# lodestone-rock/stable_diffusion_training

Measured on AMD Instinct MI355X. Metric: training images/sec, SD1.5 512×512 bf16, ε-pred MSE parity; 1/2/4/8 GPUs, higher is better.
Workload: dtype bf16; 1 GPU; SD1.5 512x512 train_step: VAE encode + CLIP-L fwd/bwd + UNet fwd/bwd + clip + Lion-8bit + EMA, batch 4/GPU, 77-token captions, random-init weights; global_batch=4, latent=64x64x4, parallelism=dp1, launch=hip_graph, setup_steps=3

## Files before the change

include/sdt.h:

```cpp
#ifndef SDT_H_
#define SDT_H_

#include <stdint.h>

#ifdef __cplusplus
extern "C" {
#endif

#ifndef __HIP_PLATFORM_AMD__
typedef struct ihipStream_t* hipStream_t;
#endif

enum { SDT_OK = 0, SDT_ERR_INVALID_ARG = -1, SDT_ERR_UNSUPPORTED = -2, SDT_ERR_LAUNCH = -3 };

const char* sdt_last_error(void);
int sdt_abi_version(void);
int sdt_device_count(void);

int sdt_event_create(void** event);
int sdt_event_destroy(void* event);
int sdt_event_record(void* event, int external, hipStream_t stream);
int sdt_stream_wait_event(hipStream_t stream, void* event);
int sdt_stream_wait_event_external(hipStream_t stream, void* event);

// ... 41 lines not shown
                             float offset_mag, float perturb_mag, int prediction_type, hipStream_t stream);
int sdt_inpaint_pack_input(const uint16_t* latents_nhwc, const uint16_t* masked_latents_nhwc, const float* latent_mask,
                           uint16_t* input_nhwc, int R, int B, int L, int H, int W, int cpad_src, int cpad_m, int cpad_dst,
                           hipStream_t stream);
int sdt_control_concat_add(const uint16_t* a, const uint16_t* skip, const uint16_t* res, const float* scale, uint16_t* wide,
                           int64_t rows, int64_t rows_per_sample, int Ca, int Cb, hipStream_t stream);
int sdt_ip_attention_fwd(const uint16_t* q, const uint16_t* kv, const uint16_t* o_txt, const float* scale_ip, uint16_t* out, int B, int H,
                         int Nq, int T, int D, int ldq, int ldkv, float scale, hipStream_t stream);
int sdt_ip_attention_bwd(const uint16_t* q, const uint16_t* kv, const uint16_t* dout, const float* scale_ip, const uint16_t* dq_in,
                         uint16_t* dq, uint16_t* dkv, int B, int H, int Nq, int T, int D, int ldq, int ldkv, int ld_dkv, float scale,
                         void* workspace, int64_t workspace_bytes, hipStream_t stream);
int64_t sdt_ip_attention_bwd_workspace_bytes(int B, int H, int Nq, int T, int D);
int sdt_mse_loss_fwd_bwd(const uint16_t* pred_nhwc, const float* target_nchw, const float* weight, float* loss_accum,
                         uint16_t* dpred_nhwc, int B, int C, int H, int W, int cpad, void* workspace, int64_t workspace_bytes,
                         hipStream_t stream);
int64_t sdt_reduce_workspace_bytes(void);
int sdt_loss_mask_prepare(const float* mask, float* effective, float* pooled, float* sums, int B, int h, int w, int f, float floor_value,
                          void* workspace, int64_t workspace_bytes, hipStream_t stream);
int sdt_masked_mse_loss_fwd_bwd(const uint16_t* pred_nhwc, const float* target_nchw, const float* effective_mask, const float* mask_sums,
                                const float* snr_weight, const float* loss_weight, float* loss_accum, float* loss_per_sample,
                                uint16_t* dpred_nhwc, int B, int C, int H, int W, int cpad, void* workspace, int64_t workspace_bytes,
                                hipStream_t stream);
int sdt_robust_loss_fwd_bwd(const uint16_t* pred_nhwc, const float* target_nchw, const float* effective_mask, const float* mask_sums,
                            const float* snr_weight, const float* loss_weight, const float* huber_c, int loss_type, float* loss_accum,
                            float* loss_per_sample, uint16_t* dpred_nhwc, int B, int C, int H, int W, int cpad, void* workspace,
                            int64_t workspace_bytes, hipStream_t stream);
int sdt_timestep_embedding(const int32_t* timesteps, uint16_t* out, int B, int dim, int flip_sin_to_cos,
                           float freq_shift, hipStream_t stream);

int sdt_sqnorm_accumulate(const float* g, int64_t n, double* out_sq, void* workspace, int64_t workspace_bytes, hipStream_t stream);
int sdt_sqnorm_accumulate_bf16(const uint16_t* g, int64_t n, double* out_sq, void* workspace, int64_t workspace_bytes, hipStream_t stream);
int64_t sdt_sqnorm_workspace_bytes(void);
#define SDT_ACC_INIT 0
#define SDT_ACC_ADD 1
#define SDT_ACC_FINISH 2
#define SDT_ACC_SCALE 3
int sdt_grad_accumulate(float* acc, const void* g, int g_bf16, int64_t n, int mode, float scale, double* out_sq, void* workspace,
                        int64_t workspace_bytes, hipStream_t stream);
int sdt_lion8_step(float* p, const void* g, int g_bf16, int8_t* codes, float* inv_scale, float* ema, uint16_t* w_bf16, int64_t n,
                   int block_size, const double* sqnorm, const float* thresholds, double max_norm, double lr, double wd,
                   double b1, double b2, double ema_rate, hipStream_t stream);
int sdt_lion32_step(float* p, const float* g, float* mom, float* ema, uint16_t* w_bf16, int64_t n,
                    const double* sqnorm, double max_norm, double lr, double wd, double b1, double b2, double ema_rate,
                    hipStream_t stream);
int sdt_opt_schedule_select(int64_t* step, const float* lr_tab, int64_t n_lr, const float* ema_tab, int64_t n_ema, float* cur,
                            hipStream_t stream);
int sdt_lion8_step_scheduled(float* p, const void* g, int g_bf16, int8_t* codes, float* inv_scale, float* ema, uint16_t* w_bf16,
                             int64_t n, int block_size, const double* sqnorm, const float* thresholds, double max_norm, const float* cur,
                             double wd, double b1, double b2, hipStream_t stream);
int sdt_lion32_step_scheduled(float* p, const float* g, float* mom, float* ema, uint16_t* w_bf16, int64_t n, const double* sqnorm,
                              double max_norm, const float* cur, double wd, double b1, double b2, hipStream_t stream);
int sdt_adamw_select(int64_t* step, double* prods, const float* lr_tab, int64_t n_lr, const float* ema_tab, int64_t n_ema, double lr,
                     double ema_rate, double b1, double b2, float* cur, hipStream_t stream);
int sdt_adamw8_step(float* p, const void* g, int g_bf16, int8_t* m_codes, float* m_inv_scale, int8_t* s_codes, float* s_inv_scale,
                    float* ema, uint16_t* w_bf16, int64_t n, int block_size, const double* sqnorm, const float* thresholds,
                    double max_norm, const float* cur, double wd, double b1, double b2, double eps, hipStream_t stream);
int sdt_adamw32_step(float* p, const float* g, float* m, float* v, float* ema, uint16_t* w_bf16, int64_t n, const double* sqnorm,
                     double max_norm, const float* cur, double wd, double b1, double b2, double eps, hipStream_t stream);
int sdt_prodigy_select(int64_t* step, double* state, const float* lr_tab, int64_t n_lr, const float* ema_tab, int64_t n_ema, double lr,
                       double ema_rate, double b1, double b2, double d0, int use_bias_correction, int safeguard_warmup, float* cur,
                       hipStream_t stream);
int sdt_prodigy_moments_step(const float* p, const void* g, int g_bf16, float* p0, float* m, float* v, float* s, int64_t n,
                             const double* sqnorm, double max_norm, const float* cur, double* state, double b1, double b2, double beta3,
                             void* workspace, int64_t workspace_bytes, hipStream_t stream);
int sdt_prodigy_finish(double* state, float* cur, double beta3, double d0, double d_coef, double growth_rate, double eps,
                       hipStream_t stream);
int sdt_prodigy_apply_step(float* p, const float* m, const float* v, float* ema, uint16_t* w_bf16, int64_t n, const float* cur, double wd,
                           hipStream_t stream);
int64_t sdt_prodigy_workspace_bytes(void);
int sdt_lion8_quantize(const float* x, int8_t* codes, float* inv_scale, int64_t n, int block_size, const float* thresholds,
                       hipStream_t stream);
int sdt_lion8_dequantize(const int8_t* codes, const float* inv_scale, float* x, int64_t n, int block_size,
                         hipStream_t stream);

int sdt_groupnorm_fwd(const uint16_t* x, const float* gamma, const float* beta, uint16_t* y, float* stats, int B, int HW,
                      int C, int G, float eps, int fuse_silu, const float* parts, int nparts, void* workspace,
                      int64_t workspace_bytes, hipStream_t stream);
int64_t sdt_groupnorm_fwd_workspace_bytes(int B, int HW, int C, int G);
int sdt_groupnorm_bwd(const uint16_t* x, const uint16_t* dy, const float* stats, const float* gamma, const float* beta,
                      uint16_t* dx, float* dgamma, float* dbeta, const uint16_t* dres, int B, int HW, int C, int G, float eps,
                      int fuse_silu, void* workspace, int64_t workspace_bytes, hipStream_t stream);
int64_t sdt_groupnorm_bwd_workspace_bytes(int B, int HW, int C);
int sdt_layernorm_fwd(const uint16_t* x, const float* gamma, const float* beta, uint16_t* y, float* mean_rstd, int64_t M,
                      int C, float eps, hipStream_t stream);
int sdt_layernorm_bwd(const uint16_t* x, const uint16_t* dy, const float* gamma, const float* mean_rstd, uint16_t* dx,
                      float* dgamma, float* dbeta, const uint16_t* dres, int64_t M, int C, int defer_param_grads, void* workspace,
                      int64_t workspace_bytes, hipStream_t stream);
int64_t sdt_layernorm_bwd_workspace_bytes(int64_t M, int C);
int64_t sdt_layernorm_bwd_partial_rows(int64_t M, int C);
typedef struct SdtNormGradJob {
  const float* partial;
  float* dgamma;
  float* dbeta;
  int nrows, C;
} SdtNormGradJob;
int sdt_norm_param_grads_group(const SdtNormGradJob* jobs, int n, hipStream_t stream);
int sdt_norm_param_grads_group_max(void);
int sdt_clip_pool_fwd(const int32_t* ids, const uint16_t* x, const float* gamma, const float* beta, uint16_t* pooled, float* mean_rstd,
                      int32_t* pos, int R, int windows, int S, int D, int eos_id, float eps, hipStream_t stream);
int sdt_clip_pool_bwd(const uint16_t* x, const uint16_t* dpooled, const float* gamma, const float* mean_rstd, const int32_t* pos,
                      uint16_t* dx, float* dgamma, float* dbeta, int R, int windows, int S, int D, hipStream_t stream);

int sdt_gemm_nt_bf16(const uint16_t* A, const uint16_t* Bt, uint16_t* C, const float* bias, const uint16_t* rowbias,
                     const uint16_t* residual, int64_t M, int N, int Kc, int taps, int lda, int ldb,
                     int64_t b_tap_stride, int ldc, int ldres, int rows_per_batch, int gather_mode,
                     const SdtConvGeom* geom, void* workspace, int64_t workspace_bytes, float* gn_stats, int gn_groups,
                     int b_kmajor, int b_nseg, int64_t b_seg_stride, int ld_rowbias, hipStream_t stream);
int sdt_gemm_nt_gn_parts(int64_t M, int N, int Kc, int taps, int rows_per_batch, int gn_groups, int gather_mode,
                         const SdtConvGeom* geom);
int64_t sdt_gemm_nt_workspace_bytes(int64_t M, int N, int Kc, int taps);
int sdt_ff_geglu_supported(int64_t M, int F, int K);
int sdt_ff_geglu_fwd(const uint16_t* x, const uint16_t* W1, const float* bias, uint16_t* h, uint16_t* out, int64_t M, int F, int K,
                     hipStream_t stream);


int sdt_gemm_tn_wgrad(const uint16_t* A, const uint16_t* dY, void* dW, int dw_bf16, float* dbias, int64_t M, int K1, int N, int K1_valid,
                      int N_valid, int taps, int lda, int ldb, int ldw, int64_t w_tap_stride, int n_seg, int64_t seg_stride,
                      int gather_mode, const SdtConvGeom* geom, void* workspace, int64_t workspace_bytes, double* sq_slots,
                      hipStream_t stream);
int64_t sdt_wgrad_sq_slots(int K1, int N, int taps);
int sdt_sum_f64_accumulate(const double* x, int64_t n, double* out, void* workspace, int64_t workspace_bytes, hipStream_t stream);
int64_t sdt_gemm_tn_workspace_bytes(int64_t M, int K1, int N, int taps, int n_seg, int gather_mode, const SdtConvGeom* geom);
typedef struct SdtTnProblem {
  const uint16_t* A;
  const uint16_t* dY;
  void* dW;
  float* dbias;
  int64_t M;
  int K1, N, K1_valid, N_valid, lda, ldb, ldw, n_seg;
  int64_t seg_stride;
  double* sq_slots;
  int dw_bf16;
} SdtTnProblem;
int sdt_gemm_tn_wgrad_group(const SdtTnProblem* problems, int n, void* workspace, int64_t workspace_bytes, hipStream_t stream);
int64_t sdt_gemm_tn_wgrad_group_workspace_bytes(const SdtTnProblem* problems, int n);
int sdt_gemm_tn_wgrad_group_max(void);
typedef struct SdtConvWgradProblem {
  const uint16_t* A;
  const uint16_t* dY;
  void* dW;
  float* dbias;
  SdtConvGeom geom;
  int K1, N, K1_valid, N_valid, lda, ldb;
  double* sq_slots;
  int dw_bf16;
} SdtConvWgradProblem;
int sdt_conv_wgrad_group(const SdtConvWgradProblem* problems, int n, void* workspace, int64_t workspace_bytes, hipStream_t stream);
int64_t sdt_conv_wgrad_group_workspace_bytes(const SdtConvWgradProblem* problems, int n);
int sdt_colsum_accumulate(const uint16_t* dy, float* db, int64_t M, int N, int ld, void* workspace, int64_t workspace_bytes,
                          hipStream_t stream);
int sdt_colsum_batched_bf16(const uint16_t* dy, uint16_t* out, int batch, int64_t rows_per_batch, int N, int ld, void* workspace,
                            int64_t workspace_bytes, hipStream_t stream);
int64_t sdt_colsum_workspace_bytes(int batch, int64_t rows_per_batch, int N);

int sdt_attention_fwd(const uint16_t* q, const uint16_t* k, const uint16_t* v, uint16_t* out, float* lse,
                      const SdtAttnDesc* desc, hipStream_t stream);
int sdt_attention_bwd(const uint16_t* q, const uint16_t* k, const uint16_t* v, const uint16_t* out, const uint16_t* dout,
                      const float* lse, uint16_t* dq, uint16_t* dk, uint16_t* dv, float* workspace, int64_t workspace_bytes,
                      const SdtAttnDesc* desc, hipStream_t stream);
int64_t sdt_attention_bwd_workspace_bytes(const SdtAttnDesc* desc);
int sdt_softmax_rows_inplace(uint16_t* x, int64_t rows, int n, float scale, hipStream_t stream);

int sdt_act_fwd(const uint16_t* x, uint16_t* y, int64_t n, int act, hipStream_t stream);
int sdt_act_bwd(const uint16_t* x, const uint16_t* dy, uint16_t* dx, int64_t n, int act, hipStream_t stream);
int sdt_geglu_fwd(const uint16_t* h, uint16_t* out, int64_t M, int F, hipStream_t stream);
int sdt_geglu_bwd(const uint16_t* h, const uint16_t* dout, uint16_t* dh, int64_t M, int F, hipStream_t stream);
int sdt_sum_n_bf16(const uint16_t* const* inputs, int n, uint16_t* out, int64_t numel, hipStream_t stream);
int sdt_copy2d_bf16(uint16_t* dst, int64_t dst_stride, const uint16_t* src, int64_t src_stride, int64_t rows, int cols,
                    hipStream_t stream);
int sdt_copy_cols_bf16(uint16_t* wide, int64_t ld_wide, void* const* parts, const int64_t* ld_parts, const int* cols, int n,
                       int64_t rows, int to_wide, hipStream_t stream);
int sdt_add_bf16(const uint16_t* a, const uint16_t* b, uint16_t* y, int64_t n, hipStream_t stream);
int sdt_upsample2x_fwd(const uint16_t* x, uint16_t* y, int B, int H, int W, int C, hipStream_t stream);
int sdt_upsample2x_bwd(const uint16_t* dy, uint16_t* dx, int B, int H, int W, int C, hipStream_t stream);
int sdt_nchw_f32_to_nhwc_bf16(const float* x, uint16_t* y, int B, int C, int H, int W, int cpad, hipStream_t stream);
int sdt_nhwc_bf16_to_nchw_f32(const uint16_t* x, float* y, int B, int C, int H, int W, int cpad, hipStream_t stream);
int sdt_cast_f32_to_bf16(const float* x, uint16_t* y, int64_t n, hipStream_t stream);
int sdt_transpose_bf16(const uint16_t* x, uint16_t* y, int batch, int R, int C, hipStream_t stream);
int sdt_param_prepare(const float* master, uint16_t* w_bf16, uint16_t* wt_bf16, const void* descs_device, int ndesc,
                      int total_tiles, hipStream_t stream);
int sdt_param_prepare_desc_size(void);
int sdt_zero_ranges(float* base, const int64_t* ranges_device, int nranges, hipStream_t stream);
int sdt_zero_ranges_chunk(void);
int sdt_embedding_fwd(const int32_t* ids, const float* tok, const float* pos, uint16_t* out, int64_t rows, int S, int D,
                      hipStream_t stream);
int sdt_embedding_bwd(const int32_t* ids, const uint16_t* dout, float* dtok, float* dpos, int64_t rows, int S, int D,
                      hipStream_t stream);

int sdt_embedding_ext_fwd(const int32_t* ids, const float* tok, const float* ext, const float* pos, uint16_t* out, int64_t rows, int S,
                          int D, int V, int n_ext, hipStream_t stream);
int sdt_embedding_ext_bwd(const int32_t* ids, const uint16_t* dout, float* dext, int64_t rows, int D, int V, int n_ext,
                          hipStream_t stream);
int sdt_embedding_retract(float* ext, int n_ext, int D, double target_std, double power, double* stats, hipStream_t stream);

typedef struct SdtLoraJob {
  int64_t w0_off;
  int64_t a_off, b_off;
  int64_t w_off, f_off;
  int64_t dw_off;
  int64_t ga_off, gb_off;
  int32_t K, N, r;
  float scale;
  int32_t tile0_merge, tile0_project, tiles_da, reserved;
} SdtLoraJob;
int sdt_lora_job_size(void);
int sdt_lora_merge(const float* w0_base, const float* ab_base, uint16_t* w_bf16, float* f32_dst, const SdtLoraJob* jobs_host,
                   const void* jobs_device, int n, hipStream_t stream);
int sdt_lora_project(const uint16_t* dw_base, const float* ab_base, float* grad_base, const SdtLoraJob* jobs_host,
                     const void* jobs_device, int n, hipStream_t stream);

typedef struct SdtDoraJob {
  int64_t m_off;
  int64_t gm_off;
  int64_t stat_off;
  int32_t N;
  int32_t stripe0_merge;
} SdtDoraJob;
int sdt_dora_job_size(void);
int sdt_dora_merge(const float* w0_base, const float* ab_base, uint16_t* w_bf16, float* f32_dst, float* stat_base,
                   const SdtLoraJob* jobs_host, const SdtDoraJob* dora_host, const void* jobs_device, const void* dora_device, int n,
                   hipStream_t stream);
int sdt_dora_init_magnitude(const float* w0_base, const float* ab_base, float* m_base, const SdtLoraJob* jobs_host,
                            const SdtDoraJob* dora_host, const void* jobs_device, const void* dora_device, int n, hipStream_t stream);
int sdt_dora_project(const uint16_t* dw_base, const float* w0_base, const float* ab_base, float* grad_base, const float* stat_base,
                     const SdtLoraJob* jobs_host, const SdtDoraJob* dora_host, const void* jobs_device, const void* dora_device, int n,
                     hipStream_t stream);

int sdt_dpo_loss_fwd_bwd(const uint16_t* pred_nhwc, const uint16_t* ref_pred_nhwc, const float* target_nchw, float beta, float* loss_accum,
                         float* sample_mse, float* logits, float* pair_loss, float* coef, uint16_t* dpred_nhwc, int B, int C, int H, int W,
                         int cpad, void* workspace, int64_t workspace_bytes, hipStream_t stream);
int64_t sdt_dpo_loss_workspace_bytes(int B, int H, int W);
int sdt_lora_restore(const float* w0_base, uint16_t* w_bf16, const SdtLoraJob* jobs_host, const void* jobs_device, int n,
                     hipStream_t stream);

typedef struct SdtLoraSplitJob {
  int64_t part_off;
  int32_t K, N;
  int32_t tile0;
  int32_t chunks;
  int32_t cnt0;
  int32_t reserved;
} SdtLoraSplitJob;
int sdt_lora_split_job_size(void);
int sdt_lora_project_split_rows(void);
int64_t sdt_lora_project_split_workspace_bytes(const SdtLoraJob* jobs_host, int n);
int sdt_lora_project_split(const uint16_t* dw_base, const float* ab_base, float* grad_base, const SdtLoraJob* jobs_host,
                           const SdtLoraSplitJob* split_host, const void* jobs_device, const void* split_device, int n, void* workspace,
                           int64_t workspace_bytes, hipStream_t stream);

typedef struct SdtLohaJob {
  int64_t a2_off, b2_off;
  int64_t ga2_off, gb2_off;
  int64_t part_off;
  int32_t K, N;
} SdtLohaJob;
int sdt_loha_job_size(void);
int sdt_loha_merge(const float* w0_base, const float* ab_base, uint16_t* w_bf16, float* f32_dst, const SdtLoraJob* jobs_host,
                   const SdtLohaJob* loha_host, const void* jobs_device, const void* loha_device, int n, hipStream_t stream);
int64_t sdt_loha_project_workspace_bytes(const SdtLoraJob* jobs_host, int n);
int sdt_loha_project(const uint16_t* dw_base, const float* ab_base, float* grad_base, const SdtLoraJob* jobs_host,
                     const SdtLoraSplitJob* split_host, const SdtLohaJob* loha_host, const void* jobs_device, const void* split_device,
                     const void* loha_device, int n, void* workspace, int64_t workspace_bytes, hipStream_t stream);

int sdt_conv_halo_set_tile_width(int bn);

#ifdef __cplusplus
}
#endif
#endif
```

stable_diffusion_training_amd/_lib.py:

```python
import ctypes
import os

_P = ctypes.c_void_p
_I = ctypes.c_int
_L = ctypes.c_int64
_F = ctypes.c_float
_D = ctypes.c_double


class SdtConvGeom(ctypes.Structure):
    _fields_ = [(n, _I) for n in ("batch", "in_h", "in_w", "out_h", "out_w", "kh", "kw", "stride", "pad_top", "pad_left")]


class SdtAttnDesc(ctypes.Structure):
    _fields_ = [("B", _I), ("H", _I), ("Nq", _I), ("Nk", _I), ("D", _I), ("ldq", _I), ("ldk", _I), ("ldv", _I),
                ("ldo", _I), ("scale", _F), ("causal", _I), ("ldgrad_q", _I), ("ldgrad_k", _I), ("ldgrad_v", _I),
                ("ld_dout", _I), ("key_weight", _P)]


class SdtPrepDesc(ctypes.Structure):
    _fields_ = [("src_off", _L), ("w_off", _L), ("wt_off", _L), ("batch", _I), ("R", _I), ("C", _I), ("Rp", _I),
                ("Cp", _I), ("tile0", _I), ("flags", _I)]


class SdtNormGradJob(ctypes.Structure):
    _fields_ = [("partial", _P), ("dgamma", _P), ("dbeta", _P), ("nrows", _I), ("C", _I)]


class SdtConvWgradProblem(ctypes.Structure):
    _fields_ = [("A", _P), ("dY", _P), ("dW", _P), ("dbias", _P), ("geom", SdtConvGeom), ("K1", _I), ("N", _I), ("K1_valid", _I),
                ("N_valid", _I), ("lda", _I), ("ldb", _I), ("sq_slots", _P), ("dw_bf16", _I)]


class SdtTnProblem(ctypes.Structure):
    _fields_ = [("A", _P), ("dY", _P), ("dW", _P), ("dbias", _P), ("M", _L), ("K1", _I), ("N", _I), ("K1_valid", _I),
                ("N_valid", _I), ("lda", _I), ("ldb", _I), ("ldw", _I), ("n_seg", _I), ("seg_stride", _L), ("sq_slots", _P), ("dw_bf16", _I)]


class SdtLoraJob(ctypes.Structure):
    _fields_ = [(n, _L) for n in ("w0_off", "a_off", "b_off", "w_off", "f_off", "dw_off", "ga_off", "gb_off")] + [
        ("K", _I), ("N", _I), ("r", _I), ("scale", _F), ("tile0_merge", _I), ("tile0_project", _I), ("tiles_da", _I), ("reserved", _I)]


class SdtDoraJob(ctypes.Structure):
    _fields_ = [("m_off", _L), ("gm_off", _L), ("stat_off", _L), ("N", _I), ("stripe0_merge", _I)]


class SdtLoraSplitJob(ctypes.Structure):
    _fields_ = [("part_off", _L), ("K", _I), ("N", _I), ("tile0", _I), ("chunks", _I), ("cnt0", _I), ("reserved", _I)]


class SdtLohaJob(ctypes.Structure):
    _fields_ = [(n, _L) for n in ("a2_off", "b2_off", "ga2_off", "gb2_off", "part_off")] + [("K", _I), ("N", _I)]


GATHER_PLAIN, GATHER_FPROP, GATHER_DGRAD = 0, 1, 2
ACT_SILU, ACT_QUICK_GELU, ACT_GELU_ERF = 0, 1, 2

SIGNATURES = {
    "sdt_add_noise_velocity": [_P, _P, _P, _P, _P, _P, _P, _I, _I, _I, _I, _I, _P],
    "sdt_vae_posterior_sample": [_P, _P, _P, _I, _I, _I, _I, _I, _F, _P],
    "sdt_latent_noise_target": [_P, _P, _P, _P, _P, _P, _P, _P, _P, _P, _P, _I, _I, _I, _I, _I, _I, _F, _F, _F, _I, _P],
    "sdt_inpaint_mask_pixels": [_P, _P, _P, _P, _I, _I, _I, _I, _I, _I, _P],
    "sdt_inpaint_noise_target": [_P, _P, _P, _P, _P, _P, _P, _P, _P, _P, _P, _P, _P, _P, _P, _I, _I, _I, _I, _I, _I, _F, _F, _F, _I, _P],
    "sdt_inpaint_pack_input": [_P, _P, _P, _P, _I, _I, _I, _I, _I, _I, _I, _I, _P],
    "sdt_control_concat_add": [_P, _P, _P, _P, _P, _L, _L, _I, _I, _P],
    "sdt_ip_attention_fwd": [_P, _P, _P, _P, _P, _I, _I, _I, _I, _I, _I, _I, _F, _P],
    "sdt_ip_attention_bwd": [_P, _P, _P, _P, _P, _P, _P, _I, _I, _I, _I, _I, _I, _I, _I, _F, _P, _L, _P],
    "sdt_ddim_cfg_step": [_P, _P, _P, _I, _I, _I, _I, _I, _F, _F, _F, _I, _P],
    "sdt_cfg_rescale_factors": [_P, _P, _I, _I, _I, _I, _I, _F, _F, _P],
    "sdt_sampler_cfg_step": [_P, _P, _P, _P, _P, _I, _I, _I, _I, _I, _F, _F, _F, _I, _F, _F, _F, _F, _P],
    "sdt_mse_loss_fwd_bwd": [_P, _P, _P, _P, _P, _I, _I, _I, _I, _I, _P, _L, _P],
    "sdt_loss_mask_prepare": [_P, _P, _P, _P, _I, _I, _I, _I, _F, _P, _L, _P],
    "sdt_masked_mse_loss_fwd_bwd": [_P, _P, _P, _P, _P, _P, _P, _P, _P, _I, _I, _I, _I, _I, _P, _L, _P],
    "sdt_robust_loss_fwd_bwd": [_P, _P, _P, _P, _P, _P, _P, _I, _P, _P, _P, _I, _I, _I, _I, _I, _P, _L, _P],
    "sdt_dpo_loss_fwd_bwd": [_P, _P, _P, _F, _P, _P, _P, _P, _P, _P, _I, _I, _I, _I, _I, _P, _L, _P],
    "sdt_timestep_embedding": [_P, _P, _I, _I, _I, _F, _P],
    "sdt_sqnorm_accumulate": [_P, _L, _P, _P, _L, _P],
    "sdt_sqnorm_accumulate_bf16": [_P, _L, _P, _P, _L, _P],
    "sdt_grad_accumulate": [_P, _P, _I, _L, _I, _F, _P, _P, _L, _P],
    "sdt_lion8_step": [_P, _P, _I, _P, _P, _P, _P, _L, _I, _P, _P, _D, _D, _D, _D, _D, _D, _P],
    "sdt_lion32_step": [_P, _P, _P, _P, _P, _L, _P, _D, _D, _D, _D, _D, _D, _P],
    "sdt_opt_schedule_select": [_P, _P, _L, _P, _L, _P, _P],
    "sdt_lion8_step_scheduled": [_P, _P, _I, _P, _P, _P, _P, _L, _I, _P, _P, _D, _P, _D, _D, _D, _P],
    "sdt_lion32_step_scheduled": [_P, _P, _P, _P, _P, _L, _P, _D, _P, _D, _D, _D, _P],
    "sdt_adamw_select": [_P, _P, _P, _L, _P, _L, _D, _D, _D, _D, _P, _P],
    "sdt_adamw8_step": [_P, _P, _I, _P, _P, _P, _P, _P, _P, _L, _I, _P, _P, _D, _P, _D, _D, _D, _D, _P],
    "sdt_adamw32_step": [_P, _P, _P, _P, _P, _P, _L, _P, _D, _P, _D, _D, _D, _D, _P],
    "sdt_prodigy_select": [_P, _P, _P, _L, _P, _L, _D, _D, _D, _D, _D, _I, _I, _P, _P],
    "sdt_prodigy_moments_step": [_P, _P, _I, _P, _P, _P, _P, _L, _P, _D, _P, _P, _D, _D, _D, _P, _L, _P],
    "sdt_prodigy_finish": [_P, _P, _D, _D, _D, _D, _D, _P],
    "sdt_prodigy_apply_step": [_P, _P, _P, _P, _P, _L, _P, _D, _P],
    "sdt_lion8_quantize": [_P, _P, _P, _L, _I, _P, _P],
    "sdt_lion8_dequantize": [_P, _P, _P, _L, _I, _P],
    "sdt_groupnorm_fwd": [_P, _P, _P, _P, _P, _I, _I, _I, _I, _F, _I, _P, _I, _P, _L, _P],
    "sdt_groupnorm_bwd": [_P, _P, _P, _P, _P, _P, _P, _P, _P, _I, _I, _I, _I, _F, _I, _P, _L, _P],
    "sdt_layernorm_fwd": [_P, _P, _P, _P, _P, _L, _I, _F, _P],
    "sdt_layernorm_bwd": [_P, _P, _P, _P, _P, _P, _P, _P, _L, _I, _I, _P, _L, _P],
    "sdt_norm_param_grads_group": [_P, _I, _P],
    "sdt_clip_pool_fwd": [_P, _P, _P, _P, _P, _P, _P, _I, _I, _I, _I, _I, _F, _P],
    "sdt_clip_pool_bwd": [_P, _P, _P, _P, _P, _P, _P, _P, _I, _I, _I, _I, _P],
    "sdt_sum_n_bf16": [_P, _I, _P, _L, _P],
    "sdt_event_create": [_P],
    "sdt_event_destroy": [_P],
    "sdt_event_record": [_P, _I, _P],
    "sdt_stream_wait_event": [_P, _P],
    "sdt_stream_wait_event_external": [_P, _P],
    "sdt_gemm_nt_bf16": [_P, _P, _P, _P, _P, _P, _L, _I, _I, _I, _I, _I, _L, _I, _I, _I, _I, _P, _P, _L, _P, _I, _I, _I, _L, _I, _P],
    "sdt_gemm_nt_gn_parts": [_L, _I, _I, _I, _I, _I, _I, _P],
    "sdt_gemm_tn_wgrad": [_P, _P, _P, _I, _P, _L, _I, _I, _I, _I, _I, _I, _I, _I, _L, _I, _L, _I, _P, _P, _L, _P, _P],
    "sdt_sum_f64_accumulate": [_P, _L, _P, _P, _L, _P],
    "sdt_gemm_tn_wgrad_group": [_P, _I, _P, _L, _P],
    "sdt_conv_wgrad_group": [_P, _I, _P, _L, _P],
    "sdt_zero_ranges": [_P, _P, _I, _P],
    "sdt_colsum_accumulate": [_P, _P, _L, _I, _I, _P, _L, _P],
    "sdt_colsum_batched_bf16": [_P, _P, _I, _L, _I, _I, _P, _L, _P],
    "sdt_attention_fwd": [_P, _P, _P, _P, _P, _P, _P],
    "sdt_attention_bwd": [_P, _P, _P, _P, _P, _P, _P, _P, _P, _P, _L, _P, _P],
    "sdt_softmax_rows_inplace": [_P, _L, _I, _F, _P],
    "sdt_act_fwd": [_P, _P, _L, _I, _P],
    "sdt_act_bwd": [_P, _P, _P, _L, _I, _P],
    "sdt_geglu_fwd": [_P, _P, _L, _I, _P],
    "sdt_geglu_bwd": [_P, _P, _P, _L, _I, _P],
    "sdt_copy2d_bf16": [_P, _L, _P, _L, _L, _I, _P],
    "sdt_copy_cols_bf16": [_P, _L, _P, _P, _P, _I, _L, _I, _P],
    "sdt_add_bf16": [_P, _P, _P, _L, _P],
    "sdt_upsample2x_fwd": [_P, _P, _I, _I, _I, _I, _P],
    "sdt_upsample2x_bwd": [_P, _P, _I, _I, _I, _I, _P],
    "sdt_nchw_f32_to_nhwc_bf16": [_P, _P, _I, _I, _I, _I, _I, _P],
    "sdt_nhwc_bf16_to_nchw_f32": [_P, _P, _I, _I, _I, _I, _I, _P],
    "sdt_cast_f32_to_bf16": [_P, _P, _L, _P],
    "sdt_transpose_bf16": [_P, _P, _I, _I, _I, _P],
    "sdt_param_prepare": [_P, _P, _P, _P, _I, _I, _P],
    "sdt_lora_merge": [_P, _P, _P, _P, _P, _P, _I, _P],
    "sdt_lora_restore": [_P, _P, _P, _P, _I, _P],
    "sdt_lora_project": [_P, _P, _P, _P, _P, _I, _P],
    "sdt_lora_project_split": [_P, _P, _P, _P, _P, _P, _P, _I, _P, _L, _P],
    "sdt_loha_merge": [_P, _P, _P, _P, _P, _P, _P, _P, _I, _P],
    "sdt_loha_project": [_P, _P, _P, _P, _P, _P, _P, _P, _P, _I, _P, _L, _P],
    "sdt_dora_merge": [_P, _P, _P, _P, _P, _P, _P, _P, _P, _I, _P],
    "sdt_dora_init_magnitude": [_P, _P, _P, _P, _P, _P, _P, _I, _P],
    "sdt_dora_project": [_P, _P, _P, _P, _P, _P, _P, _P, _P, _I, _P],
    "sdt_embedding_fwd": [_P, _P, _P, _P, _L, _I, _I, _P],
    "sdt_embedding_bwd": [_P, _P, _P, _P, _L, _I, _I, _P],
    "sdt_embedding_ext_fwd": [_P, _P, _P, _P, _P, _L, _I, _I, _I, _I, _P],
    "sdt_embedding_ext_bwd": [_P, _P, _P, _L, _I, _I, _I, _P],
    "sdt_embedding_retract": [_P, _I, _I, _D, _D, _P, _P],
    "sdt_ff_geglu_fwd": [_P, _P, _P, _P, _P, _L, _I, _I, _P],
    "sdt_ff_geglu_supported": [_L, _I, _I],
    "sdt_conv_halo_set_tile_width": [_I],
}
WS_QUERY = {"sdt_gemm_nt_workspace_bytes": [_L, _I, _I, _I], "sdt_gemm_tn_workspace_bytes": [_L, _I, _I, _I, _I, _I, _P], "sdt_layernorm_bwd_workspace_bytes": [_L, _I], "sdt_layernorm_bwd_partial_rows": [_L, _I],
            "sdt_groupnorm_bwd_workspace_bytes": [_I, _I, _I],
            "sdt_groupnorm_fwd_workspace_bytes": [_I, _I, _I, _I], "sdt_attention_bwd_workspace_bytes": [_P],
            "sdt_ip_attention_bwd_workspace_bytes": [_I, _I, _I, _I, _I],
            "sdt_gemm_tn_wgrad_group_workspace_bytes": [_P, _I], "sdt_conv_wgrad_group_workspace_bytes": [_P, _I], "sdt_reduce_workspace_bytes": [], "sdt_dpo_loss_workspace_bytes": [_I, _I, _I], "sdt_sqnorm_workspace_bytes": [], "sdt_prodigy_workspace_bytes": [], "sdt_colsum_workspace_bytes": [_I, _L, _I],
            "sdt_lora_project_split_workspace_bytes": [_P, _I],
            "sdt_loha_project_workspace_bytes": [_P, _I],
            "sdt_wgrad_sq_slots": [_I, _I, _I]}
NOARG = {"sdt_abi_version": _I, "sdt_gemm_tn_wgrad_group_max": _I, "sdt_norm_param_grads_group_max": _I, "sdt_zero_ranges_chunk": _I, "sdt_device_count": _I, "sdt_param_prepare_desc_size": _I, "sdt_lora_job_size": _I, "sdt_dora_job_size": _I, "sdt_lora_split_job_size": _I, "sdt_lora_project_split_rows": _I, "sdt_loha_job_size": _I, "sdt_last_error": ctypes.c_char_p}

LIB_PATH = os.path.join(os.path.dirname(os.path.abspath(__file__)), "csrc", "libsdtrain_hip.so")
if os.environ.get("SDT_LIB"):
    LIB_PATH = os.path.abspath(os.environ["SDT_LIB"])
_lib = None


class SdtError(RuntimeError):
    pass


def load():
    global _lib
    if _lib is not None:
        return _lib
    if not os.path.exists(LIB_PATH):
        raise SdtError(f"{LIB_PATH} is missing: run `python -c 'import __graft_entry__ as g; g.build()'` "
                       "(hipcc --offload-arch=gfx950). There is no CPU fallback.")
    import torch
    lib = ctypes.CDLL(LIB_PATH)
    for name, argtypes in SIGNATURES.items():
        fn = getattr(lib, name)
        fn.argtypes = argtypes
        fn.restype = _I
    for name, argtypes in WS_QUERY.items():
        fn = getattr(lib, name)
        fn.argtypes = argtypes
        fn.restype = _L
    for name, res in NOARG.items():
        fn = getattr(lib, name)
        fn.argtypes = []
        fn.restype = res
    if lib.sdt_param_prepare_desc_size() != ctypes.sizeof(SdtPrepDesc):
        raise SdtError("SdtPrepDesc layout mismatch between _lib.py and the library")
    if lib.sdt_lora_job_size() != ctypes.sizeof(SdtLoraJob):
        raise SdtError("SdtLoraJob layout mismatch between _lib.py and the library")
    if lib.sdt_dora_job_size() != ctypes.sizeof(SdtDoraJob):
        raise SdtError("SdtDoraJob layout mismatch between _lib.py and the library")
    if lib.sdt_lora_split_job_size() != ctypes.sizeof(SdtLoraSplitJob):
        raise SdtError("SdtLoraSplitJob layout mismatch between _lib.py and the library")
    if lib.sdt_loha_job_size() != ctypes.sizeof(SdtLohaJob):
        raise SdtError("SdtLohaJob layout mismatch between _lib.py and the library")
    _lib = lib
    return lib


def require_device():
    lib = load()
    if lib.sdt_device_count() < 1:
        raise SdtError("no HIP device visible: the train_step hot path runs only on the HIP kernels (no CPU fallback)")
    return lib


def call(name, *args):
    lib = _lib if _lib is not None else load()
    rc = getattr(lib, name)(*args)
    if rc != 0:
        raise SdtError(f"{name} failed ({rc}): {lib.sdt_last_error().decode()}")
```

stable_diffusion_training_amd/csrc/attention.hip:

```cpp
#include <type_traits>

#include "sdt_common.h"

#define KT 64
#define NEG_BIG -1.0e30f

typedef __attribute__((ext_vector_type(4))) short s16x4_t;

__device__ __attribute__((aligned(16))) unsigned int g_attn_zero16[4] = {0u, 0u, 0u, 0u};
__device__ __attribute__((aligned(16))) unsigned int g_attn_one16[4] = {0x3f80u, 0u, 0u, 0u};

__device__ __forceinline__ unsigned lds_offset_of(const void* p) {
  return (unsigned)(size_t)(__attribute__((address_space(3))) const unsigned char*)p;
}
__device__ __forceinline__ void glds16(const void* gsrc, void* lds_wave_base) {
  unsigned keep;
  asm volatile("s_mov_b32 %0, m0\n\ts_mov_b32 m0, %2\n\ts_nop 0\n\tglobal_load_lds_dwordx4 %1, off\n\ts_mov_b32 m0, %0"
               : "=&s"(keep) : "v"(gsrc), "s"(lds_offset_of(lds_wave_base)) : "memory");
}
__device__ __forceinline__ void glds4(const void* gsrc, void* lds_wave_base) {
  unsigned keep;
  asm volatile("s_mov_b32 %0, m0\n\ts_mov_b32 m0, %2\n\ts_nop 0\n\tglobal_load_lds_dword %1, off\n\ts_mov_b32 m0, %0"
               : "=&s"(keep) : "v"(gsrc), "s"(lds_offset_of(lds_wave_base)) : "memory");
}
// ... 241 lines not shown
        }
      if (!MSUM) l_run += psum;
    }
  };
  attn_tile_loops(tiles, p.key_w != nullptr, p.causal != 0, 0, kend, p.Nk);
  float l_tot;
  if (MSUM) l_tot = __shfl(o_acc[NB - 1][12], fr, 64);
  else l_tot = l_run + __shfl_xor(l_run, 32, 64);
  const float inv_l = 1.f / l_tot;
  if (qi < p.Nq) {
    if (fh == 0 && p.lse) p.lse[((long)b * p.H + h) * p.Nq + qi] = m_run * p.scale2 + log2f(l_tot);
    bf16_t* ob = p.out + (long)b * p.bso + (long)qi * p.ldo + h * p.D;
#pragma unroll
    for (int i = 0; i < NB; ++i)
#pragma unroll
      for (int g4 = 0; g4 < 4; ++g4) {
        const int d = i * 32 + 8 * g4 + 4 * fh;
        if (d < p.D) {
          uint2 pk;
          pk.x = pack2bf(o_acc[i][4 * g4] * inv_l, o_acc[i][4 * g4 + 1] * inv_l);
          pk.y = pack2bf(o_acc[i][4 * g4 + 2] * inv_l, o_acc[i][4 * g4 + 3] * inv_l);
          *reinterpret_cast<uint2*>(ob + d) = pk;
        }
      }
  }
}

template <int DPP, int NS, int NB>
__global__ void __launch_bounds__(256) attn_bwd_dq_kernel(const AttnParams p) {
  extern __shared__ __attribute__((aligned(16))) unsigned char smem[];
  using I = Img<DPP>;
  constexpr int STAGE = 2 * I::BYTES;
  const int lane = threadIdx.x & 63, wave = threadIdx.x >> 6, fr = lane & 31, fh = lane >> 5;
  const int wave_u = __builtin_amdgcn_readfirstlane(wave);
  const int b = blockIdx.z, h = blockIdx.y;
  const int q0 = blockIdx.x * 128;
  const int qi = q0 + wave * 32 + fr;
  const bf16_t* qb = p.q + (long)b * p.bsq + h * p.D;
  const bf16_t* dob = p.dout + (long)b * p.bsdo + h * p.D;
  const bf16_t* kb = p.k + (long)b * p.bsk + h * p.D;
  const bf16_t* vb = p.v + (long)b * p.bsv + h * p.D;

  TileDma<DPP> dma, dmav;
  dma.init(wave, lane, p.D);
  dmav.init(wave, lane, p.D);
  TrLane<DPP> tr;
  tr.init(lane);
  int kend = p.Nk;
  if (p.causal) kend = min(p.Nk, q0 + 128);
  dma.bind(kb, p.ldk, 0);
  dmav.bind(vb, p.ldv, 0);
  dma.issue(0, p.Nk, smem, wave_u);
  dmav.issue(0, p.Nk, smem + I::BYTES, wave_u);

  bf16x8_t qf[NS], dof[NS];
#pragma unroll
  for (int s = 0; s < NS; ++s) {
    uint4 v = make_uint4(0, 0, 0, 0), w = make_uint4(0, 0, 0, 0);
    const int d0 = 16 * s + 8 * fh;
    if (qi < p.Nq && d0 < p.D) {
      v = *reinterpret_cast<const uint4*>(qb + (long)qi * p.ldq + d0);
      w = *reinterpret_cast<const uint4*>(dob + (long)qi * p.lddo + d0);
    }
    qf[s] = __builtin_bit_cast(bf16x8_t, v);
    dof[s] = __builtin_bit_cast(bf16x8_t, w);
  }
  float lse2 = 0.f, dlt = 0.f;
  if (qi < p.Nq) {
    lse2 = p.lse[((long)b * p.H + h) * p.Nq + qi];
    const bf16_t* orow = p.o + (long)b * p.bso + (long)qi * p.ldo + h * p.D;
#pragma unroll
    for (int s = 0; s < NS; ++s) {
      const int d0 = 16 * s + 8 * fh;
      if (d0 < p.D) {
        float fo[8], fd[8];
        unpack8(*reinterpret_cast<const uint4*>(orow + d0), fo);
        unpack8(__builtin_bit_cast(uint4, dof[s]), fd);
#pragma unroll
        for (int e = 0; e < 8; ++e) dlt += fo[e] * fd[e];
      }
    }
  }
  dlt += __shfl_xor(dlt, 32, 64);
  if (qi < p.Nq && fh == 0) const_cast<float*>(p.delta)[((long)b * p.H + h) * p.Nq + qi] = dlt;
  f32x16_t dq_acc[NB];
#pragma unroll
  for (int i = 0; i < NB; ++i)
#pragma unroll
    for (int e = 0; e < 16; ++e) dq_acc[i][e] = 0.f;

  int cur = 0;
  auto tiles = [&](auto masked, auto weighted, int kfrom, int kto) {
    constexpr bool MASK = decltype(masked)::value, KW = decltype(weighted)::value;
    for (int kbase = kfrom; kbase < kto; kbase += KT, cur ^= 1) {
      dma_join();
      if (kbase + KT < kend) {
        dma.issue(kbase + KT, p.Nk, smem + (cur ^ 1) * STAGE, wave_u);
        dmav.issue(kbase + KT, p.Nk, smem + (cur ^ 1) * STAGE + I::BYTES, wave_u);
      }
      const unsigned char* k_img = smem + cur * STAGE;
      const unsigned char* v_img = k_img + I::BYTES;
#pragma unroll
      for (int kt = 0; kt < 2; ++kt) {
        f32x16_t st, dpt;
#pragma unroll
        for (int e = 0; e < 16; ++e) { st[e] = 0.f; dpt[e] = -dlt; }
#pragma unroll
        for (int s = 0; s < NS; ++s) {
          const bf16x8_t kf = row_frag<DPP>(k_img, kt * 32 + fr, 2 * s + fh);
          st = __builtin_amdgcn_mfma_f32_32x32x16_bf16(kf, qf[s], st, 0, 0, 0);
          const bf16x8_t vf = row_frag<DPP>(v_img, kt * 32 + fr, 2 * s + fh);
          dpt = __builtin_amdgcn_mfma_f32_32x32x16_bf16(vf, dof[s], dpt, 0, 0, 0);
        }
        float ds[16];
#pragma unroll
        for (int e = 0; e < 16; ++e) {
          float pv = __builtin_amdgcn_exp2f(fmaf(st[e], p.scale2, -lse2));
          const int key = kbase + kt * 32 + (e & 3) + 8 * (e >> 2) + 4 * fh;
          if (MASK) pv = (key >= p.Nk || (p.causal && key > qi) || qi >= p.Nq) ? 0.f : pv;
          if (KW) pv *= p.key_w[min(key, p.Nk - 1)];
          ds[e] = pv * dpt[e];
        }
#pragma unroll
        for (int s = 0; s < 2; ++s) {
          const bf16x8_t dsf = cvt_frag(ds + 8 * s);
#pragma unroll
          for (int i = 0; i < NB; ++i) {
            const bf16x8_t ktf = tr.frag(k_img, kt * 32 + 16 * s, i);
            dq_acc[i] = __builtin_amdgcn_mfma_f32_32x32x16_bf16(ktf, dsf, dq_acc[i], 0, 0, 0);
          }
        }
      }
    }
  };
  attn_tile_loops(tiles, p.key_w != nullptr, p.causal || q0 + 128 > p.Nq, 0, kend, p.Nk);
  if (qi < p.Nq) {
    bf16_t* ob = p.dq + (long)b * p.bsdq + (long)qi * p.lddq + h * p.D;
#pragma unroll
    for (int i = 0; i < NB; ++i)
#pragma unroll
      for (int g4 = 0; g4 < 4; ++g4) {
        const int d = i * 32 + 8 * g4 + 4 * fh;
        if (d < p.D) {
          uint2 pk;
          pk.x = pack2bf(dq_acc[i][4 * g4] * p.scale, dq_acc[i][4 * g4 + 1] * p.scale);
          pk.y = pack2bf(dq_acc[i][4 * g4 + 2] * p.scale, dq_acc[i][4 * g4 + 3] * p.scale);
          *reinterpret_cast<uint2*>(ob + d) = pk;
        }
      }
  }
}

template <int DPP, int NS, int NB, bool QSPLIT>
__global__ void __launch_bounds__(256) attn_bwd_dkv_kernel(const AttnParams p) {
  extern __shared__ __attribute__((aligned(16))) unsigned char smem[];
  using I = Img<DPP>;
  constexpr int STAGE = 2 * I::BYTES + 2 * KT * 4;
  const int lane = threadIdx.x & 63, wave = threadIdx.x >> 6, fr = lane & 31, fh = lane >> 5;
  const int wave_u = __builtin_amdgcn_readfirstlane(wave);
  const int b = blockIdx.z, h = blockIdx.y;
  const int kblk = QSPLIT ? (int)blockIdx.x % p.kblocks : (int)blockIdx.x;
  const int k0 = kblk * 128;
  const int ki = k0 + wave * 32 + fr;
  const float kwt = p.key_w ? p.key_w[min(ki, p.Nk - 1)] : 1.f;
  const bf16_t* qb = p.q + (long)b * p.bsq + h * p.D;
  const bf16_t* dob = p.dout + (long)b * p.bsdo + h * p.D;
  const bf16_t* kb = p.k + (long)b * p.bsk + h * p.D;
  const bf16_t* vb = p.v + (long)b * p.bsv + h * p.D;
  const float* lse_g = p.lse + ((long)b * p.H + h) * p.Nq;
  const float* dlt_g = p.delta + ((long)b * p.H + h) * p.Nq;

  TileDma<DPP> dma, dmad;
  dma.init(wave, lane, p.D);
  dmad.init(wave, lane, p.D);
  TrLane<DPP> tr;
  tr.init(lane);
  int qstart = 0, qend = p.Nq;
  if (p.causal) qstart = (k0 / KT) * KT;
  if (QSPLIT) {
    qstart = ((int)blockIdx.x / p.kblocks) * p.qchunk;
    qend = min(p.Nq, qstart + p.qchunk);
  }
  dma.bind(qb, p.ldq, qstart);
  dmad.bind(dob, p.lddo, qstart);
  auto stage = [&](int qbase, unsigned char* st) {
    dma.issue(qbase, p.Nq, st, wave_u);
    dmad.issue(qbase, p.Nq, st + I::BYTES, wave_u);
    if (wave_u < 2) {
      const int q = min(qbase + lane, p.Nq - 1);
      glds4((wave_u == 0 ? lse_g : dlt_g) + q, st + 2 * I::BYTES + wave_u * (KT * 4));
    }
  };
  if (qstart < qend) stage(qstart, smem);

  bf16x8_t kf[NS], vf[NS];
#pragma unroll
  for (int s = 0; s < NS; ++s) {
    uint4 v = make_uint4(0, 0, 0, 0), w = make_uint4(0, 0, 0, 0);
    const int d0 = 16 * s + 8 * fh;
    if (ki < p.Nk && d0 < p.D) {
      v = *reinterpret_cast<const uint4*>(kb + (long)ki * p.ldk + d0);
      w = *reinterpret_cast<const uint4*>(vb + (long)ki * p.ldv + d0);
    }
    kf[s] = __builtin_bit_cast(bf16x8_t, v);
    vf[s] = __builtin_bit_cast(bf16x8_t, w);
  }
  f32x16_t dk_acc[NB], dv_acc[NB];
#pragma unroll
  for (int i = 0; i < NB; ++i)
#pragma unroll
    for (int e = 0; e < 16; ++e) { dk_acc[i][e] = 0.f; dv_acc[i][e] = 0.f; }

  int cur = 0;
  auto tiles = [&](auto masked, auto weighted, int qfrom, int qto) {
    constexpr bool MASK = decltype(masked)::value, KW = decltype(weighted)::value;
    for (int qbase = qfrom; qbase < qto; qbase += KT, cur ^= 1) {
      dma_join();
      if (qbase + KT < qend) stage(qbase + KT, smem + (cur ^ 1) * STAGE);
      const unsigned char* q_img = smem + cur * STAGE;
      const unsigned char* do_img = q_img + I::BYTES;
      const float* lse_s = reinterpret_cast<const float*>(q_img + 2 * I::BYTES);
      const float* dlt_s = lse_s + KT;
#pragma unroll
      for (int qt = 0; qt < 2; ++qt) {
        f32x16_t sa, dpa;
        float lrow[16];
#pragma unroll
        for (int g4 = 0; g4 < 4; ++g4) {
          const float4 l4 = *reinterpret_cast<const float4*>(lse_s + qt * 32 + 8 * g4 + 4 * fh);
          const float4 d4 = *reinterpret_cast<const float4*>(dlt_s + qt * 32 + 8 * g4 + 4 * fh);
          lrow[4 * g4] = l4.x; lrow[4 * g4 + 1] = l4.y; lrow[4 * g4 + 2] = l4.z; lrow[4 * g4 + 3] = l4.w;
          dpa[4 * g4] = -d4.x; dpa[4 * g4 + 1] = -d4.y; dpa[4 * g4 + 2] = -d4.z; dpa[4 * g4 + 3] = -d4.w;
        }
#pragma unroll
        for (int e = 0; e < 16; ++e) sa[e] = 0.f;
#pragma unroll
        for (int s = 0; s < NS; ++s) {
          const bf16x8_t qf = row_frag<DPP>(q_img, qt * 32 + fr, 2 * s + fh);
          sa = __builtin_amdgcn_mfma_f32_32x32x16_bf16(qf, kf[s], sa, 0, 0, 0);
          const bf16x8_t df = row_frag<DPP>(do_img, qt * 32 + fr, 2 * s + fh);
          dpa = __builtin_amdgcn_mfma_f32_32x32x16_bf16(df, vf[s], dpa, 0, 0, 0);
        }
        float pr[16], ds[16];
#pragma unroll
        for (int e = 0; e < 16; ++e) {
          float pv = __builtin_amdgcn_exp2f(fmaf(sa[e], p.scale2, -lrow[e]));
          if (KW) pv *= kwt;
          if (MASK) {
            const int q = qbase + qt * 32 + (e & 3) + 8 * (e >> 2) + 4 * fh;
            pv = (q >= p.Nq || ki >= p.Nk || (p.causal && ki > q)) ? 0.f : pv;
          }
          pr[e] = pv;
          ds[e] = pv * dpa[e];
        }
#pragma unroll
        for (int s = 0; s < 2; ++s) {
          const bf16x8_t pf = cvt_frag(pr + 8 * s);
          const bf16x8_t dsf = cvt_frag(ds + 8 * s);
#pragma unroll
          for (int i = 0; i < NB; ++i) {
            const bf16x8_t dotf = tr.frag(do_img, qt * 32 + 16 * s, i);
            dv_acc[i] = __builtin_amdgcn_mfma_f32_32x32x16_bf16(dotf, pf, dv_acc[i], 0, 0, 0);
            const bf16x8_t qtf = tr.frag(q_img, qt * 32 + 16 * s, i);
            dk_acc[i] = __builtin_amdgcn_mfma_f32_32x32x16_bf16(qtf, dsf, dk_acc[i], 0, 0, 0);
          }
        }
      }
    }
  };
  attn_tile_loops(tiles, p.key_w != nullptr, p.causal || k0 + 128 > p.Nk, qstart, qend, p.Nq);
  if (QSPLIT) {
    if (ki < p.Nk) {
      const long C = (long)p.H * p.D;
      const long slab = 2 * (long)p.B * p.Nk * C;
      float* wk = p.kv_ws + ((int)blockIdx.x / p.kblocks) * slab + ((long)b * p.Nk + ki) * C + h * p.D;
      float* wv = wk + (long)p.B * p.Nk * C;
#pragma unroll
      for (int i = 0; i < NB; ++i)
#pragma unroll
        for (int g4 = 0; g4 < 4; ++g4) {
          const int d = i * 32 + 8 * g4 + 4 * fh;
          if (d < p.D) {
            *reinterpret_cast<float4*>(wk + d) = make_float4(dk_acc[i][4 * g4] * p.scale, dk_acc[i][4 * g4 + 1] * p.scale,
                                                             dk_acc[i][4 * g4 + 2] * p.scale, dk_acc[i][4 * g4 + 3] * p.scale);
            *reinterpret_cast<float4*>(wv + d) = make_float4(dv_acc[i][4 * g4], dv_acc[i][4 * g4 + 1], dv_acc[i][4 * g4 + 2], dv_acc[i][4 * g4 + 3]);
          }
        }
    }
    return;
  }
  if (ki < p.Nk) {
    bf16_t* dkb = p.dk + (long)b * p.bsdk + (long)ki * p.lddk + h * p.D;
    bf16_t* dvb = p.dv + (long)b * p.bsdv + (long)ki * p.lddv + h * p.D;
#pragma unroll
    for (int i = 0; i < NB; ++i)
#pragma unroll
      for (int g4 = 0; g4 < 4; ++g4) {
        const int d = i * 32 + 8 * g4 + 4 * fh;
        if (d < p.D) {
          uint2 pk;
          pk.x = pack2bf(dk_acc[i][4 * g4] * p.scale, dk_acc[i][4 * g4 + 1] * p.scale);
          pk.y = pack2bf(dk_acc[i][4 * g4 + 2] * p.scale, dk_acc[i][4 * g4 + 3] * p.scale);
          *reinterpret_cast<uint2*>(dkb + d) = pk;
          pk.x = pack2bf(dv_acc[i][4 * g4], dv_acc[i][4 * g4 + 1]);
          pk.y = pack2bf(dv_acc[i][4 * g4 + 2], dv_acc[i][4 * g4 + 3]);
          *reinterpret_cast<uint2*>(dvb + d) = pk;
        }
      }
  }
}

__global__ void __launch_bounds__(256) attn_kv_finish_kernel(const AttnParams p, int nsplit) {
  const int C = p.H * p.D, cv = C >> 3;
  const long rows = (long)p.B * p.Nk, total = rows * cv;
  const long slab = 2 * rows * C;
  for (long i = (long)blockIdx.x * blockDim.x + threadIdx.x; i < total; i += (long)gridDim.x * blockDim.x) {
    const long r = i / cv;
    const int c = (int)(i - r * cv) * 8;
    const int b = (int)(r / p.Nk), ki = (int)(r - (long)b * p.Nk);
    float fk[8], fv[8];
#pragma unroll
    for (int e = 0; e < 8; ++e) { fk[e] = 0.f; fv[e] = 0.f; }
    for (int sp = 0; sp < nsplit; ++sp) {
      const float* wk = p.kv_ws + sp * slab + r * C + c;
      const float* wv = wk + rows * C;
      const float4 a0 = *reinterpret_cast<const float4*>(wk), a1 = *reinterpret_cast<const float4*>(wk + 4);
      const float4 b0 = *reinterpret_cast<const float4*>(wv), b1 = *reinterpret_cast<const float4*>(wv + 4);
      fk[0] += a0.x; fk[1] += a0.y; fk[2] += a0.z; fk[3] += a0.w; fk[4] += a1.x; fk[5] += a1.y; fk[6] += a1.z; fk[7] += a1.w;
      fv[0] += b0.x; fv[1] += b0.y; fv[2] += b0.z; fv[3] += b0.w; fv[4] += b1.x; fv[5] += b1.y; fv[6] += b1.z; fv[7] += b1.w;
    }
    *reinterpret_cast<uint4*>(p.dk + (long)b * p.bsdk + (long)ki * p.lddk + c) = pack8(fk);
    *reinterpret_cast<uint4*>(p.dv + (long)b * p.bsdv + (long)ki * p.lddv + c) = pack8(fv);
  }
}

static int attn_qsplits(int B, int H, int Nq, int Nk, int causal) {
  if (causal) return 1;
  const long base = (long)sdt_ceil_div(Nk, 128) * H * B;
  if (base >= 128 || Nq < 1024) return 1;
  int s = (int)((256 + base - 1) / base);
  const int max_s = Nq / 256;
  if (s > max_s) s = max_s;
  return s < 2 ? 1 : s;
}

static int attn_fill(AttnParams* p, const SdtAttnDesc* d, const char* name) {
  SDT_CHECK_ARG(d, "%s: null descriptor", name);
  SDT_CHECK_ARG(d->B > 0 && d->H > 0 && d->Nq > 0 && d->Nk > 0 && d->D > 0 && d->B <= 65535 && d->H <= 65535,
                "%s: bad shape B=%d H=%d Nq=%d Nk=%d D=%d", name, d->B, d->H, d->Nq, d->Nk, d->D);
  SDT_CHECK_ARG(d->D % 8 == 0 && d->D <= 160, "%s: head dim %d must be a multiple of 8 and <= 160", name, d->D);
  SDT_CHECK_ARG(d->ldq % 8 == 0 && d->ldk % 8 == 0 && d->ldv % 8 == 0 && d->ldo % 8 == 0, "%s: row strides must be multiples of 8", name);
  SDT_CHECK_ARG(d->ldq < (1 << 24) && d->ldk < (1 << 24) && d->ldv < (1 << 24) && d->ldo < (1 << 24) && d->ld_dout < (1 << 24),
                "%s: row strides must be below 2^24 elements (a tile's byte step is kept in 32 bits)", name);
  p->B = d->B; p->H = d->H; p->Nq = d->Nq; p->Nk = d->Nk; p->D = d->D;
  p->ldq = d->ldq; p->ldk = d->ldk; p->ldv = d->ldv; p->ldo = d->ldo;
  p->bsq = (long)d->Nq * d->ldq; p->bsk = (long)d->Nk * d->ldk; p->bsv = (long)d->Nk * d->ldv; p->bso = (long)d->Nq * d->ldo;
  p->lddo = d->ldo; p->bsdo = p->bso;
  p->lddq = d->ldq; p->bsdq = p->bsq; p->lddk = d->ldk; p->bsdk = p->bsk; p->lddv = d->ldv; p->bsdv = p->bsv;
  p->scale = d->scale;
  p->scale2 = d->scale * 1.4426950408889634f;
  p->causal = d->causal;
  p->key_w = d->key_weight;
  return SDT_OK;
}

template <typename K>
static void ensure_lds(K kernel, size_t lds, bool* done) {
  if (!*done) {
    hipFuncSetAttribute((const void*)kernel, hipFuncAttributeMaxDynamicSharedMemorySize, (int)lds);
    *done = true;
  }
}
template <int DPP, int NS, int NB>
static void launch_fwd(const AttnParams& p, hipStream_t stream) {
  static_assert(NB * 32 <= DPP && NS * 16 <= DPP, "image pitch too small");
  static bool set_m = false, set_a = false;
  const size_t lds = (size_t)2 * 2 * Img<DPP>::BYTES;
  const dim3 grid(sdt_ceil_div(p.Nq, 128), p.H, p.B);
  if (p.D <= NB * 32 - 8) {
    ensure_lds(attn_fwd_kernel<DPP, NS, NB, true>, lds, &set_m);
    hipLaunchKernelGGL((attn_fwd_kernel<DPP, NS, NB, true>), grid, dim3(256), lds, stream, p);
  } else {
    ensure_lds(attn_fwd_kernel<DPP, NS, NB, false>, lds, &set_a);
    hipLaunchKernelGGL((attn_fwd_kernel<DPP, NS, NB, false>), grid, dim3(256), lds, stream, p);
  }
}
template <int DPP, int NS, int NB>
static void launch_bwd(const AttnParams& p, hipStream_t stream) {
  static_assert(NB * 32 <= DPP && NS * 16 <= DPP, "image pitch too small");
  static bool set_q = false, set_kv = false;
  const size_t lds_dq = (size_t)2 * 2 * Img<DPP>::BYTES;
  const size_t lds_dkv = (size_t)2 * (2 * Img<DPP>::BYTES + 2 * KT * sizeof(float));
  static bool set_kvs = false;
  ensure_lds(attn_bwd_dq_kernel<DPP, NS, NB>, lds_dq, &set_q);
  hipLaunchKernelGGL((attn_bwd_dq_kernel<DPP, NS, NB>), dim3(sdt_ceil_div(p.Nq, 128), p.H, p.B), dim3(256), lds_dq, stream, p);
  if (p.kv_ws) {
    AttnParams ps = p;
    const int splits = attn_qsplits(p.B, p.H, p.Nq, p.Nk, p.causal);
    ps.kblocks = sdt_ceil_div(p.Nk, 128);
    ps.qchunk = sdt_ceil_div(sdt_ceil_div(p.Nq, splits), KT) * KT;
    const int nsplit = sdt_ceil_div(p.Nq, ps.qchunk);
    ensure_lds(attn_bwd_dkv_kernel<DPP, NS, NB, true>, lds_dkv, &set_kvs);
    hipLaunchKernelGGL((attn_bwd_dkv_kernel<DPP, NS, NB, true>), dim3(ps.kblocks * nsplit, p.H, p.B), dim3(256), lds_dkv, stream, ps);
    hipLaunchKernelGGL(attn_kv_finish_kernel, dim3(sdt_grid_1d((long)p.B * p.Nk * p.H * p.D / 8, 256, 1024)), dim3(256), 0, stream, ps, nsplit);
  } else {
    ensure_lds(attn_bwd_dkv_kernel<DPP, NS, NB, false>, lds_dkv, &set_kv);
    hipLaunchKernelGGL((attn_bwd_dkv_kernel<DPP, NS, NB, false>), dim3(sdt_ceil_div(p.Nk, 128), p.H, p.B), dim3(256), lds_dkv, stream, p);
  }
}

extern "C" {

int sdt_attention_fwd(const uint16_t* q, const uint16_t* k, const uint16_t* v, uint16_t* out, float* lse,
                      const SdtAttnDesc* desc, hipStream_t stream) {
  SDT_CHECK_ARG(q && k && v && out, "sdt_attention_fwd: null pointer");
  AttnParams p = {};
  int rc = attn_fill(&p, desc, "sdt_attention_fwd");
  if (rc) return rc;
  SDT_CHECK_ARG((((uintptr_t)q | (uintptr_t)k | (uintptr_t)v | (uintptr_t)out) & 15) == 0, "sdt_attention_fwd: pointers must be 16-byte aligned");
  p.q = (const bf16_t*)q; p.k = (const bf16_t*)k; p.v = (const bf16_t*)v; p.out = (bf16_t*)out; p.lse = lse;
  const int D = p.D;
  if (D <= 48) launch_fwd<64, 3, 2>(p, stream);
  else if (D <= 64) launch_fwd<64, 4, 2>(p, stream);
  else if (D <= 80) launch_fwd<128, 5, 3>(p, stream);
  else if (D <= 96) launch_fwd<128, 6, 3>(p, stream);
  else if (D <= 128) launch_fwd<128, 8, 4>(p, stream);
  else launch_fwd<256, 10, 5>(p, stream);
  SDT_LAUNCH_CHECK("sdt_attention_fwd");
  return SDT_OK;
}

int64_t sdt_attention_bwd_workspace_bytes(const SdtAttnDesc* d) {
  if (!d || d->B <= 0 || d->H <= 0 || d->Nq <= 0 || d->Nk <= 0 || d->D <= 0) return 0;
  int64_t n = (int64_t)d->B * d->H * d->Nq;
  n = (n + 3) / 4 * 4;
  const int qs = attn_qsplits(d->B, d->H, d->Nq, d->Nk, d->causal);
  if (qs > 1) n += (int64_t)qs * 2 * d->B * d->Nk * d->H * d->D;
  return n * (int64_t)sizeof(float);
}

int sdt_attention_bwd(const uint16_t* q, const uint16_t* k, const uint16_t* v, const uint16_t* out, const uint16_t* dout,
                      const float* lse, uint16_t* dq, uint16_t* dk, uint16_t* dv, float* delta_ws, int64_t workspace_bytes,
                      const SdtAttnDesc* desc, hipStream_t stream) {
  SDT_CHECK_ARG(q && k && v && out && dout && lse && dq && dk && dv && delta_ws, "sdt_attention_bwd: null pointer");
  SDT_CHECK_ARG(desc && workspace_bytes >= (int64_t)sizeof(float) * desc->B * desc->H * desc->Nq, "sdt_attention_bwd: workspace too small");
  AttnParams p = {};
  int rc = attn_fill(&p, desc, "sdt_attention_bwd");
  if (rc) return rc;
  p.q = (const bf16_t*)q; p.k = (const bf16_t*)k; p.v = (const bf16_t*)v; p.o = (const bf16_t*)out;
  p.dout = (const bf16_t*)dout; p.lse = const_cast<float*>(lse); p.delta = delta_ws;
  p.dq = (bf16_t*)dq; p.dk = (bf16_t*)dk; p.dv = (bf16_t*)dv;
  if (desc->ldgrad_q) { p.lddq = desc->ldgrad_q; p.bsdq = (long)p.Nq * p.lddq; }
  if (desc->ldgrad_k) { p.lddk = desc->ldgrad_k; p.bsdk = (long)p.Nk * p.lddk; }
  if (desc->ldgrad_v) { p.lddv = desc->ldgrad_v; p.bsdv = (long)p.Nk * p.lddv; }
  if (desc->ld_dout) { p.lddo = desc->ld_dout; p.bsdo = (long)p.Nq * p.lddo; }
  if (attn_qsplits(p.B, p.H, p.Nq, p.Nk, p.causal) > 1 && workspace_bytes >= sdt_attention_bwd_workspace_bytes(desc))
    p.kv_ws = delta_ws + ((long)p.B * p.H * p.Nq + 3) / 4 * 4;
  const int D = p.D;
  if (D <= 48) launch_bwd<64, 3, 2>(p, stream);
  else if (D <= 64) launch_bwd<64, 4, 2>(p, stream);
  else if (D <= 80) launch_bwd<128, 5, 3>(p, stream);
  else if (D <= 96) launch_bwd<128, 6, 3>(p, stream);
  else if (D <= 128) launch_bwd<128, 8, 4>(p, stream);
  else launch_bwd<256, 10, 5>(p, stream);
  SDT_LAUNCH_CHECK("sdt_attention_bwd");
  return SDT_OK;
}

}
```

stable_diffusion_training_amd/csrc/elementwise.hip:

```cpp
#include "sdt_common.h"

__global__ void __launch_bounds__(256) add_noise_kernel(const float* __restrict__ lat, const float* __restrict__ noise,
                                                        const int* __restrict__ t, const float* __restrict__ acp,
                                                        bf16_t* __restrict__ noisy_nhwc, float* __restrict__ noisy_nchw,
                                                        float* __restrict__ vel_nchw, int B, int C, int HW, int cpad) {
  const long total = (long)B * HW;
  for (long i = (long)blockIdx.x * blockDim.x + threadIdx.x; i < total; i += (long)gridDim.x * blockDim.x) {
    const int b = (int)(i / HW), p = (int)(i % HW);
    const float a = acp[t[b]];
    const float sa = sqrtf(a), so = sqrtf(1.0f - a);
    for (int c = 0; c < cpad; ++c) {
      float nz = 0.f;
      if (c < C) {
        const long off = ((long)b * C + c) * HW + p;
        const float x0 = lat[off], e = noise[off];
        nz = sa * x0 + so * e;
        if (noisy_nchw) noisy_nchw[off] = nz;
        if (vel_nchw) vel_nchw[off] = sa * e - so * x0;
      }
      noisy_nhwc[i * cpad + c] = f2bf(nz);
    }
  }
}

// ... 973 lines not shown
                   ((d.src_off | d.w_off | d.wt_off) & 3) == 0;
  if (vec) {
#pragma unroll
    for (int ps = 0; ps < 4; ++ps) {
      const int r = ps * 16 + (threadIdx.x >> 4), c = (threadIdx.x & 15) * 4;
      const float4 f = *reinterpret_cast<const float4*>(src + (long)(r0 + r) * d.C + c0 + c);
      uint2 pk;
      pk.x = pack2bf(f.x, f.y);
      pk.y = pack2bf(f.z, f.w);
      *reinterpret_cast<uint2*>(w + (long)(r0 + r) * d.Cp + c0 + c) = pk;
      tile[r][c] = (bf16_t)(pk.x & 0xffffu); tile[r][c + 1] = (bf16_t)(pk.x >> 16);
      tile[r][c + 2] = (bf16_t)(pk.y & 0xffffu); tile[r][c + 3] = (bf16_t)(pk.y >> 16);
    }
    if (!wt) return;
    __syncthreads();
#pragma unroll
    for (int ps = 0; ps < 4; ++ps) {
      const int c = ps * 16 + (threadIdx.x >> 4), r = (threadIdx.x & 15) * 4;
      uint2 pk;
      pk.x = (unsigned)(unsigned short)tile[r][c] | ((unsigned)(unsigned short)tile[r + 1][c] << 16);
      pk.y = (unsigned)(unsigned short)tile[r + 2][c] | ((unsigned)(unsigned short)tile[r + 3][c] << 16);
      *reinterpret_cast<uint2*>(wt + (long)(c0 + c) * d.Rp + r0 + r) = pk;
    }
    return;
  }
  for (int i = threadIdx.x; i < 64 * 64; i += 256) {
    const int r = i >> 6, c = i & 63;
    bf16_t v = 0;
    if (r0 + r < d.R && c0 + c < d.C) v = f2bf(src[(long)(r0 + r) * d.C + c0 + c]);
    tile[r][c] = v;
    if (r0 + r < d.Rp && c0 + c < d.Cp) w[(long)(r0 + r) * d.Cp + c0 + c] = v;
  }
  if (!wt) return;
  __syncthreads();
  for (int i = threadIdx.x; i < 64 * 64; i += 256) {
    const int c = i >> 6, r = i & 63;
    if (r0 + r < d.Rp && c0 + c < d.Cp) wt[(long)(c0 + c) * d.Rp + r0 + r] = tile[r][c];
  }
}

__global__ void __launch_bounds__(256) embedding_fwd_kernel(const int* __restrict__ ids, const float* __restrict__ tok,
                                                            const float* __restrict__ pos, bf16_t* __restrict__ out,
                                                            long rows, int S, int D) {
  const long total = rows * D;
  for (long i = (long)blockIdx.x * blockDim.x + threadIdx.x; i < total; i += (long)gridDim.x * blockDim.x) {
    const long r = i / D;
    const int c = (int)(i % D);
    out[i] = f2bf(tok[(long)ids[r] * D + c] + pos[(long)(r % S) * D + c]);
  }
}
__global__ void __launch_bounds__(256) embedding_bwd_kernel(const int* __restrict__ ids, const bf16_t* __restrict__ dout,
                                                            float* __restrict__ dtok, float* __restrict__ dpos, long rows,
                                                            int S, int D) {
  const long blk = blockIdx.x;
  if (blk >= rows) {
    const long s0 = blk - rows;
    for (int c = threadIdx.x; c < D; c += 256) {
      float g = 0.f;
      for (long r = s0; r < rows; r += S) g += bf2f(dout[r * D + c]);
      dpos[s0 * D + c] += g;
    }
    return;
  }
  const int id = ids[blk];
  int dup = 0;
  for (long j = threadIdx.x; j < blk; j += 256) dup |= ids[j] == id;
  if (__syncthreads_or(dup)) return;
  for (int c = threadIdx.x; c < D; c += 256) {
    float g = 0.f;
    for (long j = blk; j < rows; ++j)
      if (ids[j] == id) g += bf2f(dout[j * D + c]);
    dtok[(long)id * D + c] += g;
  }
}

__device__ __forceinline__ const float* embedding_ext_row(int id, const float* tok, const float* ext, int D, int V, int n_ext) {
  if (id >= 0 && id < V) return tok + (long)id * D;
  const long e = (long)id - V;
  if (e >= 0 && e < n_ext) return ext + e * D;
  return nullptr;
}
template <bool VEC>
__global__ void __launch_bounds__(256) embedding_ext_fwd_kernel(const int* __restrict__ ids, const float* __restrict__ tok,
                                                                const float* __restrict__ ext, const float* __restrict__ pos,
                                                                bf16_t* __restrict__ out, long rows, int S, int D, int V, int n_ext) {
  if (VEC) {
    const int dv = D >> 2;
    const long total = rows * dv;
    for (long i = (long)blockIdx.x * blockDim.x + threadIdx.x; i < total; i += (long)gridDim.x * blockDim.x) {
      const long r = i / dv;
      const int c = (int)(i % dv) << 2;
      const float* t = embedding_ext_row(ids[r], tok, ext, D, V, n_ext);
      const float4 a = t ? *reinterpret_cast<const float4*>(t + c) : make_float4(0.f, 0.f, 0.f, 0.f);
      const float4 p = *reinterpret_cast<const float4*>(pos + (long)(r % S) * D + c);
      uint2 o;
      o.x = (unsigned)f2bf(a.x + p.x) | ((unsigned)f2bf(a.y + p.y) << 16);
      o.y = (unsigned)f2bf(a.z + p.z) | ((unsigned)f2bf(a.w + p.w) << 16);
      *reinterpret_cast<uint2*>(out + r * D + c) = o;
    }
  } else {
    const long total = rows * D;
    for (long i = (long)blockIdx.x * blockDim.x + threadIdx.x; i < total; i += (long)gridDim.x * blockDim.x) {
      const long r = i / D;
      const int c = (int)(i % D);
      const float* t = embedding_ext_row(ids[r], tok, ext, D, V, n_ext);
      out[i] = f2bf((t ? t[c] : 0.f) + pos[(long)(r % S) * D + c]);
    }
  }
}
__global__ void __launch_bounds__(256) embedding_ext_bwd_kernel(const int* __restrict__ ids, const bf16_t* __restrict__ dout,
                                                                float* __restrict__ dext, long rows, int D, int V) {
  const int j = blockIdx.x;
  const int c = blockIdx.y * 256 + threadIdx.x;
  const long want = (long)V + j;
  if (c >= D) return;
  float g = 0.f;
  for (long r = 0; r < rows; ++r)
    if ((long)ids[r] == want) g += bf2f(dout[r * D + c]);
  dext[(long)j * D + c] = g;
}
__device__ __forceinline__ double block_tree_sum_256(double v, double* sm) {
  const int t = threadIdx.x;
  __syncthreads();
  sm[t] = v;
  __syncthreads();
  for (int s = 128; s > 0; s >>= 1) {
    if (t < s) sm[t] += sm[t + s];
    __syncthreads();
  }
  return sm[0];
}
__global__ void __launch_bounds__(256) embedding_retract_kernel(float* __restrict__ ext, long n, double target_std, double power,
                                                                double* __restrict__ stats) {
  __shared__ double sm[256];
  double s = 0.0;
  for (long i = threadIdx.x; i < n; i += 256) s += (double)ext[i];
  const double mean = block_tree_sum_256(s, sm) / (double)n;
  double q = 0.0;
  for (long i = threadIdx.x; i < n; i += 256) {
    const double d = (double)ext[i] - mean;
    q += d * d;
  }
  const double ss = block_tree_sum_256(q, sm);
  const double sd = n > 1 ? sqrt(ss / (double)(n - 1)) : 0.0;
  const float factor = sd == 0.0 ? 1.0f : (float)pow(target_std / sd, power);
  for (long i = threadIdx.x; i < n; i += 256) ext[i] = ext[i] * factor;
  if (threadIdx.x == 0) {
    stats[0] = mean;
    stats[1] = sd;
    stats[2] = (double)factor;
  }
}

__global__ void __launch_bounds__(256) colsum_kernel(const bf16_t* __restrict__ dy, float* __restrict__ db, bf16_t* __restrict__ out_bf,
                                                     long M, int N, int ld, int rows_per_block, long batch_stride_dy,
                                                     int batch_stride_db, int* counters, float* __restrict__ part) {
  dy += (long)blockIdx.z * batch_stride_dy;
  __shared__ float red[8][32][8];
  __shared__ int s_last;
  const int tx = threadIdx.x & 31, ty = threadIdx.x >> 5;
  const int cv = blockIdx.x * 32 + tx;
  const long m0 = (long)blockIdx.y * rows_per_block;
  const long m1 = (m0 + rows_per_block < M) ? m0 + rows_per_block : M;
  float acc[8] = {0, 0, 0, 0, 0, 0, 0, 0};
  if (cv * 8 < N) {
    for (long m = m0 + ty; m < m1; m += 8) {
      float f[8];
      unpack8(*reinterpret_cast<const uint4*>(dy + m * ld + cv * 8), f);
#pragma unroll
      for (int j = 0; j < 8; ++j) acc[j] += f[j];
    }
  }
#pragma unroll
  for (int j = 0; j < 8; ++j) red[ty][tx][j] = acc[j];
  __syncthreads();
  const int group = blockIdx.z * gridDim.x + blockIdx.x;
  float* grp = part + (long)group * gridDim.y * 256;
  {
    const int col = threadIdx.x;
    float sum = 0.f;
#pragma unroll
    for (int k = 0; k < 8; ++k) sum += red[k][col >> 3][col & 7];
    sdt_store_wt(grp + (long)blockIdx.y * 256 + col, sum);
  }
  if (!sdt_arrive_last<true>(counters + group, (int)gridDim.y, &s_last)) return;
  const int n = blockIdx.x * 256 + threadIdx.x;
  if (n < N) {
    float t = 0.f;
    for (int y = 0; y < (int)gridDim.y; ++y) t += sdt_load_wt(grp + (long)y * 256 + threadIdx.x);
    if (out_bf) out_bf[(long)blockIdx.z * batch_stride_db + n] = f2bf(t);
    else db[(long)blockIdx.z * batch_stride_db + n] += t;
  }
}


__global__ void __launch_bounds__(256) softmax_rows_kernel(bf16_t* __restrict__ x, int n, float scale) {
  __shared__ float scratch[16];
  bf16_t* row = x + (long)blockIdx.x * n;
  float mx = -3.0e38f;
  for (int i = threadIdx.x; i < n; i += blockDim.x) mx = fmaxf(mx, bf2f(row[i]) * scale);
  mx = wave_max(mx);
  {
    const int w = threadIdx.x >> 6;
    if ((threadIdx.x & 63) == 0) scratch[w] = mx;
    __syncthreads();
    mx = scratch[0];
    for (int i = 1; i < (int)(blockDim.x >> 6); ++i) mx = fmaxf(mx, scratch[i]);
  }
  float s = 0.f;
  for (int i = threadIdx.x; i < n; i += blockDim.x) s += __expf(bf2f(row[i]) * scale - mx);
  s = block_sum(s, scratch);
  const float inv = 1.f / s;
  for (int i = threadIdx.x; i < n; i += blockDim.x) row[i] = f2bf(__expf(bf2f(row[i]) * scale - mx) * inv);
}

struct SumPtrs { const uint4* p[32]; };
__global__ void __launch_bounds__(256) sum_n_kernel(const SumPtrs ptrs, uint4* __restrict__ out, int n, long nvec) {
  for (long i = (long)blockIdx.x * blockDim.x + threadIdx.x; i < nvec; i += (long)gridDim.x * blockDim.x) {
    float acc[8], f[8];
    unpack8(ptrs.p[0][i], acc);
    for (int k = 1; k < n; ++k) {
      unpack8(ptrs.p[k][i], f);
#pragma unroll
      for (int e = 0; e < 8; ++e) acc[e] += f[e];
    }
    out[i] = pack8(acc);
  }
}


#define ZR_CHUNK 4096
__global__ void __launch_bounds__(256) zero_ranges_kernel(float4* __restrict__ base, const long* __restrict__ ranges) {
  const long first = ranges[2 * blockIdx.x], count = ranges[2 * blockIdx.x + 1];
  for (long i = threadIdx.x; i < count; i += 256) base[first + i] = make_float4(0.f, 0.f, 0.f, 0.f);
}

#define MASKED_MAX_BLOCKS 128
#define MASKED_MAX_B 8192
static int masked_blocks(int B, long hw) {
  long nb = (hw + 255) / 256, fit = (65536 / (long)sizeof(float) - B) / B;
  if (nb > MASKED_MAX_BLOCKS) nb = MASKED_MAX_BLOCKS;
  if (nb > fit) nb = fit;
  return (int)(nb < 1 ? 1 : nb);
}

template <int F>
static void loss_mask_prepare_launch(bool vec, dim3 grid, hipStream_t stream, const float* mask, float floor_v, float* e, float* mp,
                                     float* S, int h, int w, int* counters, float* part) {
  if (vec) hipLaunchKernelGGL((loss_mask_prepare_kernel<F, (F >= 4)>), grid, dim3(256), 0, stream, mask, floor_v, e, mp, S, h, w, counters, part);
  else hipLaunchKernelGGL((loss_mask_prepare_kernel<F, false>), grid, dim3(256), 0, stream, mask, floor_v, e, mp, S, h, w, counters, part);
}

extern "C" {

int sdt_add_noise_velocity(const float* latents, const float* noise, const int32_t* timesteps,
                           const float* alphas_cumprod, uint16_t* noisy_nhwc_bf16, float* noisy_nchw,
                           float* velocity_nchw, int B, int C, int H, int W, int cpad, hipStream_t stream) {
  SDT_CHECK_ARG(latents && noise && timesteps && alphas_cumprod && noisy_nhwc_bf16, "sdt_add_noise_velocity: null pointer");
  SDT_CHECK_ARG(B > 0 && C > 0 && H > 0 && W > 0 && cpad >= C, "sdt_add_noise_velocity: bad shape B=%d C=%d H=%d W=%d cpad=%d", B, C, H, W, cpad);
  hipLaunchKernelGGL(add_noise_kernel, dim3(sdt_grid_1d((long)B * H * W, 256)), dim3(256), 0, stream, latents, noise,
                     timesteps, alphas_cumprod, (bf16_t*)noisy_nhwc_bf16, noisy_nchw, velocity_nchw, B, C, H * W, cpad);
  SDT_LAUNCH_CHECK("sdt_add_noise_velocity");
  return SDT_OK;
}

int sdt_ddim_cfg_step(const uint16_t* pred_nhwc, float* latents_nchw, uint16_t* next_input_nhwc, int B, int C, int H, int W,
                      int cpad, float guidance_scale, float alpha_prod_t, float alpha_prod_prev, int prediction_type,
                      hipStream_t stream) {
  SDT_CHECK_ARG(pred_nhwc && latents_nchw && next_input_nhwc, "sdt_ddim_cfg_step: null pointer");
  SDT_CHECK_ARG(B > 0 && C > 0 && H > 0 && W > 0 && cpad >= C, "sdt_ddim_cfg_step: bad shape B=%d C=%d H=%d W=%d cpad=%d", B, C, H, W, cpad);
  SDT_CHECK_ARG(prediction_type >= 0 && prediction_type <= 2, "sdt_ddim_cfg_step: prediction_type %d (0 epsilon, 1 sample, 2 v_prediction)", prediction_type);
  SDT_CHECK_ARG(alpha_prod_t > 0.f && alpha_prod_t <= 1.f && alpha_prod_prev > 0.f && alpha_prod_prev <= 1.f,
                "sdt_ddim_cfg_step: alpha products must lie in (0, 1]");
  hipLaunchKernelGGL(ddim_cfg_step_kernel, dim3(sdt_grid_1d((long)B * H * W, 256)), dim3(256), 0, stream, (const bf16_t*)pred_nhwc,
                     latents_nchw, (bf16_t*)next_input_nhwc, B, C, H * W, cpad, guidance_scale, sqrtf(alpha_prod_t),
                     sqrtf(1.0f - alpha_prod_t), sqrtf(alpha_prod_prev), sqrtf(1.0f - alpha_prod_prev), prediction_type);
  SDT_LAUNCH_CHECK("sdt_ddim_cfg_step");
  return SDT_OK;
}

int sdt_cfg_rescale_factors(const uint16_t* pred_nhwc, float* factors, int B, int C, int H, int W, int cpad, float guidance_scale,
                            float guidance_rescale, hipStream_t stream) {
  SDT_CHECK_ARG(pred_nhwc && factors, "sdt_cfg_rescale_factors: null pointer");
  SDT_CHECK_ARG(((uintptr_t)pred_nhwc & 15) == 0, "sdt_cfg_rescale_factors: pred_nhwc misaligned (16 bytes)");
  SDT_CHECK_ARG(B > 0 && C > 0 && H > 0 && W > 0 && cpad >= C && cpad % 8 == 0 && (long)C * H * W >= 2,
                "sdt_cfg_rescale_factors: bad shape B=%d C=%d H=%d W=%d cpad=%d (cpad a multiple of 8, C*H*W >= 2)", B, C, H, W, cpad);
  SDT_CHECK_ARG(guidance_rescale >= 0.f && guidance_rescale <= 1.f && std::isfinite(guidance_scale),
                "sdt_cfg_rescale_factors: guidance_rescale %g must lie in [0, 1], guidance_scale finite", guidance_rescale);
  hipLaunchKernelGGL(cfg_rescale_factors_kernel, dim3(B), dim3(256), 0, stream, (const uint4*)pred_nhwc, factors, B, C, H * W, cpad,
                     guidance_scale, guidance_rescale);
  SDT_LAUNCH_CHECK("sdt_cfg_rescale_factors");
  return SDT_OK;
}

int sdt_sampler_cfg_step(const uint16_t* pred_nhwc, float* latents_nchw, uint16_t* next_input_nhwc, float* x0_history_nchw,
                         const float* rescale_factors, int B, int C, int H, int W, int cpad, float guidance_scale, float alpha_s,
                         float sigma_s, int prediction_type, float c_x, float c_x0, float c_eps, float c_d1, hipStream_t stream) {
  SDT_CHECK_ARG(pred_nhwc && latents_nchw && next_input_nhwc, "sdt_sampler_cfg_step: null pointer");
  SDT_CHECK_ARG((((uintptr_t)pred_nhwc | (uintptr_t)next_input_nhwc) & 15) == 0, "sdt_sampler_cfg_step: pred / next input misaligned (16 bytes)");
  SDT_CHECK_ARG(B > 0 && C > 0 && H > 0 && W > 0 && cpad >= C && cpad % 8 == 0,
                "sdt_sampler_cfg_step: bad shape B=%d C=%d H=%d W=%d cpad=%d (cpad a multiple of 8)", B, C, H, W, cpad);
  SDT_CHECK_ARG(prediction_type >= 0 && prediction_type <= 2, "sdt_sampler_cfg_step: prediction_type %d (0 epsilon, 1 sample, 2 v_prediction)", prediction_type);
  SDT_CHECK_ARG(alpha_s >= 0.f && alpha_s <= 1.f && sigma_s >= 0.f && sigma_s <= 1.f, "sdt_sampler_cfg_step: alpha_s / sigma_s must lie in [0, 1]");
  SDT_CHECK_ARG(!(prediction_type == 0 && alpha_s == 0.f) && !(prediction_type == 1 && sigma_s == 0.f),
                "sdt_sampler_cfg_step: %s prediction needs %s > 0", prediction_type == 0 ? "epsilon" : "sample",
                prediction_type == 0 ? "alpha_s" : "sigma_s");
  SDT_CHECK_ARG(std::isfinite(guidance_scale) && std::isfinite(c_x) && std::isfinite(c_x0) && std::isfinite(c_eps) && std::isfinite(c_d1),
                "sdt_sampler_cfg_step: guidance scale and coefficients must be finite");
  SDT_CHECK_ARG(c_d1 == 0.f || x0_history_nchw, "sdt_sampler_cfg_step: c_d1 != 0 needs the x0 history");
  hipLaunchKernelGGL(sampler_cfg_step_kernel, dim3(sdt_grid_1d((long)B * H * W, 256)), dim3(256), 0, stream, (const uint4*)pred_nhwc,
                     latents_nchw, (uint4*)next_input_nhwc, x0_history_nchw, rescale_factors, B, C, H * W, cpad, guidance_scale,
                     alpha_s, sigma_s, prediction_type, c_x, c_x0, c_eps, c_d1);
  SDT_LAUNCH_CHECK("sdt_sampler_cfg_step");
  return SDT_OK;
}

int sdt_vae_posterior_sample(const uint16_t* moments_nhwc, const float* eps_nhwc, float* latents_nchw, int B, int L,
                             int H, int W, int moment_stride, float scale, hipStream_t stream) {
  SDT_CHECK_ARG(moments_nhwc && eps_nhwc && latents_nchw && B > 0 && L > 0 && moment_stride >= 2 * L,
                "sdt_vae_posterior_sample: bad args");
  hipLaunchKernelGGL(posterior_sample_kernel, dim3(sdt_grid_1d((long)B * H * W * L, 256)), dim3(256), 0, stream,
                     (const bf16_t*)moments_nhwc, eps_nhwc, latents_nchw, B, L, H * W, moment_stride, scale);
  SDT_LAUNCH_CHECK("sdt_vae_posterior_sample");
  return SDT_OK;
}

int sdt_latent_noise_target(const uint16_t* moments_nhwc, const float* eps_nhwc, const float* noise_nchw, const float* offset,
                            const float* perturb_nchw, const int32_t* timesteps, const float* alphas_cumprod,
                            uint16_t* noisy_nhwc_bf16, float* target_nchw, float* latents_nchw, float* noisy_nchw, int B, int L,
                            int H, int W, int moment_stride, int cpad, float scale, float offset_mag, float perturb_mag,
                            int prediction_type, hipStream_t stream) {
  SDT_CHECK_ARG(moments_nhwc && eps_nhwc && noise_nchw && timesteps && alphas_cumprod && noisy_nhwc_bf16,
                "sdt_latent_noise_target: null pointer");
  SDT_CHECK_ARG(B > 0 && L > 0 && H > 0 && W > 0 && cpad >= L && moment_stride >= 2 * L,
                "sdt_latent_noise_target: bad shape B=%d L=%d H=%d W=%d moment_stride=%d cpad=%d (cpad >= L, moment_stride >= 2L)", B, L,
                H, W, moment_stride, cpad);
  SDT_CHECK_ARG(prediction_type == 0 || prediction_type == 2,
                "sdt_latent_noise_target: prediction_type %d (0 epsilon, 2 v_prediction)", prediction_type);
  SDT_CHECK_ARG(offset || offset_mag == 0.f, "sdt_latent_noise_target: offset_mag %g needs the offset noise", offset_mag);
  SDT_CHECK_ARG(perturb_nchw || perturb_mag == 0.f, "sdt_latent_noise_target: perturb_mag %g needs the perturbation noise", perturb_mag);
  SDT_CHECK_ARG(target_nchw || (prediction_type == 0 && !offset && !perturb_nchw),
                "sdt_latent_noise_target: the target may be NULL only for epsilon without offset or perturbation noise (it is the noise)");
  const bool vin = moment_stride % 8 == 0 && L % 4 == 0 && ((uintptr_t)moments_nhwc & 15) == 0;
  const bool vout = cpad % 8 == 0 && ((uintptr_t)noisy_nhwc_bf16 & 15) == 0;
  auto kern = vin ? (vout ? latent_noise_target_kernel<true, true> : latent_noise_target_kernel<true, false>)
// ... 333 lines not shown
  SDT_LAUNCH_CHECK("sdt_copy_cols_bf16");
  return SDT_OK;
}

int sdt_add_bf16(const uint16_t* a, const uint16_t* b, uint16_t* y, int64_t n, hipStream_t stream) {
  SDT_CHECK_ARG(a && b && y, "sdt_add_bf16: null pointer");
  int rc = check_vec(a, b, y, n, "sdt_add_bf16");
  if (rc) return rc;
  if (n == 0) return SDT_OK;
  hipLaunchKernelGGL(add_kernel, dim3(sdt_grid_1d(n / 8, 256)), dim3(256), 0, stream, (const uint4*)a, (const uint4*)b,
                     (uint4*)y, (long)(n / 8));
  SDT_LAUNCH_CHECK("sdt_add_bf16");
  return SDT_OK;
}

int sdt_upsample2x_fwd(const uint16_t* x, uint16_t* y, int B, int H, int W, int C, hipStream_t stream) {
  SDT_CHECK_ARG(x && y && B > 0 && H > 0 && W > 0 && C > 0 && C % 8 == 0, "sdt_upsample2x_fwd: bad args");
  hipLaunchKernelGGL(upsample2x_fwd_kernel, dim3(sdt_grid_1d((long)B * 4 * H * W * (C / 8), 256)), dim3(256), 0, stream,
                     (const uint4*)x, (uint4*)y, B, H, W, C / 8);
  SDT_LAUNCH_CHECK("sdt_upsample2x_fwd");
  return SDT_OK;
}

int sdt_upsample2x_bwd(const uint16_t* dy, uint16_t* dx, int B, int H, int W, int C, hipStream_t stream) {
  SDT_CHECK_ARG(dy && dx && B > 0 && H > 0 && W > 0 && C > 0 && C % 8 == 0, "sdt_upsample2x_bwd: bad args");
  hipLaunchKernelGGL(upsample2x_bwd_kernel, dim3(sdt_grid_1d((long)B * H * W * (C / 8), 256)), dim3(256), 0, stream,
                     (const uint4*)dy, (uint4*)dx, B, H, W, C / 8);
  SDT_LAUNCH_CHECK("sdt_upsample2x_bwd");
  return SDT_OK;
}

int sdt_nchw_f32_to_nhwc_bf16(const float* x, uint16_t* y, int B, int C, int H, int W, int cpad, hipStream_t stream) {
  SDT_CHECK_ARG(x && y && B > 0 && C > 0 && cpad >= C, "sdt_nchw_f32_to_nhwc_bf16: bad args");
  hipLaunchKernelGGL(nchw_to_nhwc_kernel, dim3(sdt_grid_1d((long)B * H * W * cpad, 256)), dim3(256), 0, stream, x,
                     (bf16_t*)y, B, C, H * W, cpad);
  SDT_LAUNCH_CHECK("sdt_nchw_f32_to_nhwc_bf16");
  return SDT_OK;
}

int sdt_nhwc_bf16_to_nchw_f32(const uint16_t* x, float* y, int B, int C, int H, int W, int cpad, hipStream_t stream) {
  SDT_CHECK_ARG(x && y && B > 0 && C > 0 && cpad >= C, "sdt_nhwc_bf16_to_nchw_f32: bad args");
  hipLaunchKernelGGL(nhwc_to_nchw_kernel, dim3(sdt_grid_1d((long)B * H * W * C, 256)), dim3(256), 0, stream,
                     (const bf16_t*)x, y, B, C, H * W, cpad);
  SDT_LAUNCH_CHECK("sdt_nhwc_bf16_to_nchw_f32");
  return SDT_OK;
}

int sdt_cast_f32_to_bf16(const float* x, uint16_t* y, int64_t n, hipStream_t stream) {
  SDT_CHECK_ARG(x && y && n >= 0, "sdt_cast_f32_to_bf16: bad args");
  if (n == 0) return SDT_OK;
  hipLaunchKernelGGL(cast_f32_bf16_kernel, dim3(sdt_grid_1d(n, 256 * 4)), dim3(256), 0, stream, x, (bf16_t*)y, (long)n);
  SDT_LAUNCH_CHECK("sdt_cast_f32_to_bf16");
  return SDT_OK;
}

int sdt_transpose_bf16(const uint16_t* x, uint16_t* y, int batch, int R, int C, hipStream_t stream) {
  SDT_CHECK_ARG(x && y && batch > 0 && R > 0 && C > 0 && batch < 65536, "sdt_transpose_bf16: bad args");
  hipLaunchKernelGGL(transpose_bf16_kernel, dim3(sdt_ceil_div(C, 64), sdt_ceil_div(R, 64), batch), dim3(256), 0, stream,
                     (const bf16_t*)x, (bf16_t*)y, R, C);
  SDT_LAUNCH_CHECK("sdt_transpose_bf16");
  return SDT_OK;
}

int sdt_param_prepare(const float* master, uint16_t* w_bf16, uint16_t* wt_bf16, const void* descs_device, int ndesc,
                      int total_tiles, hipStream_t stream) {
  SDT_CHECK_ARG(master && w_bf16 && descs_device && ndesc > 0 && total_tiles > 0, "sdt_param_prepare: bad args");
  hipLaunchKernelGGL(param_prepare_kernel, dim3(total_tiles), dim3(256), 0, stream, master, (bf16_t*)w_bf16,
                     (bf16_t*)wt_bf16, (const SdtPrepDesc*)descs_device, ndesc);
  SDT_LAUNCH_CHECK("sdt_param_prepare");
  return SDT_OK;
}

int sdt_zero_ranges_chunk(void) { return ZR_CHUNK; }

int sdt_zero_ranges(float* base, const int64_t* ranges_device, int nranges, hipStream_t stream) {
  SDT_CHECK_ARG(base && ranges_device && nranges > 0 && ((uintptr_t)base & 15) == 0, "sdt_zero_ranges: bad args");
  hipLaunchKernelGGL(zero_ranges_kernel, dim3(nranges), dim3(256), 0, stream, reinterpret_cast<float4*>(base),
                     reinterpret_cast<const long*>(ranges_device));
  SDT_LAUNCH_CHECK("sdt_zero_ranges");
  return SDT_OK;
}

int sdt_param_prepare_desc_size(void) { return (int)sizeof(SdtPrepDesc); }

int sdt_embedding_fwd(const int32_t* ids, const float* tok, const float* pos, uint16_t* out, int64_t rows, int S, int D,
                      hipStream_t stream) {
  SDT_CHECK_ARG(ids && tok && pos && out && rows > 0 && S > 0 && D > 0, "sdt_embedding_fwd: bad args");
  hipLaunchKernelGGL(embedding_fwd_kernel, dim3(sdt_grid_1d(rows * D, 256)), dim3(256), 0, stream, ids, tok, pos,
                     (bf16_t*)out, (long)rows, S, D);
  SDT_LAUNCH_CHECK("sdt_embedding_fwd");
  return SDT_OK;
}

int sdt_embedding_bwd(const int32_t* ids, const uint16_t* dout, float* dtok, float* dpos, int64_t rows, int S, int D,
                      hipStream_t stream) {
  SDT_CHECK_ARG(ids && dout && dtok && dpos && rows > 0 && S > 0 && D > 0, "sdt_embedding_bwd: bad args");
  SDT_CHECK_ARG(rows + S < (1L << 31), "sdt_embedding_bwd: too many rows");
  hipLaunchKernelGGL(embedding_bwd_kernel, dim3((unsigned)(rows + S)), dim3(256), 0, stream, ids,
                     (const bf16_t*)dout, dtok, dpos, (long)rows, S, D);
  SDT_LAUNCH_CHECK("sdt_embedding_bwd");
  return SDT_OK;
}

static inline bool sdt_aligned(const void* p, uintptr_t a) { return p && ((uintptr_t)p & (a - 1)) == 0; }

int sdt_embedding_ext_fwd(const int32_t* ids, const float* tok, const float* ext, const float* pos, uint16_t* out, int64_t rows, int S,
                          int D, int V, int n_ext, hipStream_t stream) {
  SDT_CHECK_ARG(sdt_aligned(ids, 4) && sdt_aligned(tok, 4) && sdt_aligned(ext, 4) && sdt_aligned(pos, 4) && sdt_aligned(out, 2),
                "sdt_embedding_ext_fwd: null or misaligned pointer");
  SDT_CHECK_ARG(rows > 0 && S > 0 && D > 0 && V > 0, "sdt_embedding_ext_fwd: rows=%ld S=%d D=%d V=%d must be positive", (long)rows, S, D, V);
  SDT_CHECK_ARG(n_ext >= 1 && n_ext <= 256, "sdt_embedding_ext_fwd: n_ext=%d outside 1..256", n_ext);
  const bool vec = D % 4 == 0 && sdt_aligned(tok, 16) && sdt_aligned(ext, 16) && sdt_aligned(pos, 16) && sdt_aligned(out, 8);
  if (vec)
    hipLaunchKernelGGL(embedding_ext_fwd_kernel<true>, dim3(sdt_grid_1d(rows * (D / 4), 256)), dim3(256), 0, stream, ids, tok, ext, pos,
                       (bf16_t*)out, (long)rows, S, D, V, n_ext);
  else
    hipLaunchKernelGGL(embedding_ext_fwd_kernel<false>, dim3(sdt_grid_1d(rows * D, 256)), dim3(256), 0, stream, ids, tok, ext, pos,
                       (bf16_t*)out, (long)rows, S, D, V, n_ext);
  SDT_LAUNCH_CHECK("sdt_embedding_ext_fwd");
  return SDT_OK;
}

int sdt_embedding_ext_bwd(const int32_t* ids, const uint16_t* dout, float* dext, int64_t rows, int D, int V, int n_ext,
                          hipStream_t stream) {
  SDT_CHECK_ARG(sdt_aligned(ids, 4) && sdt_aligned(dout, 2) && sdt_aligned(dext, 4), "sdt_embedding_ext_bwd: null or misaligned pointer");
  SDT_CHECK_ARG(rows > 0 && D > 0 && V > 0, "sdt_embedding_ext_bwd: rows=%ld D=%d V=%d must be positive", (long)rows, D, V);
  SDT_CHECK_ARG(n_ext >= 1 && n_ext <= 256, "sdt_embedding_ext_bwd: n_ext=%d outside 1..256", n_ext);
  SDT_CHECK_ARG((D + 255) / 256 <= 65535, "sdt_embedding_ext_bwd: D=%d too wide", D);
  hipLaunchKernelGGL(embedding_ext_bwd_kernel, dim3(n_ext, (D + 255) / 256), dim3(256), 0, stream, ids, (const bf16_t*)dout, dext,
                     (long)rows, D, V);
  SDT_LAUNCH_CHECK("sdt_embedding_ext_bwd");
  return SDT_OK;
}

int sdt_embedding_retract(float* ext, int n_ext, int D, double target_std, double power, double* stats, hipStream_t stream) {
  SDT_CHECK_ARG(sdt_aligned(ext, 4) && sdt_aligned(stats, 8), "sdt_embedding_retract: null or misaligned pointer");
  SDT_CHECK_ARG(D > 0, "sdt_embedding_retract: D=%d must be positive", D);
  SDT_CHECK_ARG(n_ext >= 1 && n_ext <= 256, "sdt_embedding_retract: n_ext=%d outside 1..256", n_ext);
  SDT_CHECK_ARG(target_std > 0.0 && target_std <= 3.4e38 && power == power && power >= -1e6 && power <= 1e6,
                "sdt_embedding_retract: target_std=%g must be finite and > 0, power=%g finite", target_std, power);
  hipLaunchKernelGGL(embedding_retract_kernel, dim3(1), dim3(256), 0, stream, ext, (long)n_ext * D, target_std, power, stats);
  SDT_LAUNCH_CHECK("sdt_embedding_retract");
  return SDT_OK;
}

static int64_t colsum_ws_need(int groups, int nby) { return SDT_WS_COUNTER_BYTES + (int64_t)groups * nby * 256 * (int64_t)sizeof(float); }

int64_t sdt_colsum_workspace_bytes(int batch, int64_t rows_per_batch, int N) {
  if (batch <= 0 || rows_per_batch <= 0 || N <= 0) return 0;
  const int ncb = sdt_ceil_div(sdt_ceil_div(N, 8), 32);
  return colsum_ws_need(ncb * batch, (int)((rows_per_batch + 63) / 64));
}

static int colsum_launch(const uint16_t* dy, float* db, uint16_t* out_bf, int batch, int64_t rows, int N, int ld, int want_blocks,
                         void* workspace, int64_t workspace_bytes, const char* name, hipStream_t stream) {
  const int ncb = sdt_ceil_div(sdt_ceil_div(N, 8), 32);
  int nby = (int)((rows + 63) / 64);
  const int want = (want_blocks + ncb * batch - 1) / (ncb * batch);
  if (nby > want) nby = want;
  const int rpb = (int)((rows + nby - 1) / nby);
  nby = sdt_ceil_div(rows, rpb);
  SDT_CHECK_ARG((int64_t)ncb * batch * (int64_t)sizeof(int) <= SDT_WS_COUNTER_BYTES, "%s: too many column groups", name);
  SDT_CHECK_ARG(workspace && ((uintptr_t)workspace & 15) == 0 && workspace_bytes >= colsum_ws_need(ncb * batch, nby),
                "%s: workspace of sdt_colsum_workspace_bytes() needed", name);
  hipLaunchKernelGGL(colsum_kernel, dim3(ncb, nby, batch), dim3(256), 0, stream, (const bf16_t*)dy, db, (bf16_t*)out_bf, (long)rows, N, ld,
                     rpb, batch > 1 ? (long)rows * ld : 0L, N, reinterpret_cast<int*>(workspace),
                     reinterpret_cast<float*>((unsigned char*)workspace + SDT_WS_COUNTER_BYTES));
  return SDT_OK;
}

int sdt_colsum_accumulate(const uint16_t* dy, float* db, int64_t M, int N, int ld, void* workspace, int64_t workspace_bytes,
                          hipStream_t stream) {
  SDT_CHECK_ARG(dy && db && M >= 0 && N > 0 && ld >= N && ld % 8 == 0 && ((uintptr_t)dy & 15) == 0,
                "sdt_colsum_accumulate: bad args (ld=%d must be a multiple of 8)", ld);
  if (M == 0) return SDT_OK;
  int rc = colsum_launch(dy, db, nullptr, 1, M, N, ld, 256, workspace, workspace_bytes, "sdt_colsum_accumulate", stream);
  if (rc) return rc;
  SDT_LAUNCH_CHECK("sdt_colsum_accumulate");
  return SDT_OK;
}

int sdt_colsum_batched_bf16(const uint16_t* dy, uint16_t* out, int batch, int64_t rows_per_batch, int N, int ld, void* workspace,
                            int64_t workspace_bytes, hipStream_t stream) {
  SDT_CHECK_ARG(dy && out && batch > 0 && batch < 65536 && rows_per_batch > 0 && N > 0 && ld >= N && ld % 8 == 0 &&
                    ((uintptr_t)dy & 15) == 0, "sdt_colsum_batched_bf16: bad args");
  int rc = colsum_launch(dy, nullptr, out, batch, rows_per_batch, N, ld, 512, workspace, workspace_bytes, "sdt_colsum_batched_bf16", stream);
  if (rc) return rc;
  SDT_LAUNCH_CHECK("sdt_colsum_batched_bf16");
  return SDT_OK;
}

int sdt_softmax_rows_inplace(uint16_t* x, int64_t rows, int n, float scale, hipStream_t stream) {
  SDT_CHECK_ARG(x && rows > 0 && n > 0 && rows < 2147483647L, "sdt_softmax_rows_inplace: bad args");
  hipLaunchKernelGGL(softmax_rows_kernel, dim3((unsigned)rows), dim3(256), 0, stream, (bf16_t*)x, n, scale);
  SDT_LAUNCH_CHECK("sdt_softmax_rows_inplace");
  return SDT_OK;
}

int sdt_sum_n_bf16(const uint16_t* const* inputs, int n, uint16_t* out, int64_t numel, hipStream_t stream) {
  SDT_CHECK_ARG(inputs && out && n >= 1 && n <= 32 && numel >= 0 && numel % 8 == 0, "sdt_sum_n_bf16: bad arguments (n=%d numel=%ld)", n, (long)numel);
  SumPtrs sp;
  for (int k = 0; k < n; ++k) {
    SDT_CHECK_ARG(inputs[k] && ((uintptr_t)inputs[k] & 15) == 0, "sdt_sum_n_bf16: input %d null or misaligned", k);
    sp.p[k] = reinterpret_cast<const uint4*>(inputs[k]);
  }
  for (int k = n; k < 32; ++k) sp.p[k] = nullptr;
  if (numel == 0) return SDT_OK;
  hipLaunchKernelGGL(sum_n_kernel, dim3(sdt_grid_1d(numel / 8, 256, 2048)), dim3(256), 0, stream, sp, reinterpret_cast<uint4*>(out), n, numel / 8);
  SDT_LAUNCH_CHECK("sdt_sum_n_bf16");
  return SDT_OK;
}

}
```

stable_diffusion_training_amd/ops.py:

```python
import contextlib
import os

import torch
from torch.autograd import Function

from . import _lib
from ._lib import GATHER_DGRAD, GATHER_FPROP, GATHER_PLAIN, SdtAttnDesc, SdtConvGeom, call

BF16 = torch.bfloat16


def _stream():
    return torch.cuda.current_stream().cuda_stream


def copy_cols(wide, parts, cols, rows, to_wide):
    ld_wide = wide.stride(-2) if wide.dim() > 1 else wide.shape[-1]
    col0 = 0
    for i in range(0, len(parts), 32):
        ps, cs = parts[i: i + 32], cols[i: i + 32]
        n = len(ps)
        ptrs = (_lib.ctypes.c_void_p * n)(*[None if t is None else t.data_ptr() for t in ps])
        lds = (_lib.ctypes.c_int64 * n)(*[c if t is None else t.stride(-2) for t, c in zip(ps, cs)])
        cv = (_lib.ctypes.c_int * n)(*cs)
# ... 84 lines not shown
        e1.record()
        GEMM_NT_TIMER.records.append((e0, e1, 2.0 * M * N * Kc * taps, (M, N, Kc, taps, mode)))
        return
    _gemm_nt(A, Bt, out, M, N, Kc, taps, lda, ldb, b_tap_stride, bias, rowbias, residual, rows_per_batch, mode, geom,
             gn_stats, gn_groups, b_kmajor, b_nseg, b_seg_stride)


_WS_CACHE = {}
_SPLITK_WS = {}


def _splitk_workspace(need, device):
    ws = _SPLITK_WS.get(device)
    if ws is None or ws.numel() < need:
        ws = _SPLITK_WS[device] = torch.zeros(max(need, 32 << 20), dtype=torch.uint8, device=device)
    return ws


def _gemm_nt(A, Bt, out, M, N, Kc, taps, lda, ldb, b_tap_stride, bias, rowbias, residual, rows_per_batch, mode, geom,
             gn_stats=None, gn_groups=0, b_kmajor=False, b_nseg=0, b_seg_stride=0):
    key = (M, N, Kc, taps)
    need = _WS_CACHE.get(key)
    if need is None:
        need = _WS_CACHE[key] = _lib.load().sdt_gemm_nt_workspace_bytes(M, N, Kc, taps)
    ws = _splitk_workspace(need, out.device) if need else None
    call("sdt_gemm_nt_bf16", A.data_ptr(), Bt.data_ptr(), out.data_ptr(), _ptr(bias), _ptr(rowbias), _ptr(residual), M, N,
         Kc, taps, lda, ldb, b_tap_stride, N, N if residual is not None else 0, rows_per_batch, mode,
         None if geom is None else _lib.ctypes.addressof(geom), _ptr(ws), ws.numel() if ws is not None else 0, _ptr(gn_stats),
         gn_groups, int(b_kmajor), b_nseg, b_seg_stride, 0 if rowbias is None else rowbias.stride(0), _stream())


_GN_ARENA = {}
_GN_PARTS = {}


def gn_arena_begin(device, nbytes=1 << 20):
    a = _GN_ARENA.get(device)
    if a is None:
        a = _GN_ARENA[device] = [torch.zeros(nbytes // 4, dtype=torch.float32, device=device), 0, True]
    else:
        a[0].zero_()
    a[1], a[2] = 0, True


def gn_arena_end(device):
    a = _GN_ARENA.get(device)
    if a is not None:
        a[2] = False


def gn_arena_active(device):
    a = _GN_ARENA.get(device)
    return a is not None and a[2]


@contextlib.contextmanager
def gn_arena(device):
    own = not gn_arena_active(device)
    if own:
        gn_arena_begin(device)
    try:
        yield
    finally:
        if own:
            gn_arena_end(device)


def _arena_zeros(n, device):
    a = _GN_ARENA.get(device)
    if a is not None and a[2] and a[1] + n <= a[0].numel():
        out = a[0][a[1]: a[1] + n]
        a[1] += (n + 3) // 4 * 4
        return out
    return torch.zeros(n, dtype=torch.float32, device=device)


def _gn_parts(M, N, Kc, taps, rows_per_batch, groups, mode, geom):
    key = (M, N, Kc, taps, rows_per_batch, groups, mode, None if geom is None else bytes(geom))
    r = _GN_PARTS.get(key)
    if r is None:
        r = _GN_PARTS[key] = int(_lib.load().sdt_gemm_nt_gn_parts(M, N, Kc, taps, rows_per_batch, groups, mode,
                                                                   None if geom is None else _lib.ctypes.addressof(geom)))
    return r


def gemm_tn(A, dY, dW, M, K1, N, K1v, Nv, taps, lda, ldb, *, mode=GATHER_PLAIN, geom=None, dbias=None, n_seg=0, seg_stride=0, sq=None):
    if GEMM_TN_TIMER is not None:
        e0, e1 = torch.cuda.Event(enable_timing=True), torch.cuda.Event(enable_timing=True)
        e0.record()
        _gemm_tn(A, dY, dW, M, K1, N, K1v, Nv, taps, lda, ldb, mode, geom, dbias, n_seg, seg_stride, sq)
        e1.record()
        GEMM_TN_TIMER.records.append((e0, e1, 2.0 * M * K1 * N * taps, (M, K1, N, taps, mode)))
        return
    _gemm_tn(A, dY, dW, M, K1, N, K1v, Nv, taps, lda, ldb, mode, geom, dbias, n_seg, seg_stride, sq)


def sq_begin(store):
    st = getattr(store, "_sq_state", None)
    if st is None:
        want = sum(lf.numel for lf in store.leaves.values() if lf.quantised)
        if not want:
            return
        n = store.quant_total // 512 + (1 << 16)
        st = store._sq_state = dict(buf=torch.zeros(n, dtype=torch.float64, device=store.device), want=want)
    else:
        st["buf"].zero_()
    st.update(next=0, cov=0, on=True)


def sq_end(store):
    st = getattr(store, "_sq_state", None)
    if st is None or not st.get("on"):
        return None
    st["on"] = False
    return (st["buf"], st["next"]) if st["cov"] == st["want"] else None


def _sq_slots(store, paths, K1, N, taps):
    st = getattr(store, "_sq_state", None)
    if st is None or not st.get("on"):
        return None
    leaves = [store.leaves[p] for p in paths if p is not None and p.endswith("/kernel")]
    if not leaves or not all(lf.quantised for lf in leaves):
        return None
    n = int(_lib.load().sdt_wgrad_sq_slots(K1, N, taps))
    if st["next"] + n > st["buf"].numel():
        st["cov"] = -1 << 60
        return None
    ptr = st["buf"].data_ptr() + 8 * st["next"]
    st["next"] += n
    st["cov"] += sum(lf.numel for lf in leaves)
    return ptr


_TN_WS_CACHE = {}
_TN_WS = {}


def _tn_workspace(need, device):
    ws = _TN_WS.get(device)
    if ws is None or ws.numel() < need:
        ws = _TN_WS[device] = torch.zeros(max(need, 64 << 20), dtype=torch.uint8, device=device)
    return ws


WGRAD_GROUP_LIMIT = 32
CONV_GROUP_LIMIT = 8
WGRAD_DUMP = bool(os.environ.get("SDT_WGRAD_DUMP"))
_WGRAD_QUEUE = None
_CONV_QUEUE = []
_NORM_QUEUE = []


class wgrad_grouping:
    def __enter__(self):
        global _WGRAD_QUEUE
        self.prev = _WGRAD_QUEUE
        _WGRAD_QUEUE = []
        return self

    def __exit__(self, *exc):
        global _WGRAD_QUEUE
        try:
            if exc[0] is None:
                flush_wgrads()
        finally:
            _WGRAD_QUEUE = self.prev
            del _NORM_QUEUE[:]
            del _CONV_QUEUE[:]


def flush_norm_grads():
    if not _NORM_QUEUE:
        return
    step = _lib.load().sdt_norm_param_grads_group_max()
    for i in range(0, len(_NORM_QUEUE), step):
        jobs = _NORM_QUEUE[i: i + step]
        arr = (_lib.SdtNormGradJob * len(jobs))(*[j[0] for j in jobs])
        call("sdt_norm_param_grads_group", arr, len(jobs), _stream())
    for job, keep, store, paths in _NORM_QUEUE:
        _ready(store, *paths)
    del _NORM_QUEUE[:]


def flush_conv_wgrads():
    q = _CONV_QUEUE
    if not q:
        return
    lib = _lib.load()
    step = lib.sdt_gemm_tn_wgrad_group_max()
    for i in range(0, len(q), step):
        jobs = q[i: i + step]
        arr = (_lib.SdtConvWgradProblem * len(jobs))(*[j[0] for j in jobs])
        need = lib.sdt_conv_wgrad_group_workspace_bytes(arr, len(jobs))
        ws = _tn_workspace(need, jobs[0][1][0].device) if need else None
        if WGRAD_DUMP:
            print("WGRAD_GROUP conv " + ";".join(f"{j[0].geom.batch},{j[0].geom.out_h},{j[0].geom.out_w},{j[0].K1},{j[0].N},{j[0].geom.kh},{j[0].geom.stride}"
                                               for j in jobs), flush=True)
        e0 = e1 = None
        if GEMM_TN_TIMER is not None:
            e0, e1 = torch.cuda.Event(enable_timing=True), torch.cuda.Event(enable_timing=True)
            e0.record()
        call("sdt_conv_wgrad_group", arr, len(jobs), _ptr(ws), ws.numel() if ws is not None else 0, _stream())
        if e0 is not None:
            e1.record()
            GEMM_TN_TIMER.records.append((e0, e1, sum(j[4] for j in jobs), ("conv group", len(jobs))))
    for prob, keep, store, paths, fl in q:
        _ready(store, *paths)
    del q[:]


def wgrad_conv(x, dy, dW, geom, lf, taps, M_out, *, dbias=None, store=None, paths=()):
    sq = _sq_slots(store, paths, lf.Rp, lf.Cp, taps)
    if _WGRAD_QUEUE is None:
        gemm_tn(x, dy, dW, M_out, lf.Rp, lf.Cp, lf.R, lf.C, taps, lf.Rp, lf.Cp, mode=GATHER_FPROP, geom=geom, dbias=dbias, sq=sq)
        _ready(store, *paths)
        return
    prob = _lib.SdtConvWgradProblem(x.data_ptr(), dy.data_ptr(), dW.data_ptr(), _ptr(dbias), geom, lf.Rp, lf.Cp, lf.R, lf.C, lf.Rp, lf.Cp, sq,
                                    int(dW.dtype == BF16))
    _CONV_QUEUE.append((prob, (x, dy), store, paths, 2.0 * M_out * lf.Rp * lf.Cp * taps))
    if len(_CONV_QUEUE) >= CONV_GROUP_LIMIT:
        flush_conv_wgrads()


def flush_wgrads():
    flush_norm_grads()
    flush_conv_wgrads()
    q = _WGRAD_QUEUE
    if not q:
        return
    lib = _lib.load()
    step = min(len(q), lib.sdt_gemm_tn_wgrad_group_max())
    for i in range(0, len(q), step):
        jobs = q[i: i + step]
        arr = (_lib.SdtTnProblem * len(jobs))(*[j[0] for j in jobs])
        need = lib.sdt_gemm_tn_wgrad_group_workspace_bytes(arr, len(jobs))
        ws = _tn_workspace(need, jobs[0][1][0].device) if need else None
        if WGRAD_DUMP:
            print("WGRAD_GROUP dense " + ";".join(f"{j[0].M},{j[0].K1},{j[0].N},{j[0].lda},{j[0].ldb},{j[0].n_seg}" for j in jobs), flush=True)
        e0 = e1 = None
        if GEMM_TN_TIMER is not None:
            e0, e1 = torch.cuda.Event(enable_timing=True), torch.cuda.Event(enable_timing=True)
            e0.record()
        call("sdt_gemm_tn_wgrad_group", arr, len(jobs), _ptr(ws), ws.numel() if ws is not None else 0, _stream())
        if e0 is not None:
            e1.record()
            GEMM_TN_TIMER.records.append((e0, e1, sum(2.0 * j[0].M * j[0].K1 * j[0].N for j in jobs), ("group", len(jobs))))
    for prob, keep, store, paths in q:
        _ready(store, *paths)
    del q[:]


def wgrad_dense(x, dy, dW, M, K1, N, K1v, Nv, lda, ldb, *, dbias=None, n_seg=0, seg_stride=0, store=None, paths=()):
    sq = _sq_slots(store, paths, K1, N, 1)
    if _WGRAD_QUEUE is None:
        gemm_tn(x, dy, dW, M, K1, N, K1v, Nv, 1, lda, ldb, dbias=dbias, n_seg=n_seg, seg_stride=seg_stride, sq=sq)
        _ready(store, *paths)
        return
    prob = _lib.SdtTnProblem(x.data_ptr(), dy.data_ptr(), dW.data_ptr(), _ptr(dbias), M, K1, N, K1v, Nv, lda, ldb,
                             n_seg if n_seg else Nv, n_seg, seg_stride, sq, int(dW.dtype == BF16))
    _WGRAD_QUEUE.append((prob, (x, dy), store, paths))
    if len(_WGRAD_QUEUE) >= WGRAD_GROUP_LIMIT:
        flush_wgrads()


def _gemm_tn(A, dY, dW, M, K1, N, K1v, Nv, taps, lda, ldb, mode, geom, dbias=None, n_seg=0, seg_stride=0, sq=None):
    ldw = n_seg if n_seg else Nv
    gp = None if geom is None else _lib.ctypes.addressof(geom)
    key = (M, K1, N, taps, n_seg, mode, None if geom is None else bytes(geom))
    need = _TN_WS_CACHE.get(key)
    if need is None:
        need = _TN_WS_CACHE[key] = _lib.load().sdt_gemm_tn_workspace_bytes(M, K1, N, taps, n_seg, mode, gp)
    ws = _tn_workspace(need, dY.device) if need else None
    call("sdt_gemm_tn_wgrad", A.data_ptr(), dY.data_ptr(), dW.data_ptr(), int(dW.dtype == BF16), _ptr(dbias), M, K1, N, K1v, Nv, taps, lda, ldb, ldw,
         K1v * Nv, n_seg, seg_stride, mode, gp, _ptr(ws), ws.numel() if ws is not None else 0, sq, _stream())


def reduce_workspace(need, device):
    return _splitk_workspace(max(int(need), 1), device)


def colsum(dy, db, M, N, ld):
    need = _lib.load().sdt_colsum_workspace_bytes(1, M, N)
    ws = reduce_workspace(need, dy.device)
    call("sdt_colsum_accumulate", dy.data_ptr(), db.data_ptr(), M, N, ld, ws.data_ptr(), ws.numel(), _stream())


def _wgrad_dest(store, wpaths):
    if store.trainable:
        return store.grad_view, True, store
    ad = getattr(store, "adapter", None)
    if ad is not None and ad.takes(wpaths):
        return ad.scratch_view, False, None
    return None


def _leaf_grad(view, lf):
    return view(lf.offset, lf.offset + lf.numel).view(lf.shape)


class _Linear(Function):

    @staticmethod
    def forward(ctx, x, residual, store, wpath, bpath, gn_groups):
        _check(x, "linear input")
        W, lf = store.wmat(wpath)
        K = x.shape[-1]
        if K != lf.Rp:
            raise _lib.SdtError(f"{wpath}: input width {K} != padded in-features {lf.Rp}")
        M = x.numel() // K
        y = torch.empty(*x.shape[:-1], lf.Cp, dtype=BF16, device=x.device)
        if residual is not None:
            _check(residual, "linear residual")
        stats, rpb = None, 0
        if gn_groups and x.dim() == 3:
            rpb = x.shape[1]
            nparts = _gn_parts(M, lf.Cp, lf.Rp, 1, rpb, gn_groups, GATHER_PLAIN, None)
            if nparts:
                stats = torch.empty(x.shape[0], nparts, gn_groups, 2, dtype=torch.float32, device=x.device)
        gemm_nt(x, W, y, M, lf.Cp, lf.Rp, 1, lf.Rp, lf.Cp, 0, bias=_padded_bias(store, bpath, lf.Cp), residual=residual,
                rows_per_batch=rpb if stats is not None else 0, gn_stats=stats, gn_groups=gn_groups if stats is not None else 0,
                b_kmajor=True)
        ctx.save_for_backward(x)
        ctx.meta = (store, wpath, bpath, residual is not None)
        if gn_groups:
            ctx.set_materialize_grads(False)
            if stats is not None:
                ctx.mark_non_differentiable(stats)
            return y, stats
        return y

    @staticmethod
    def backward(ctx, dy, dstats=None):
        if dy is None:
            return None, None, None, None, None, None
        (x,) = ctx.saved_tensors
        store, wpath, bpath, has_res = ctx.meta
        dy = dy.contiguous()
        W, lf = store.wmat(wpath)
        M = x.numel() // lf.Rp
        dx = None
        if ctx.needs_input_grad[0]:
            dx = torch.empty_like(x)
            gemm_nt(dy, W, dx, M, lf.Rp, lf.Cp, 1, lf.Cp, lf.Cp, 0)
        dest = _wgrad_dest(store, (wpath,))
        if dest is not None:
            view, with_bias, book = dest
            wgrad_dense(x, dy, _leaf_grad(view, lf), M, lf.Rp, lf.Cp, lf.R, lf.C, lf.Rp, lf.Cp,
                        dbias=store.g(bpath) if (bpath is not None and with_bias) else None, store=book,
                        paths=(wpath, bpath) if book is not None else ())
        return dx, (dy if has_res else None), None, None, None, None


def linear(x, store, name, residual=None, gn_groups=0):
    bpath = name + "/bias" if store.has(name + "/bias") else None
    return _Linear.apply(x, residual, store, name + "/kernel", bpath, gn_groups)


class _LinearMulti(Function):

    @staticmethod
    def forward(ctx, x, store, wpaths, bpaths):
        _check(x, "linear_multi input")
        lfs = [store.leaves[w] for w in wpaths]
        lf, n = lfs[0], len(lfs)
        K, N = lf.Rp, lf.Cp
        if x.shape[-1] != K:
            raise _lib.SdtError(f"{wpaths[0]}: input width {x.shape[-1]} != in-features {K}")
        M = x.numel() // K
        Wn = store.w[lf.w_off: lf.w_off + n * K * N]
        bias = None
        if bpaths is not None:
            b0 = store.leaves[bpaths[0]]
            bias = store.master[b0.offset: b0.offset + n * N]
        y = torch.empty(*x.shape[:-1], n * N, dtype=BF16, device=x.device)
        gemm_nt(x, Wn, y, M, n * N, K, 1, K, N, 0, bias=bias, b_kmajor=True, b_nseg=N, b_seg_stride=K * N)
        ctx.save_for_backward(x)
        ctx.meta = (store, wpaths, bpaths)
        return y

    @staticmethod
    def backward(ctx, dy):
        (x,) = ctx.saved_tensors
        store, wpaths, bpaths = ctx.meta
        dy = dy.contiguous()
        lfs = [store.leaves[w] for w in wpaths]
        lf, n = lfs[0], len(lfs)
        K, N = lf.Rp, lf.Cp
        M = x.numel() // K
        dx = None
        if ctx.needs_input_grad[0]:
            dx = torch.empty_like(x)
            W = store.w[lf.w_off: lf.w_off + n * K * N]
            gemm_nt(dy, W, dx, M, K, N, n, n * N, N, K * N)
        dest = _wgrad_dest(store, wpaths)
        if dest is not None:
            view, with_bias, book = dest
            g0 = view(lf.offset, lf.offset + n * K * N)
            db = None
            if bpaths is not None and with_bias:
                b0 = store.leaves[bpaths[0]]
                db = store.grad_view(b0.offset, b0.offset + n * N)
            wgrad_dense(x, dy, g0, M, K, n * N, K, n * N, K, n * N, dbias=db, n_seg=N, seg_stride=lfs[1].offset - lf.offset,
                        store=book, paths=(tuple(wpaths) + tuple(bpaths or ())) if book is not None else ())
        return dx, None, None, None


def linear_multi(x, store, names):
    wpaths = tuple(n + "/kernel" for n in names)
    has_b = [store.has(n + "/bias") for n in names]
    if any(has_b) and not all(has_b):
        return None
    bpaths = tuple(n + "/bias" for n in names) if all(has_b) else None
    if not store.mergeable(wpaths, bpaths):
        return None
    return _LinearMulti.apply(x, store, wpaths, bpaths)


class _Conv2d(Function):

    @staticmethod
    def forward(ctx, x, rowbias, residual, store, wpath, bpath, stride, pad, gn_groups):
        _check(x, "conv input")
        W, lf = store.wmat(wpath)
        B, H, Wd, C = x.shape
        kh, kw = store.leaves[wpath].shape[:2]
        if C != lf.Rp:
            raise _lib.SdtError(f"{wpath}: input channels {C} != padded in-channels {lf.Rp}")
        (pt, pb), (pl, pr) = pad
        OH = (H + pt + pb - kh) // stride + 1
        OW = (Wd + pl + pr - kw) // stride + 1
        geom = SdtConvGeom(B, H, Wd, OH, OW, kh, kw, stride, pt, pl)
        plain = kh == 1 and kw == 1 and stride == 1 and pt == 0 and pl == 0
        y = torch.empty(B, OH, OW, lf.Cp, dtype=BF16, device=x.device)
        M = B * OH * OW
        mode = GATHER_PLAIN if plain else GATHER_FPROP
        stats = None
        nparts = _gn_parts(M, lf.Cp, lf.Rp, kh * kw, OH * OW, gn_groups, mode, None if plain else geom) if gn_groups else 0
        if nparts:
            stats = torch.empty(B, nparts, gn_groups, 2, dtype=torch.float32, device=x.device)
        gemm_nt(x, W, y, M, lf.Cp, lf.Rp, kh * kw, lf.Rp, lf.Cp, lf.Rp * lf.Cp, bias=_padded_bias(store, bpath, lf.Cp),
                rowbias=rowbias, residual=residual, rows_per_batch=OH * OW, mode=mode, geom=None if plain else geom,
                gn_stats=stats, gn_groups=gn_groups if stats is not None else 0, b_kmajor=True)
        ctx.save_for_backward(x)
        ctx.meta = (store, wpath, bpath, geom, plain, rowbias is not None, residual is not None)
        if gn_groups:
            ctx.set_materialize_grads(False)
            if stats is not None:
                ctx.mark_non_differentiable(stats)
            return y, stats
        return y

    @staticmethod
    def backward(ctx, dy, dstats=None):
        if dy is None:
            return None, None, None, None, None, None, None, None, None
        (x,) = ctx.saved_tensors
        store, wpath, bpath, geom, plain, has_rb, has_res = ctx.meta
        dy = dy.contiguous()
        W, lf = store.wmat(wpath)
        B, H, Wd, C = x.shape
        taps = geom.kh * geom.kw
        M_out = B * geom.out_h * geom.out_w
        dx = None
        if ctx.needs_input_grad[0]:
            dx = torch.empty_like(x)
            gemm_nt(dy, W, dx, B * H * Wd, lf.Rp, lf.Cp, taps, lf.Cp, lf.Cp, lf.Rp * lf.Cp,
                    mode=GATHER_PLAIN if plain else GATHER_DGRAD, geom=None if plain else geom)
        dest = _wgrad_dest(store, (wpath,))
        if dest is not None:
            view, with_bias, book = dest
            dW = _leaf_grad(view, lf)
            db = store.g(bpath) if (bpath is not None and with_bias) else None
            paths = (wpath, bpath) if book is not None else ()
            if plain:
                wgrad_dense(x, dy, dW, M_out, lf.Rp, lf.Cp, lf.R, lf.C, lf.Rp, lf.Cp, dbias=db, store=book, paths=paths)
            else:
                wgrad_conv(x, dy, dW, geom, lf, taps, M_out, dbias=db, store=book, paths=paths)
        drb = None
        if has_rb:
            drb = torch.empty(B, lf.Cp, dtype=BF16, device=x.device)
            ws = reduce_workspace(_lib.load().sdt_colsum_workspace_bytes(B, geom.out_h * geom.out_w, lf.Cp), x.device)
            call("sdt_colsum_batched_bf16", dy.data_ptr(), drb.data_ptr(), B, geom.out_h * geom.out_w, lf.Cp, lf.Cp, ws.data_ptr(),
                 ws.numel(), _stream())
        return dx, drb, (dy if has_res else None), None, None, None, None, None, None


def conv2d(x, store, name, stride=1, pad=1, rowbias=None, residual=None, gn_groups=0):
    if isinstance(pad, int):
        pad = ((pad, pad), (pad, pad))
    bpath = name + "/bias" if store.has(name + "/bias") else None
    return _Conv2d.apply(x, rowbias, residual, store, name + "/kernel", bpath, stride, pad, gn_groups)


class _GroupNorm(Function):
    @staticmethod
    def forward(ctx, x, store, name, groups, eps, silu, skip, parts):
        _check(x, "groupnorm input")
        B, C = x.shape[0], x.shape[-1]
        HW = x.numel() // (B * C)
        y = torch.empty_like(x)
        stats = torch.empty(B, groups, 2, dtype=torch.float32, device=x.device)
        nparts = 0
        need = _lib.load().sdt_groupnorm_fwd_workspace_bytes(B, HW, C, groups)
        ws = torch.empty(need, dtype=torch.uint8, device=x.device)
        if parts is not None:
            if parts.dim() != 4 or parts.shape[0] != B or tuple(parts.shape[2:]) != (groups, 2) or not parts.is_contiguous():
                raise _lib.SdtError(f"{name}: producer statistics have shape {tuple(parts.shape)}, expected {(B, 'nparts', groups, 2)}")
            nparts = parts.shape[1]
        call("sdt_groupnorm_fwd", x.data_ptr(), store.p(name + "/scale").data_ptr(), store.p(name + "/bias").data_ptr(),
             y.data_ptr(), stats.data_ptr(), B, HW, C, groups, eps, int(silu), _ptr(parts), nparts, _ptr(ws), need, _stream())
        ctx.save_for_backward(x, stats)
        ctx.meta = (store, name, groups, eps, silu)
        ctx.set_materialize_grads(False)
        return (y, x) if skip else y

    @staticmethod
    def backward(ctx, dy, dskip=None):
        x, stats = ctx.saved_tensors
        store, name, groups, eps, silu = ctx.meta
        dy = dy.contiguous()
        if dskip is not None:
            dskip = dskip.contiguous()
        B, C = x.shape[0], x.shape[-1]
        HW = x.numel() // (B * C)
        dx = torch.empty_like(x)
        dg = store.g(name + "/scale").data_ptr() if store.trainable else None
        db = store.g(name + "/bias").data_ptr() if store.trainable else None
        need = _lib.load().sdt_groupnorm_bwd_workspace_bytes(B, HW, C)
        ws = torch.empty(need, dtype=torch.uint8, device=x.device)
        call("sdt_groupnorm_bwd", x.data_ptr(), dy.data_ptr(), stats.data_ptr(), store.p(name + "/scale").data_ptr(),
             store.p(name + "/bias").data_ptr(), dx.data_ptr(), dg, db, _ptr(dskip), B, HW, C, groups, eps,
             int(silu), ws.data_ptr(), need, _stream())
        if store.trainable:
            _ready(store, name + "/scale", name + "/bias")
        return dx, None, None, None, None, None, None, None


def group_norm(x, store, name, groups=32, eps=1e-5, silu=False, skip=False, stats=None):
    return _GroupNorm.apply(x, store, name, groups, eps, silu, skip, stats)


class _LayerNorm(Function):
    @staticmethod
    def forward(ctx, x, store, name, eps, skip):
        _check(x, "layernorm input")
        C = x.shape[-1]
        M = x.numel() // C
        y = torch.empty_like(x)
        mr = torch.empty(M, 2, dtype=torch.float32, device=x.device)
        call("sdt_layernorm_fwd", x.data_ptr(), store.p(name + "/scale").data_ptr(), store.p(name + "/bias").data_ptr(),
             y.data_ptr(), mr.data_ptr(), M, C, eps, _stream())
        ctx.save_for_backward(x, mr)
        ctx.meta = (store, name)
        ctx.set_materialize_grads(False)
        return (y, x) if skip else y

    @staticmethod
    def backward(ctx, dy, dskip=None):
        x, mr = ctx.saved_tensors
        store, name = ctx.meta
        dy = dy.contiguous()
        if dskip is not None:
            dskip = dskip.contiguous()
        C = x.shape[-1]
        M = x.numel() // C
        dx = torch.empty_like(x)
        dg = store.g(name + "/scale").data_ptr() if store.trainable else None
        db = store.g(name + "/bias").data_ptr() if store.trainable else None
        need = _lib.load().sdt_layernorm_bwd_workspace_bytes(M, C) if store.trainable else 0
        ws = torch.empty(need, dtype=torch.uint8, device=x.device) if need else None
        defer = store.trainable and _WGRAD_QUEUE is not None
        call("sdt_layernorm_bwd", x.data_ptr(), dy.data_ptr(), store.p(name + "/scale").data_ptr(), mr.data_ptr(),
             dx.data_ptr(), dg, db, _ptr(dskip), M, C, int(defer), _ptr(ws), need, _stream())
        if defer:
            job = _lib.SdtNormGradJob(ws.data_ptr(), dg, db, int(_lib.load().sdt_layernorm_bwd_partial_rows(M, C)), C)
            _NORM_QUEUE.append((job, ws, store, (name + "/scale", name + "/bias")))
        elif store.trainable:
            _ready(store, name + "/scale", name + "/bias")
        return dx, None, None, None, None


def layer_norm(x, store, name, eps=1e-5, skip=False):
    return _LayerNorm.apply(x, store, name, eps, skip)


class _ClipPool(Function):

    @staticmethod
    def forward(ctx, x, ids, store, name, eos_id, eps, windows):
        _check(x, "clip_pool input")
        rows, S, D = x.shape
        if ids.dtype != torch.int32 or not ids.is_contiguous() or tuple(ids.shape) != (rows, S):
            raise _lib.SdtError(f"clip_pool: ids must be contiguous int32 {(rows, S)}, got {ids.dtype} {tuple(ids.shape)}")
        if rows % windows:
            raise _lib.SdtError(f"clip_pool: {rows} rows are not a whole number of {windows}-window samples")
        R = rows // windows
        pooled = torch.empty(R, D, dtype=BF16, device=x.device)
        mr = torch.empty(R, 2, dtype=torch.float32, device=x.device)
        pos = torch.empty(R, dtype=torch.int32, device=x.device)
        call("sdt_clip_pool_fwd", ids.data_ptr(), x.data_ptr(), store.p(name + "/scale").data_ptr(), store.p(name + "/bias").data_ptr(),
             pooled.data_ptr(), mr.data_ptr(), pos.data_ptr(), R, windows, S, D, int(eos_id), float(eps), _stream())
        ctx.save_for_backward(x, mr, pos)
        ctx.meta = (store, name, R, windows)
        ctx.mark_non_differentiable(pos)
        ctx.set_materialize_grads(False)
        return pooled, pos

    @staticmethod
    def backward(ctx, dpooled, dpos=None):
        x, mr, pos = ctx.saved_tensors
        store, name, R, windows = ctx.meta
        if dpooled is None:
            return None, None, None, None, None, None, None
        dpooled = dpooled.contiguous()
        _, S, D = x.shape
        dx = torch.empty_like(x)
        dg = store.g(name + "/scale").data_ptr() if store.trainable else None
        db = store.g(name + "/bias").data_ptr() if store.trainable else None
        call("sdt_clip_pool_bwd", x.data_ptr(), dpooled.data_ptr(), store.p(name + "/scale").data_ptr(), mr.data_ptr(), pos.data_ptr(),
             dx.data_ptr(), dg, db, R, windows, S, D, _stream())
        if store.trainable:
            _ready(store, name + "/scale", name + "/bias")
        return dx, None, None, None, None, None, None


def clip_pool(x, ids, store, name, eos_id, eps=1e-5, windows=1):
    return _ClipPool.apply(x, ids, store, name, eos_id, eps, windows)


class _Fanout(Function):

    @staticmethod
    def forward(ctx, x, n):
        ctx.set_materialize_grads(False)
        return tuple(x.view_as(x) for _ in range(n))

    @staticmethod
    def backward(ctx, *grads):
        gs = [g.contiguous() for g in grads if g is not None]
        if not gs:
            return None, None
        if len(gs) == 1:
            return gs[0], None
        out = torch.empty_like(gs[0])
        for i in range(0, len(gs), 31):
            chunk = ([out] if i else []) + gs[i:i + 31]
            arr = (_lib.ctypes.c_void_p * len(chunk))(*[t.data_ptr() for t in chunk])
            call("sdt_sum_n_bf16", arr, len(chunk), out.data_ptr(), out.numel(), _stream())
        return out, None


class _ColSlices(Function):

    @staticmethod
    def forward(ctx, y, n):
        ctx.set_materialize_grads(False)
        ctx.n = n
        C = y.shape[-1] // n
        return tuple(y[..., i * C: (i + 1) * C] for i in range(n))

    @staticmethod
    def backward(ctx, *grads):
        n = ctx.n
        g0 = next((g for g in grads if g is not None), None)
        if g0 is None:
            return None, None
        C = g0.shape[-1]
        rows = g0.numel() // C
        dy = torch.empty(*g0.shape[:-1], n * C, dtype=BF16, device=g0.device)
        copy_cols(dy.view(rows, n * C), [None if g is None else g.contiguous().view(rows, C) for g in grads], [C] * n, rows, True)
        return dy, None


def col_slices(y, n):
    return _ColSlices.apply(y, n)


def fanout(x, n):
    if n <= 1 or not (torch.is_grad_enabled() and x.requires_grad):
        return (x,) * max(n, 1)
    _check(x, "fanout input")
    return _Fanout.apply(x, n)


class _Act(Function):
    @staticmethod
    def forward(ctx, x, act):
        _check(x, "activation input")
        y = torch.empty_like(x)
        call("sdt_act_fwd", x.data_ptr(), y.data_ptr(), x.numel(), act, _stream())
        ctx.save_for_backward(x)
        ctx.act = act
        return y

    @staticmethod
    def backward(ctx, dy):
        (x,) = ctx.saved_tensors
        dy = dy.contiguous()
        dx = torch.empty_like(x)
        call("sdt_act_bwd", x.data_ptr(), dy.data_ptr(), dx.data_ptr(), x.numel(), ctx.act, _stream())
        return dx, None


def silu(x):
    return _Act.apply(x, _lib.ACT_SILU)


def quick_gelu(x):
    return _Act.apply(x, _lib.ACT_QUICK_GELU)


def gelu_erf(x):
    return _Act.apply(x, _lib.ACT_GELU_ERF)


class _Geglu(Function):
    @staticmethod
    def forward(ctx, h):
        _check(h, "geglu input")
        F2 = h.shape[-1]
        M = h.numel() // F2
        out = torch.empty(*h.shape[:-1], F2 // 2, dtype=BF16, device=h.device)
        call("sdt_geglu_fwd", h.data_ptr(), out.data_ptr(), M, F2 // 2, _stream())
        ctx.save_for_backward(h)
        return out

    @staticmethod
    def backward(ctx, dout):
        (h,) = ctx.saved_tensors
        dout = dout.contiguous()
        F2 = h.shape[-1]
        dh = torch.empty_like(h)
        call("sdt_geglu_bwd", h.data_ptr(), dout.data_ptr(), dh.data_ptr(), h.numel() // F2, F2 // 2, _stream())
        return dh


def geglu(h):
    return _Geglu.apply(h)


class _FeedForwardGeglu(Function):

    @staticmethod
    def forward(ctx, x, residual, store, n1, n2):
        _check(x, "feed-forward input")
        W1, l1 = store.wmat(n1 + "/kernel")
        W2, l2 = store.wmat(n2 + "/kernel")
        K, F = l1.Rp, l1.Cp // 2
        M = x.numel() // K
        h = torch.empty(*x.shape[:-1], 2 * F, dtype=BF16, device=x.device)
        f = torch.empty(*x.shape[:-1], F, dtype=BF16, device=x.device)
        b1 = _ptr(_padded_bias(store, n1 + "/bias" if store.has(n1 + "/bias") else None, l1.Cp))
        if GEMM_NT_TIMER is not None:
            e0, e1 = torch.cuda.Event(enable_timing=True), torch.cuda.Event(enable_timing=True)
            e0.record()
            call("sdt_ff_geglu_fwd", x.data_ptr(), W1.data_ptr(), b1, h.data_ptr(), f.data_ptr(), M, F, K, _stream())
            e1.record()
            GEMM_NT_TIMER.records.append((e0, e1, 2.0 * M * 2 * F * K, (M, 2 * F, K, 1, "ff1+geglu")))
        else:
            call("sdt_ff_geglu_fwd", x.data_ptr(), W1.data_ptr(), b1, h.data_ptr(), f.data_ptr(), M, F, K, _stream())
        y = torch.empty(*x.shape[:-1], l2.Cp, dtype=BF16, device=x.device)
        if residual is not None:
            _check(residual, "feed-forward residual")
        gemm_nt(f, W2, y, M, l2.Cp, l2.Rp, 1, l2.Rp, l2.Cp, 0, bias=_padded_bias(store, n2 + "/bias" if store.has(n2 + "/bias") else None, l2.Cp),
                residual=residual, b_kmajor=True)
        ctx.save_for_backward(x, h, f)
        ctx.meta = (store, n1, n2, residual is not None)
        return y

    @staticmethod
    def backward(ctx, dy):
        x, h, f = ctx.saved_tensors
        store, n1, n2, has_res = ctx.meta
        dy = dy.contiguous()
        W1, l1 = store.wmat(n1 + "/kernel")
        W2, l2 = store.wmat(n2 + "/kernel")
        K, F = l1.Rp, l1.Cp // 2
        M = x.numel() // K
        df = torch.empty_like(f)
        gemm_nt(dy, W2, df, M, l2.Rp, l2.Cp, 1, l2.Cp, l2.Cp, 0)
        dh = torch.empty_like(h)
        call("sdt_geglu_bwd", h.data_ptr(), df.data_ptr(), dh.data_ptr(), M, F, _stream())
        dest = _wgrad_dest(store, (n2 + "/kernel",))
        if dest is not None:
            view, with_bias, book = dest
            b2 = n2 + "/bias" if (with_bias and store.has(n2 + "/bias")) else None
            wgrad_dense(f, dy, _leaf_grad(view, l2), M, l2.Rp, l2.Cp, l2.R, l2.C, l2.Rp, l2.Cp,
                        dbias=store.g(b2) if b2 is not None else None, store=book, paths=(n2 + "/kernel", b2) if book is not None else ())
        dx = None
        if ctx.needs_input_grad[0]:
            dx = torch.empty_like(x)
            gemm_nt(dh, W1, dx, M, l1.Rp, l1.Cp, 1, l1.Cp, l1.Cp, 0)
        dest = _wgrad_dest(store, (n1 + "/kernel",))
        if dest is not None:
            view, with_bias, book = dest
            b1 = n1 + "/bias" if (with_bias and store.has(n1 + "/bias")) else None
            wgrad_dense(x, dh, _leaf_grad(view, l1), M, l1.Rp, l1.Cp, l1.R, l1.C, l1.Rp, l1.Cp,
                        dbias=store.g(b1) if b1 is not None else None, store=book, paths=(n1 + "/kernel", b1) if book is not None else ())
        return dx, (dy if has_res else None), None, None, None


def feed_forward_geglu(x, store, n1, n2, residual=None):
    l1, l2 = store.leaves[n1 + "/kernel"], store.leaves[n2 + "/kernel"]
    K, F = l1.Rp, l1.Cp // 2
    M = x.numel() // K
    if (l1.batch == 1 and l2.batch == 1 and l1.Cp == l1.C and l2.Rp == F and l2.Cp == K and x.shape[-1] == K
            and _lib.load().sdt_ff_geglu_supported(M, F, K)):
        return _FeedForwardGeglu.apply(x, residual, store, n1, n2)
    return linear(geglu(linear(x, store, n1)), store, n2, residual=residual)


class _Upsample2x(Function):
    @staticmethod
    def forward(ctx, x):
        _check(x, "upsample input")
        B, H, W, C = x.shape
        y = torch.empty(B, 2 * H, 2 * W, C, dtype=BF16, device=x.device)
        call("sdt_upsample2x_fwd", x.data_ptr(), y.data_ptr(), B, H, W, C, _stream())
        ctx.shape = (B, H, W, C)
        return y

    @staticmethod
    def backward(ctx, dy):
        B, H, W, C = ctx.shape
        dy = dy.contiguous()
        dx = torch.empty(B, H, W, C, dtype=BF16, device=dy.device)
        call("sdt_upsample2x_bwd", dy.data_ptr(), dx.data_ptr(), B, H, W, C, _stream())
        return dx
# ... 18 lines not shown
    @staticmethod
    def backward(ctx, dy):
        sa, sb = ctx.meta
        dy = dy.contiguous()
        Ca, Cb = sa[-1], sb[-1]
        rows = dy.numel() // (Ca + Cb)
        da = torch.empty(sa, dtype=BF16, device=dy.device)
        db = torch.empty(sb, dtype=BF16, device=dy.device)
        copy_cols(dy.view(rows, Ca + Cb), [da.view(rows, Ca), db.view(rows, Cb)], [Ca, Cb], rows, False)
        return da, db


def concat_channels(a, b):
    return _ConcatChannels.apply(a, b)


class _ControlAdd(Function):

    @staticmethod
    def forward(ctx, a, skip, res, scale):
        _check(skip, "control_add skip")
        _check(res, "control_add res")
        if skip.shape != res.shape:
            raise _lib.SdtError(f"control_add: skip {tuple(skip.shape)} and res {tuple(res.shape)} differ")
        if skip.dim() < 2 or skip.numel() == 0:
            raise _lib.SdtError(f"control_add: skip {tuple(skip.shape)} must be a non-empty (B, ..., C) tensor")
        Cb = skip.shape[-1]
        rows = skip.numel() // Cb
        Ca = 0
        if a is not None:
            _check(a, "control_add a")
            Ca = a.shape[-1]
            if a.shape[:-1] != skip.shape[:-1]:
                raise _lib.SdtError(f"control_add: a {tuple(a.shape)} and skip {tuple(skip.shape)} differ in their rows")
        if scale is not None and (scale.dtype != torch.float32 or not scale.is_contiguous() or tuple(scale.shape) != (skip.shape[0],)
                                  or scale.device != skip.device):
            raise _lib.SdtError(f"control_add: scale must be a contiguous float32 ({skip.shape[0]},) tensor on {skip.device}, got "
                                f"{scale.dtype} {tuple(scale.shape)} on {scale.device}")
        if res.device != skip.device or (a is not None and a.device != skip.device):
            raise _lib.SdtError("control_add: a, skip and res must live on one device")
        y = torch.empty(*skip.shape[:-1], Ca + Cb, dtype=BF16, device=skip.device)
        call("sdt_control_concat_add", _ptr(a), skip.data_ptr(), res.data_ptr(), _ptr(scale), y.data_ptr(), rows,
             rows // skip.shape[0], Ca, Cb, _stream())
        ctx.meta = (None if a is None else a.shape, skip.shape)
        return y

    @staticmethod
    def backward(ctx, dy):
        sa, sb = ctx.meta
        need_skip, need_res = ctx.needs_input_grad[1], ctx.needs_input_grad[2]
        if sa is None:
            return None, (dy if need_skip else None), (dy if need_res else None), None
        dy = dy.contiguous()
        Ca, Cb = sa[-1], sb[-1]
        rows = dy.numel() // (Ca + Cb)
        da = torch.empty(sa, dtype=BF16, device=dy.device)
        db = torch.empty(sb, dtype=BF16, device=dy.device)
        copy_cols(dy.view(rows, Ca + Cb), [da.view(rows, Ca), db.view(rows, Cb)], [Ca, Cb], rows, False)
        return da, (db if need_skip else None), (db if need_res else None), None


def control_add(a, skip, res, scale=None):
    if scale is not None and res.requires_grad:
        raise ValueError("control_add: a scale is for sampling only - res requires grad, and training runs at unit scale")
    return _ControlAdd.apply(a, skip, res, scale)


class _Add(Function):
    @staticmethod
    def forward(ctx, a, b):
        _check(a, "add a")
        _check(b, "add b")
        y = torch.empty_like(a)
        call("sdt_add_bf16", a.data_ptr(), b.data_ptr(), y.data_ptr(), a.numel(), _stream())
        return y

    @staticmethod
    def backward(ctx, dy):
        return dy, dy


def add(a, b):
    return _Add.apply(a, b)


class _Attention(Function):

    @staticmethod
    def forward(ctx, q, k, v, heads, scale, causal, key_weight=None):
        for t, n in ((q, "q"), (k, "k"), (v, "v")):
            _check(t, n)
        B, Nq, C = q.shape
        Nk = k.shape[1]
        D = C // heads
        desc = SdtAttnDesc(B, heads, Nq, Nk, D, C, k.shape[2], v.shape[2], C, scale, int(causal), 0, 0, 0, 0, _kw_ptr(key_weight, Nk))
        ctx.key_weight = key_weight
        out = torch.empty_like(q)
        lse = torch.empty(B, heads, Nq, dtype=torch.float32, device=q.device)
        call("sdt_attention_fwd", q.data_ptr(), k.data_ptr(), v.data_ptr(), out.data_ptr(), lse.data_ptr(),
             _lib.ctypes.addressof(desc), _stream())
        ctx.save_for_backward(q, k, v, out, lse)
        ctx.desc = desc
        return out

    @staticmethod
    def backward(ctx, dout):
        q, k, v, out, lse = ctx.saved_tensors
        dout = dout.contiguous()
        dq, dk, dv = torch.empty_like(q), torch.empty_like(k), torch.empty_like(v)
        need = _lib.load().sdt_attention_bwd_workspace_bytes(_lib.ctypes.addressof(ctx.desc))
        ws = torch.empty(need, dtype=torch.uint8, device=q.device)
        call("sdt_attention_bwd", q.data_ptr(), k.data_ptr(), v.data_ptr(), out.data_ptr(), dout.data_ptr(), lse.data_ptr(),
             dq.data_ptr(), dk.data_ptr(), dv.data_ptr(), ws.data_ptr(), need, _lib.ctypes.addressof(ctx.desc), _stream())
        return dq, dk, dv, None, None, None, None


def _kw_ptr(key_weight, Nk):
    if key_weight is None:
        return None
    if key_weight.dtype != torch.float32 or not key_weight.is_contiguous() or key_weight.numel() != Nk:
        raise ValueError(f"key_weight must be a contiguous float32 array of {Nk} elements")
    return key_weight.data_ptr()


def attention(q, k, v, heads, scale, causal=False, key_weight=None):
    return _Attention.apply(q, k, v, heads, scale, causal, key_weight)


class _AttentionPacked(Function):

    @staticmethod
    def forward(ctx, a, b, heads, scale, causal, key_weight=None):
        _check(a, "attention q")
        B, Nq = a.shape[0], a.shape[1]
        if b is None:
            C = a.shape[2] // 3
            q, k, v, Nk, ldq, ldkv = a.data_ptr(), a.data_ptr() + 2 * C, a.data_ptr() + 4 * C, Nq, 3 * C, 3 * C
        else:
            C = a.shape[2]
            Nk = b.shape[1]
            if (b.dtype != BF16 or not b.is_cuda or b.shape[2] != 2 * C or b.stride(2) != 1 or b.stride(1) % 8 or b.stride(1) < 2 * C
                    or (B > 1 and b.stride(0) != Nk * b.stride(1))):
                raise _lib.SdtError(f"attention kv: expected bf16 (B, Nk, 2C) rows at a constant pitch, got {b.dtype} {tuple(b.shape)} strides {b.stride()}")
            q, k, v, ldq, ldkv = a.data_ptr(), b.data_ptr(), b.data_ptr() + 2 * C, C, b.stride(1)
        D = C // heads
        ldg = ldkv if b is None else 2 * C
        desc = SdtAttnDesc(B, heads, Nq, Nk, D, ldq, ldkv, ldkv, C, scale, int(causal), ldq, ldg, ldg, 0, _kw_ptr(key_weight, Nk))
        ctx.key_weight = key_weight
        out = torch.empty(B, Nq, C, dtype=BF16, device=a.device)
        lse = torch.empty(B, heads, Nq, dtype=torch.float32, device=a.device)
        call("sdt_attention_fwd", q, k, v, out.data_ptr(), lse.data_ptr(), _lib.ctypes.addressof(desc), _stream())
        ctx.save_for_backward(a, b, out, lse)
        ctx.desc, ctx.C = desc, C
        return out

    @staticmethod
    def backward(ctx, dout):
        a, b, out, lse = ctx.saved_tensors
        C = ctx.C
        dout = dout.contiguous()
        da = torch.empty_like(a)
        db = None if b is None else torch.empty(b.shape, dtype=BF16, device=b.device)
        if b is None:
            q, k, v = a.data_ptr(), a.data_ptr() + 2 * C, a.data_ptr() + 4 * C
            dq, dk, dv = da.data_ptr(), da.data_ptr() + 2 * C, da.data_ptr() + 4 * C
        else:
            q, k, v = a.data_ptr(), b.data_ptr(), b.data_ptr() + 2 * C
            dq, dk, dv = da.data_ptr(), db.data_ptr(), db.data_ptr() + 2 * C
        need = _lib.load().sdt_attention_bwd_workspace_bytes(_lib.ctypes.addressof(ctx.desc))
        ws = torch.empty(need, dtype=torch.uint8, device=a.device)
        call("sdt_attention_bwd", q, k, v, out.data_ptr(), dout.data_ptr(), lse.data_ptr(), dq, dk, dv, ws.data_ptr(), need,
             _lib.ctypes.addressof(ctx.desc), _stream())
        return da, db, None, None, None, None


def attention_packed(a, b, heads, scale, causal=False, key_weight=None):
    return _AttentionPacked.apply(a, b, heads, scale, causal, key_weight)


def _kv_pitch(b, B, C, what):
    if (b.dim() != 3 or b.dtype != BF16 or not b.is_cuda or b.shape[0] != B or b.shape[2] != 2 * C or b.stride(2) != 1 or b.stride(1) % 8
            or b.stride(1) < 2 * C or (B > 1 and b.stride(0) != b.shape[1] * b.stride(1))):
        raise _lib.SdtError(f"{what}: expected bf16 ({B}, N, {2 * C}) rows at a constant pitch, got {b.dtype} {tuple(b.shape)} strides {b.stride()}")
    return b.stride(1)


class _AttentionIP(Function):

    @staticmethod
    def forward(ctx, q, kv_txt, kv_ip, heads, scale, key_weight, scale_ip):
        _check(q, "attention_ip q")
        if q.dim() != 3 or q.shape[2] % heads:
            raise _lib.SdtError(f"attention_ip: q {tuple(q.shape)} must be (B, Nq, heads * D) with heads = {heads}")
        B, Nq, C = q.shape
        ld_txt = _kv_pitch(kv_txt, B, C, "attention_ip kv_txt")
        ld_ip = _kv_pitch(kv_ip, B, C, "attention_ip kv_ip")
        Nk, T, D = kv_txt.shape[1], kv_ip.shape[1], C // heads
        if scale_ip is not None and (scale_ip.dtype != torch.float32 or not scale_ip.is_contiguous() or tuple(scale_ip.shape) != (B,)
                                     or scale_ip.device != q.device):
            raise _lib.SdtError(f"attention_ip: scale_ip must be a contiguous float32 ({B},) tensor on {q.device}, got {scale_ip.dtype} "
                                f"{tuple(scale_ip.shape)} on {scale_ip.device}")
        desc = SdtAttnDesc(B, heads, Nq, Nk, D, C, ld_txt, ld_txt, C, scale, 0, C, 2 * C, 2 * C, 0, _kw_ptr(key_weight, Nk))
        ctx.key_weight = key_weight
        o_txt = torch.empty(B, Nq, C, dtype=BF16, device=q.device)
        lse = torch.empty(B, heads, Nq, dtype=torch.float32, device=q.device)
        call("sdt_attention_fwd", q.data_ptr(), kv_txt.data_ptr(), kv_txt.data_ptr() + 2 * C, o_txt.data_ptr(), lse.data_ptr(),
             _lib.ctypes.addressof(desc), _stream())
        out = torch.empty_like(o_txt)
        call("sdt_ip_attention_fwd", q.data_ptr(), kv_ip.data_ptr(), o_txt.data_ptr(), _ptr(scale_ip), out.data_ptr(), B, heads, Nq, T, D,
             C, ld_ip, scale, _stream())
        ctx.save_for_backward(q, kv_txt, kv_ip, o_txt, lse, scale_ip)
        ctx.desc, ctx.dims = desc, (B, heads, Nq, T, D, C, ld_ip, scale)
        return out

    @staticmethod
    def backward(ctx, dout):
        q, kv_txt, kv_ip, o_txt, lse, scale_ip = ctx.saved_tensors
        B, heads, Nq, T, D, C, ld_ip, scale = ctx.dims
        dout = dout.contiguous()
        dq_txt = torch.empty_like(q)
        dkv_txt = torch.empty(kv_txt.shape, dtype=BF16, device=q.device)
        need = _lib.load().sdt_attention_bwd_workspace_bytes(_lib.ctypes.addressof(ctx.desc))
        ws = torch.empty(need, dtype=torch.uint8, device=q.device)
        call("sdt_attention_bwd", q.data_ptr(), kv_txt.data_ptr(), kv_txt.data_ptr() + 2 * C, o_txt.data_ptr(), dout.data_ptr(),
             lse.data_ptr(), dq_txt.data_ptr(), dkv_txt.data_ptr(), dkv_txt.data_ptr() + 2 * C, ws.data_ptr(), need,
             _lib.ctypes.addressof(ctx.desc), _stream())
        dq = torch.empty_like(q)
        dkv_ip = torch.empty(B, T, 2 * C, dtype=BF16, device=q.device)
        need = _lib.load().sdt_ip_attention_bwd_workspace_bytes(B, heads, Nq, T, D)
        ws = torch.empty(need, dtype=torch.uint8, device=q.device)
        call("sdt_ip_attention_bwd", q.data_ptr(), kv_ip.data_ptr(), dout.data_ptr(), _ptr(scale_ip), dq_txt.data_ptr(), dq.data_ptr(),
             dkv_ip.data_ptr(), B, heads, Nq, T, D, C, ld_ip, 2 * C, scale, ws.data_ptr(), need, _stream())
        return dq, dkv_txt, dkv_ip, None, None, None, None


def attention_ip(q, kv_txt, kv_ip, heads, scale, key_weight=None, scale_ip=None):
    if scale_ip is not None and kv_ip.requires_grad:
        raise ValueError("attention_ip: a scale_ip is for sampling only - kv_ip requires grad, and training runs at unit scale")
    return _AttentionIP.apply(q, kv_txt, kv_ip, heads, scale, key_weight, scale_ip)


class _Embedding(Function):
    @staticmethod
    def forward(ctx, anchor, ids, store, tok_path, pos_path, S):
        tok, pos = store.p(tok_path), store.p(pos_path)
        D = tok.shape[1]
        rows = ids.numel()
        out = torch.empty(*ids.shape, D, dtype=BF16, device=ids.device)
        tk = getattr(store, "tokens", None)
        if tk is not None:
            ext = tk.rows(tok_path)
            call("sdt_embedding_ext_fwd", ids.data_ptr(), tok.data_ptr(), ext.data_ptr(), pos.data_ptr(), out.data_ptr(), rows, S, D,
                 tok.shape[0], ext.shape[0], _stream())
        else:
            call("sdt_embedding_fwd", ids.data_ptr(), tok.data_ptr(), pos.data_ptr(), out.data_ptr(), rows, S, D, _stream())
        ctx.save_for_backward(ids)
        ctx.meta = (store, tok_path, pos_path, S, D)
        return out

    @staticmethod
    def backward(ctx, dout):
        (ids,) = ctx.saved_tensors
        store, tok_path, pos_path, S, D = ctx.meta
        tk = getattr(store, "tokens", None)
        if tk is not None:
            dout = dout.contiguous()
            call("sdt_embedding_ext_bwd", ids.data_ptr(), dout.data_ptr(), tk.grad(tok_path).data_ptr(), ids.numel(), D,
                 store.leaves[tok_path].shape[0], tk.num_tokens, _stream())
            _ready(tk.store, tk.new_paths[tok_path])
        elif store.trainable:
            dout = dout.contiguous()
            call("sdt_embedding_bwd", ids.data_ptr(), dout.data_ptr(), store.g(tok_path).data_ptr(),
                 store.g(pos_path).data_ptr(), ids.numel(), S, D, _stream())
            _ready(store, tok_path, pos_path)
        return None, None, None, None, None, None


def embedding(ids, store, tok_path, pos_path, S, anchor):
    return _Embedding.apply(anchor, ids, store, tok_path, pos_path, S)
```

Baseline: 102.0 images/sec.

## Defer cross-attention dK/dV and row-bias colsums into grouped off-chain launches

Cross-attention backward is split into an immediate dQ kernel and a deferred dK/dV pass. The dK/dV jobs from many layers are queued and run as one grouped kernel once the shared text-embedding slice gradient is needed, and conv row-bias column sums are batched the same way. This takes many small, under-filled launches off the critical backward chain and packs them into fewer, fuller grids. In exchange it adds a tagging mechanism to detect slices with a second consumer, keeps extra buffers alive until the flush, and only activates when an offchain flag is set in the wgrad grouping context.

Measured after the change: 103.3 images/sec (median of 6 runs). +1.3%, better.

```diff
diff --git a/include/sdt.h b/include/sdt.h
--- a/include/sdt.h
+++ b/include/sdt.h
@@ -217,6 +217,16 @@
 int sdt_colsum_batched_bf16(const uint16_t* dy, uint16_t* out, int batch, int64_t rows_per_batch, int N, int ld, void* workspace,
                             int64_t workspace_bytes, hipStream_t stream);
 int64_t sdt_colsum_workspace_bytes(int batch, int64_t rows_per_batch, int N);
+typedef struct SdtColsumProblem {
+  const uint16_t* dy;
+  uint16_t* out;
+  int batch;
+  int64_t rows_per_batch;
+  int N, ld;
+} SdtColsumProblem;
+int sdt_colsum_batched_group(const SdtColsumProblem* problems, int n, void* workspace, int64_t workspace_bytes, hipStream_t stream);
+int sdt_colsum_batched_group_max(void);
+int64_t sdt_colsum_batched_group_workspace_bytes(const SdtColsumProblem* problems, int n);
 
 int sdt_attention_fwd(const uint16_t* q, const uint16_t* k, const uint16_t* v, uint16_t* out, float* lse,
                       const SdtAttnDesc* desc, hipStream_t stream);
@@ -224,6 +234,19 @@
                       const float* lse, uint16_t* dq, uint16_t* dk, uint16_t* dv, float* workspace, int64_t workspace_bytes,
                       const SdtAttnDesc* desc, hipStream_t stream);
 int64_t sdt_attention_bwd_workspace_bytes(const SdtAttnDesc* desc);
+typedef struct SdtAttnDkvProblem {
+  const uint16_t *q, *k, *v, *dout;
+  const float *lse, *delta;
+  uint16_t *dk, *dv;
+  float* slabs;
+  SdtAttnDesc desc;
+} SdtAttnDkvProblem;
+int sdt_attention_bwd_dq(const uint16_t* q, const uint16_t* k, const uint16_t* v, const uint16_t* out, const uint16_t* dout,
+                         const float* lse, uint16_t* dq, float* delta, const SdtAttnDesc* desc, hipStream_t stream);
+int sdt_attention_bwd_dkv_group(const SdtAttnDkvProblem* problems, int n, hipStream_t stream);
+int sdt_attention_bwd_dkv_group_max(void);
+int64_t sdt_attention_bwd_delta_bytes(const SdtAttnDesc* desc);
+int64_t sdt_attention_bwd_slab_bytes(const SdtAttnDesc* desc);
 int sdt_softmax_rows_inplace(uint16_t* x, int64_t rows, int n, float scale, hipStream_t stream);
 
 int sdt_act_fwd(const uint16_t* x, uint16_t* y, int64_t n, int act, hipStream_t stream);
diff --git a/stable_diffusion_training_amd/_lib.py b/stable_diffusion_training_amd/_lib.py
--- a/stable_diffusion_training_amd/_lib.py
+++ b/stable_diffusion_training_amd/_lib.py
@@ -25,6 +25,15 @@
 
 class SdtNormGradJob(ctypes.Structure):
     _fields_ = [("partial", _P), ("dgamma", _P), ("dbeta", _P), ("nrows", _I), ("C", _I)]
+
+
+class SdtAttnDkvProblem(ctypes.Structure):
+    _fields_ = [("q", _P), ("k", _P), ("v", _P), ("dout", _P), ("lse", _P), ("delta", _P), ("dk", _P), ("dv", _P), ("slabs", _P),
+                ("desc", SdtAttnDesc)]
+
+
+class SdtColsumProblem(ctypes.Structure):
+    _fields_ = [("dy", _P), ("out", _P), ("batch", _I), ("rows_per_batch", _L), ("N", _I), ("ld", _I)]
 
 
 class SdtConvWgradProblem(ctypes.Structure):
@@ -115,8 +124,11 @@
     "sdt_zero_ranges": [_P, _P, _I, _P],
     "sdt_colsum_accumulate": [_P, _P, _L, _I, _I, _P, _L, _P],
     "sdt_colsum_batched_bf16": [_P, _P, _I, _L, _I, _I, _P, _L, _P],
+    "sdt_colsum_batched_group": [_P, _I, _P, _L, _P],
     "sdt_attention_fwd": [_P, _P, _P, _P, _P, _P, _P],
     "sdt_attention_bwd": [_P, _P, _P, _P, _P, _P, _P, _P, _P, _P, _L, _P, _P],
+    "sdt_attention_bwd_dq": [_P, _P, _P, _P, _P, _P, _P, _P, _P, _P],
+    "sdt_attention_bwd_dkv_group": [_P, _I, _P],
     "sdt_softmax_rows_inplace": [_P, _L, _I, _F, _P],
     "sdt_act_fwd": [_P, _P, _L, _I, _P],
     "sdt_act_bwd": [_P, _P, _P, _L, _I, _P],
@@ -153,12 +165,13 @@
 WS_QUERY = {"sdt_gemm_nt_workspace_bytes": [_L, _I, _I, _I], "sdt_gemm_tn_workspace_bytes": [_L, _I, _I, _I, _I, _I, _P], "sdt_layernorm_bwd_workspace_bytes": [_L, _I], "sdt_layernorm_bwd_partial_rows": [_L, _I],
             "sdt_groupnorm_bwd_workspace_bytes": [_I, _I, _I],
             "sdt_groupnorm_fwd_workspace_bytes": [_I, _I, _I, _I], "sdt_attention_bwd_workspace_bytes": [_P],
+            "sdt_attention_bwd_delta_bytes": [_P], "sdt_attention_bwd_slab_bytes": [_P], "sdt_colsum_batched_group_workspace_bytes": [_P, _I],
             "sdt_ip_attention_bwd_workspace_bytes": [_I, _I, _I, _I, _I],
             "sdt_gemm_tn_wgrad_group_workspace_bytes": [_P, _I], "sdt_conv_wgrad_group_workspace_bytes": [_P, _I], "sdt_reduce_workspace_bytes": [], "sdt_dpo_loss_workspace_bytes": [_I, _I, _I], "sdt_sqnorm_workspace_bytes": [], "sdt_prodigy_workspace_bytes": [], "sdt_colsum_workspace_bytes": [_I, _L, _I],
             "sdt_lora_project_split_workspace_bytes": [_P, _I],
             "sdt_loha_project_workspace_bytes": [_P, _I],
             "sdt_wgrad_sq_slots": [_I, _I, _I]}
-NOARG = {"sdt_abi_version": _I, "sdt_gemm_tn_wgrad_group_max": _I, "sdt_norm_param_grads_group_max": _I, "sdt_zero_ranges_chunk": _I, "sdt_device_count": _I, "sdt_param_prepare_desc_size": _I, "sdt_lora_job_size": _I, "sdt_dora_job_size": _I, "sdt_lora_split_job_size": _I, "sdt_lora_project_split_rows": _I, "sdt_loha_job_size": _I, "sdt_last_error": ctypes.c_char_p}
+NOARG = {"sdt_abi_version": _I, "sdt_gemm_tn_wgrad_group_max": _I, "sdt_norm_param_grads_group_max": _I, "sdt_attention_bwd_dkv_group_max": _I, "sdt_colsum_batched_group_max": _I, "sdt_zero_ranges_chunk": _I, "sdt_device_count": _I, "sdt_param_prepare_desc_size": _I, "sdt_lora_job_size": _I, "sdt_dora_job_size": _I, "sdt_lora_split_job_size": _I, "sdt_lora_project_split_rows": _I, "sdt_loha_job_size": _I, "sdt_last_error": ctypes.c_char_p}
 
 LIB_PATH = os.path.join(os.path.dirname(os.path.abspath(__file__)), "csrc", "libsdtrain_hip.so")
 if os.environ.get("SDT_LIB"):
diff --git a/stable_diffusion_training_amd/csrc/attention.hip b/stable_diffusion_training_amd/csrc/attention.hip
--- a/stable_diffusion_training_amd/csrc/attention.hip
+++ b/stable_diffusion_training_amd/csrc/attention.hip
@@ -417,14 +417,12 @@
 }
 
 template <int DPP, int NS, int NB, bool QSPLIT>
-__global__ void __launch_bounds__(256) attn_bwd_dkv_kernel(const AttnParams p) {
-  extern __shared__ __attribute__((aligned(16))) unsigned char smem[];
+__device__ __forceinline__ void attn_bwd_dkv_body(const AttnParams& p, const int bx, const int h, const int b, unsigned char* smem) {
   using I = Img<DPP>;
   constexpr int STAGE = 2 * I::BYTES + 2 * KT * 4;
   const int lane = threadIdx.x & 63, wave = threadIdx.x >> 6, fr = lane & 31, fh = lane >> 5;
   const int wave_u = __builtin_amdgcn_readfirstlane(wave);
-  const int b = blockIdx.z, h = blockIdx.y;
-  const int kblk = QSPLIT ? (int)blockIdx.x % p.kblocks : (int)blockIdx.x;
+  const int kblk = QSPLIT ? bx % p.kblocks : bx;
   const int k0 = kblk * 128;
   const int ki = k0 + wave * 32 + fr;
   const float kwt = p.key_w ? p.key_w[min(ki, p.Nk - 1)] : 1.f;
@@ -443,7 +441,7 @@
   int qstart = 0, qend = p.Nq;
   if (p.causal) qstart = (k0 / KT) * KT;
   if (QSPLIT) {
-    qstart = ((int)blockIdx.x / p.kblocks) * p.qchunk;
+    qstart = (bx / p.kblocks) * p.qchunk;
     qend = min(p.Nq, qstart + p.qchunk);
   }
   dma.bind(qb, p.ldq, qstart);
@@ -538,7 +536,7 @@
     if (ki < p.Nk) {
       const long C = (long)p.H * p.D;
       const long slab = 2 * (long)p.B * p.Nk * C;
-      float* wk = p.kv_ws + ((int)blockIdx.x / p.kblocks) * slab + ((long)b * p.Nk + ki) * C + h * p.D;
+      float* wk = p.kv_ws + (bx / p.kblocks) * slab + ((long)b * p.Nk + ki) * C + h * p.D;
       float* wv = wk + (long)p.B * p.Nk * C;
 #pragma unroll
       for (int i = 0; i < NB; ++i)
@@ -575,11 +573,48 @@
   }
 }
 
-__global__ void __launch_bounds__(256) attn_kv_finish_kernel(const AttnParams p, int nsplit) {
+template <int DPP, int NS, int NB, bool QSPLIT>
+__global__ void __launch_bounds__(256) attn_bwd_dkv_kernel(const AttnParams p) {
+  extern __shared__ __attribute__((aligned(16))) unsigned char smem[];
+  attn_bwd_dkv_body<DPP, NS, NB, QSPLIT>(p, (int)blockIdx.x, (int)blockIdx.y, (int)blockIdx.z, smem);
+}
+
+#define ATTN_GROUP_MAX 8
+#define ATTN_DKV_GROUP_ABI_MAX 32
+struct AttnGroupParams {
+  int n;
+  int wg_end[ATTN_GROUP_MAX];
+  int gx[ATTN_GROUP_MAX];
+  AttnParams prob[ATTN_GROUP_MAX];
+};
+static_assert(sizeof(AttnGroupParams) <= 4096, "the grouped attention launches pass their problem table as kernel arguments");
+
+__device__ __forceinline__ int attn_group_find(const AttnGroupParams& gp, int* local) {
+  const int blk = blockIdx.x;
+  int i = 0;
+  while (i + 1 < gp.n && blk >= gp.wg_end[i]) ++i;
+  *local = blk - (i ? gp.wg_end[i - 1] : 0);
+  return i;
+}
+
+template <int DPP, int NS, int NB>
+__global__ void __launch_bounds__(256) attn_bwd_dkv_group_kernel(const AttnGroupParams gp) {
+  extern __shared__ __attribute__((aligned(16))) unsigned char smem[];
+  int local;
+  const int i = attn_group_find(gp, &local);
+  const AttnParams p = gp.prob[i];
+  const int gx = gp.gx[i];
+  const int rest = local / gx, bx = local - rest * gx;
+  const int b = rest / p.H, h = rest - b * p.H;
+  if (p.kv_ws) attn_bwd_dkv_body<DPP, NS, NB, true>(p, bx, h, b, smem);
+  else attn_bwd_dkv_body<DPP, NS, NB, false>(p, bx, h, b, smem);
+}
+
+__device__ __forceinline__ void attn_kv_finish_body(const AttnParams& p, const int nsplit, const int bid, const int nblocks) {
   const int C = p.H * p.D, cv = C >> 3;
   const long rows = (long)p.B * p.Nk, total = rows * cv;
   const long slab = 2 * rows * C;
-  for (long i = (long)blockIdx.x * blockDim.x + threadIdx.x; i < total; i += (long)gridDim.x * blockDim.x) {
+  for (long i = (long)bid * blockDim.x + threadIdx.x; i < total; i += (long)nblocks * blockDim.x) {
     const long r = i / cv;
     const int c = (int)(i - r * cv) * 8;
     const int b = (int)(r / p.Nk), ki = (int)(r - (long)b * p.Nk);
@@ -598,6 +633,15 @@
     *reinterpret_cast<uint4*>(p.dv + (long)b * p.bsdv + (long)ki * p.lddv + c) = pack8(fv);
   }
 }
+__global__ void __launch_bounds__(256) attn_kv_finish_kernel(const AttnParams p, int nsplit) {
+  attn_kv_finish_body(p, nsplit, (int)blockIdx.x, (int)gridDim.x);
+}
+__global__ void __launch_bounds__(256) attn_kv_finish_group_kernel(const AttnGroupParams gp) {
+  int local;
+  const int i = attn_group_find(gp, &local);
+  const AttnParams p = gp.prob[i];
+  attn_kv_finish_body(p, gp.gx[i], local, gp.wg_end[i] - (i ? gp.wg_end[i - 1] : 0));
+}
 
 static int attn_qsplits(int B, int H, int Nq, int Nk, int causal) {
   if (causal) return 1;
@@ -608,6 +652,13 @@
   if (s > max_s) s = max_s;
   return s < 2 ? 1 : s;
 }
+static int attn_split_plan(AttnParams* p) {
+  const int splits = attn_qsplits(p->B, p->H, p->Nq, p->Nk, p->causal);
+  p->kblocks = sdt_ceil_div(p->Nk, 128);
+  p->qchunk = sdt_ceil_div(sdt_ceil_div(p->Nq, splits), KT) * KT;
+  return sdt_ceil_div(p->Nq, p->qchunk);
+}
+static int attn_finish_blocks(const AttnParams& p) { return sdt_grid_1d((long)p.B * p.Nk * p.H * p.D / 8, 256, 1024); }
 
 static int attn_fill(AttnParams* p, const SdtAttnDesc* d, const char* name) {
   SDT_CHECK_ARG(d, "%s: null descriptor", name);
@@ -651,7 +702,7 @@
   }
 }
 template <int DPP, int NS, int NB>
-static void launch_bwd(const AttnParams& p, hipStream_t stream) {
+static void launch_bwd(const AttnParams& p, bool with_dkv, hipStream_t stream) {
   static_assert(NB * 32 <= DPP && NS * 16 <= DPP, "image pitch too small");
   static bool set_q = false, set_kv = false;
   const size_t lds_dq = (size_t)2 * 2 * Img<DPP>::BYTES;
@@ -659,19 +710,60 @@
   static bool set_kvs = false;
   ensure_lds(attn_bwd_dq_kernel<DPP, NS, NB>, lds_dq, &set_q);
   hipLaunchKernelGGL((attn_bwd_dq_kernel<DPP, NS, NB>), dim3(sdt_ceil_div(p.Nq, 128), p.H, p.B), dim3(256), lds_dq, stream, p);
+  if (!with_dkv) return;
   if (p.kv_ws) {
     AttnParams ps = p;
-    const int splits = attn_qsplits(p.B, p.H, p.Nq, p.Nk, p.causal);
-    ps.kblocks = sdt_ceil_div(p.Nk, 128);
-    ps.qchunk = sdt_ceil_div(sdt_ceil_div(p.Nq, splits), KT) * KT;
-    const int nsplit = sdt_ceil_div(p.Nq, ps.qchunk);
+    const int nsplit = attn_split_plan(&ps);
     ensure_lds(attn_bwd_dkv_kernel<DPP, NS, NB, true>, lds_dkv, &set_kvs);
     hipLaunchKernelGGL((attn_bwd_dkv_kernel<DPP, NS, NB, true>), dim3(ps.kblocks * nsplit, p.H, p.B), dim3(256), lds_dkv, stream, ps);
-    hipLaunchKernelGGL(attn_kv_finish_kernel, dim3(sdt_grid_1d((long)p.B * p.Nk * p.H * p.D / 8, 256, 1024)), dim3(256), 0, stream, ps, nsplit);
+    hipLaunchKernelGGL(attn_kv_finish_kernel, dim3(attn_finish_blocks(p)), dim3(256), 0, stream, ps, nsplit);
   } else {
     ensure_lds(attn_bwd_dkv_kernel<DPP, NS, NB, false>, lds_dkv, &set_kv);
     hipLaunchKernelGGL((attn_bwd_dkv_kernel<DPP, NS, NB, false>), dim3(sdt_ceil_div(p.Nk, 128), p.H, p.B), dim3(256), lds_dkv, stream, p);
   }
+}
+template <int DPP, int NS, int NB>
+static void launch_dkv_group(const AttnGroupParams& gp, hipStream_t stream) {
+  static bool set_g = false;
+  const size_t lds_dkv = (size_t)2 * (2 * Img<DPP>::BYTES + 2 * KT * sizeof(float));
+  ensure_lds(attn_bwd_dkv_group_kernel<DPP, NS, NB>, lds_dkv, &set_g);
+  hipLaunchKernelGGL((attn_bwd_dkv_group_kernel<DPP, NS, NB>), dim3(gp.wg_end[gp.n - 1]), dim3(256), lds_dkv, stream, gp);
+}
+
+static int attn_class(int D) { return D <= 48 ? 0 : D <= 64 ? 1 : D <= 80 ? 2 : D <= 96 ? 3 : D <= 128 ? 4 : 5; }
+static void attn_bwd_dispatch(const AttnParams& p, bool with_dkv, hipStream_t stream) {
+  switch (attn_class(p.D)) {
+    case 0: launch_bwd<64, 3, 2>(p, with_dkv, stream); break;
+    case 1: launch_bwd<64, 4, 2>(p, with_dkv, stream); break;
+    case 2: launch_bwd<128, 5, 3>(p, with_dkv, stream); break;
+    case 3: launch_bwd<128, 6, 3>(p, with_dkv, stream); break;
+    case 4: launch_bwd<128, 8, 4>(p, with_dkv, stream); break;
+    default: launch_bwd<256, 10, 5>(p, with_dkv, stream); break;
+  }
+}
+static void attn_dkv_group_dispatch(int cls, const AttnGroupParams& gp, hipStream_t stream) {
+  switch (cls) {
+    case 0: launch_dkv_group<64, 3, 2>(gp, stream); break;
+    case 1: launch_dkv_group<64, 4, 2>(gp, stream); break;
+    case 2: launch_dkv_group<128, 5, 3>(gp, stream); break;
+    case 3: launch_dkv_group<128, 6, 3>(gp, stream); break;
+    case 4: launch_dkv_group<128, 8, 4>(gp, stream); break;
+    default: launch_dkv_group<256, 10, 5>(gp, stream); break;
+  }
+}
+static int attn_fill_bwd(AttnParams* p, const SdtAttnDesc* desc, const char* name, const uint16_t* q, const uint16_t* k, const uint16_t* v,
+                         const uint16_t* out, const uint16_t* dout, const float* lse, const float* delta, uint16_t* dq, uint16_t* dk,
+                         uint16_t* dv) {
+  int rc = attn_fill(p, desc, name);
+  if (rc) return rc;
+  p->q = (const bf16_t*)q; p->k = (const bf16_t*)k; p->v = (const bf16_t*)v; p->o = (const bf16_t*)out;
+  p->dout = (const bf16_t*)dout; p->lse = const_cast<float*>(lse); p->delta = delta;
+  p->dq = (bf16_t*)dq; p->dk = (bf16_t*)dk; p->dv = (bf16_t*)dv;
+  if (desc->ldgrad_q) { p->lddq = desc->ldgrad_q; p->bsdq = (long)p->Nq * p->lddq; }
+  if (desc->ldgrad_k) { p->lddk = desc->ldgrad_k; p->bsdk = (long)p->Nk * p->lddk; }
+  if (desc->ldgrad_v) { p->lddv = desc->ldgrad_v; p->bsdv = (long)p->Nk * p->lddv; }
+  if (desc->ld_dout) { p->lddo = desc->ld_dout; p->bsdo = (long)p->Nq * p->lddo; }
+  return SDT_OK;
 }
 
 extern "C" {
@@ -697,11 +789,16 @@
 
 int64_t sdt_attention_bwd_workspace_bytes(const SdtAttnDesc* d) {
   if (!d || d->B <= 0 || d->H <= 0 || d->Nq <= 0 || d->Nk <= 0 || d->D <= 0) return 0;
-  int64_t n = (int64_t)d->B * d->H * d->Nq;
-  n = (n + 3) / 4 * 4;
+  return sdt_attention_bwd_delta_bytes(d) + sdt_attention_bwd_slab_bytes(d);
+}
+int64_t sdt_attention_bwd_delta_bytes(const SdtAttnDesc* d) {
+  if (!d || d->B <= 0 || d->H <= 0 || d->Nq <= 0 || d->Nk <= 0 || d->D <= 0) return 0;
+  return ((int64_t)d->B * d->H * d->Nq + 3) / 4 * 4 * (int64_t)sizeof(float);
+}
+int64_t sdt_attention_bwd_slab_bytes(const SdtAttnDesc* d) {
+  if (!d || d->B <= 0 || d->H <= 0 || d->Nq <= 0 || d->Nk <= 0 || d->D <= 0) return 0;
   const int qs = attn_qsplits(d->B, d->H, d->Nq, d->Nk, d->causal);
-  if (qs > 1) n += (int64_t)qs * 2 * d->B * d->Nk * d->H * d->D;
-  return n * (int64_t)sizeof(float);
+  return qs > 1 ? (int64_t)qs * 2 * d->B * d->Nk * d->H * d->D * (int64_t)sizeof(float) : 0;
 }
 
 int sdt_attention_bwd(const uint16_t* q, const uint16_t* k, const uint16_t* v, const uint16_t* out, const uint16_t* dout,
@@ -710,26 +807,86 @@
   SDT_CHECK_ARG(q && k && v && out && dout && lse && dq && dk && dv && delta_ws, "sdt_attention_bwd: null pointer");
   SDT_CHECK_ARG(desc && workspace_bytes >= (int64_t)sizeof(float) * desc->B * desc->H * desc->Nq, "sdt_attention_bwd: workspace too small");
   AttnParams p = {};
-  int rc = attn_fill(&p, desc, "sdt_attention_bwd");
+  int rc = attn_fill_bwd(&p, desc, "sdt_attention_bwd", q, k, v, out, dout, lse, delta_ws, dq, dk, dv);
   if (rc) return rc;
-  p.q = (const bf16_t*)q; p.k = (const bf16_t*)k; p.v = (const bf16_t*)v; p.o = (const bf16_t*)out;
-  p.dout = (const bf16_t*)dout; p.lse = const_cast<float*>(lse); p.delta = delta_ws;
-  p.dq = (bf16_t*)dq; p.dk = (bf16_t*)dk; p.dv = (bf16_t*)dv;
-  if (desc->ldgrad_q) { p.lddq = desc->ldgrad_q; p.bsdq = (long)p.Nq * p.lddq; }
-  if (desc->ldgrad_k) { p.lddk = desc->ldgrad_k; p.bsdk = (long)p.Nk * p.lddk; }
-  if (desc->ldgrad_v) { p.lddv = desc->ldgrad_v; p.bsdv = (long)p.Nk * p.lddv; }
-  if (desc->ld_dout) { p.lddo = desc->ld_dout; p.bsdo = (long)p.Nq * p.lddo; }
   if (attn_qsplits(p.B, p.H, p.Nq, p.Nk, p.causal) > 1 && workspace_bytes >= sdt_attention_bwd_workspace_bytes(desc))
     p.kv_ws = delta_ws + ((long)p.B * p.H * p.Nq + 3) / 4 * 4;
-  const int D = p.D;
-  if (D <= 48) launch_bwd<64, 3, 2>(p, stream);
-  else if (D <= 64) launch_bwd<64, 4, 2>(p, stream);
-  else if (D <= 80) launch_bwd<128, 5, 3>(p, stream);
-  else if (D <= 96) launch_bwd<128, 6, 3>(p, stream);
-  else if (D <= 128) launch_bwd<128, 8, 4>(p, stream);
-  else launch_bwd<256, 10, 5>(p, stream);
+  attn_bwd_dispatch(p, true, stream);
   SDT_LAUNCH_CHECK("sdt_attention_bwd");
   return SDT_OK;
 }
 
-}
+int sdt_attention_bwd_dq(const uint16_t* q, const uint16_t* k, const uint16_t* v, const uint16_t* out, const uint16_t* dout,
+                         const float* lse, uint16_t* dq, float* delta, const SdtAttnDesc* desc, hipStream_t stream) {
+  SDT_CHECK_ARG(q && k && v && out && dout && lse && dq && delta && desc, "sdt_attention_bwd_dq: null pointer");
+  AttnParams p = {};
+  int rc = attn_fill_bwd(&p, desc, "sdt_attention_bwd_dq", q, k, v, out, dout, lse, delta, dq, nullptr, nullptr);
+  if (rc) return rc;
+  attn_bwd_dispatch(p, false, stream);
+  SDT_LAUNCH_CHECK("sdt_attention_bwd_dq");
+  return SDT_OK;
+}
+
+int sdt_attention_bwd_dkv_group_max(void) { return ATTN_DKV_GROUP_ABI_MAX; }
+
+int sdt_attention_bwd_dkv_group(const SdtAttnDkvProblem* problems, int n, hipStream_t stream) {
+  SDT_CHECK_ARG(problems && n > 0 && n <= ATTN_DKV_GROUP_ABI_MAX, "sdt_attention_bwd_dkv_group: 1..%d problems", ATTN_DKV_GROUP_ABI_MAX);
+  static thread_local AttnParams ps[ATTN_DKV_GROUP_ABI_MAX];
+  static thread_local int nsplit[ATTN_DKV_GROUP_ABI_MAX], gxs[ATTN_DKV_GROUP_ABI_MAX];
+  long all_wgs = 0;
+  for (int i = 0; i < n; ++i) {
+    const SdtAttnDkvProblem& q = problems[i];
+    SDT_CHECK_ARG(q.q && q.k && q.v && q.dout && q.lse && q.delta && q.dk && q.dv, "sdt_attention_bwd_dkv_group: problem %d: null pointer", i);
+    SDT_CHECK_ARG((((uintptr_t)q.q | (uintptr_t)q.k | (uintptr_t)q.v | (uintptr_t)q.dout | (uintptr_t)q.dk | (uintptr_t)q.dv |
+                    (uintptr_t)q.slabs | (uintptr_t)q.lse | (uintptr_t)q.delta) & 15) == 0,
+                  "sdt_attention_bwd_dkv_group: problem %d: pointers must be 16-byte aligned", i);
+    ps[i] = AttnParams{};
+    int rc = attn_fill_bwd(&ps[i], &q.desc, "sdt_attention_bwd_dkv_group", q.q, q.k, q.v, nullptr, q.dout, q.lse, q.delta, nullptr, q.dk, q.dv);
+    if (rc) return rc;
+    SDT_CHECK_ARG(ps[i].lddk % 8 == 0 && ps[i].lddv % 8 == 0 && ps[i].lddo % 8 == 0,
+                  "sdt_attention_bwd_dkv_group: problem %d: row strides must be multiples of 8", i);
+    nsplit[i] = 0;
+    if (attn_qsplits(ps[i].B, ps[i].H, ps[i].Nq, ps[i].Nk, ps[i].causal) > 1) {
+      SDT_CHECK_ARG(q.slabs, "sdt_attention_bwd_dkv_group: problem %d: slabs of sdt_attention_bwd_slab_bytes() needed", i);
+      ps[i].kv_ws = q.slabs;
+      nsplit[i] = attn_split_plan(&ps[i]);
+    }
+    gxs[i] = nsplit[i] ? ps[i].kblocks * nsplit[i] : sdt_ceil_div(ps[i].Nk, 128);
+    all_wgs += (long)gxs[i] * ps[i].H * ps[i].B;
+    SDT_CHECK_ARG(all_wgs < (1L << 30), "sdt_attention_bwd_dkv_group: too many workgroups");
+  }
+  AttnGroupParams gp;
+  for (int cls = 0; cls < 6; ++cls) {
+    gp.n = 0;
+    for (int i = 0; i <= n; ++i) {
+      if (i < n && attn_class(ps[i].D) == cls) {
+        const AttnParams& p = ps[i];
+        gp.prob[gp.n] = p;
+        gp.gx[gp.n] = gxs[i];
+        gp.wg_end[gp.n] = gxs[i] * p.H * p.B + (gp.n ? gp.wg_end[gp.n - 1] : 0);
+        ++gp.n;
+      }
+      if (gp.n == ATTN_GROUP_MAX || (i == n && gp.n > 0)) {
+        attn_dkv_group_dispatch(cls, gp, stream);
+        gp.n = 0;
+      }
+    }
+  }
+  gp.n = 0;
+  for (int i = 0; i <= n; ++i) {
+    if (i < n && nsplit[i]) {
+      gp.prob[gp.n] = ps[i];
+      gp.gx[gp.n] = nsplit[i];
+      gp.wg_end[gp.n] = attn_finish_blocks(ps[i]) + (gp.n ? gp.wg_end[gp.n - 1] : 0);
+      ++gp.n;
+    }
+    if (gp.n == ATTN_GROUP_MAX || (i == n && gp.n > 0)) {
+      hipLaunchKernelGGL(attn_kv_finish_group_kernel, dim3(gp.wg_end[gp.n - 1]), dim3(256), 0, stream, gp);
+      gp.n = 0;
+    }
+  }
+  SDT_LAUNCH_CHECK("sdt_attention_bwd_dkv_group");
+  return SDT_OK;
+}
+
+}
diff --git a/stable_diffusion_training_amd/csrc/elementwise.hip b/stable_diffusion_training_amd/csrc/elementwise.hip
--- a/stable_diffusion_training_amd/csrc/elementwise.hip
+++ b/stable_diffusion_training_amd/csrc/elementwise.hip
@@ -1149,15 +1149,15 @@
   }
 }
 
-__global__ void __launch_bounds__(256) colsum_kernel(const bf16_t* __restrict__ dy, float* __restrict__ db, bf16_t* __restrict__ out_bf,
-                                                     long M, int N, int ld, int rows_per_block, long batch_stride_dy,
-                                                     int batch_stride_db, int* counters, float* __restrict__ part) {
-  dy += (long)blockIdx.z * batch_stride_dy;
+__device__ __forceinline__ void colsum_body(const bf16_t* __restrict__ dy, float* __restrict__ db, bf16_t* __restrict__ out_bf, long M, int N,
+                                            int ld, int rows_per_block, long batch_stride_dy, int batch_stride_db, int* counters,
+                                            float* __restrict__ part, const int bx, const int by, const int bz, const int gx, const int gy) {
+  dy += (long)bz * batch_stride_dy;
   __shared__ float red[8][32][8];
   __shared__ int s_last;
   const int tx = threadIdx.x & 31, ty = threadIdx.x >> 5;
-  const int cv = blockIdx.x * 32 + tx;
-  const long m0 = (long)blockIdx.y * rows_per_block;
+  const int cv = bx * 32 + tx;
+  const long m0 = (long)by * rows_per_block;
   const long m1 = (m0 + rows_per_block < M) ? m0 + rows_per_block : M;
   float acc[8] = {0, 0, 0, 0, 0, 0, 0, 0};
   if (cv * 8 < N) {
@@ -1171,23 +1171,56 @@
 #pragma unroll
   for (int j = 0; j < 8; ++j) red[ty][tx][j] = acc[j];
   __syncthreads();
-  const int group = blockIdx.z * gridDim.x + blockIdx.x;
-  float* grp = part + (long)group * gridDim.y * 256;
+  const int group = bz * gx + bx;
+  float* grp = part + (long)group * gy * 256;
   {
     const int col = threadIdx.x;
     float sum = 0.f;
 #pragma unroll
     for (int k = 0; k < 8; ++k) sum += red[k][col >> 3][col & 7];
-    sdt_store_wt(grp + (long)blockIdx.y * 256 + col, sum);
-  }
-  if (!sdt_arrive_last<true>(counters + group, (int)gridDim.y, &s_last)) return;
-  const int n = blockIdx.x * 256 + threadIdx.x;
+    sdt_store_wt(grp + (long)by * 256 + col, sum);
+  }
+  if (!sdt_arrive_last<true>(counters + group, gy, &s_last)) return;
+  const int n = bx * 256 + threadIdx.x;
   if (n < N) {
     float t = 0.f;
-    for (int y = 0; y < (int)gridDim.y; ++y) t += sdt_load_wt(grp + (long)y * 256 + threadIdx.x);
-    if (out_bf) out_bf[(long)blockIdx.z * batch_stride_db + n] = f2bf(t);
-    else db[(long)blockIdx.z * batch_stride_db + n] += t;
-  }
+    for (int y = 0; y < gy; ++y) t += sdt_load_wt(grp + (long)y * 256 + threadIdx.x);
+    if (out_bf) out_bf[(long)bz * batch_stride_db + n] = f2bf(t);
+    else db[(long)bz * batch_stride_db + n] += t;
+  }
+}
+__global__ void __launch_bounds__(256) colsum_kernel(const bf16_t* __restrict__ dy, float* __restrict__ db, bf16_t* __restrict__ out_bf,
+                                                     long M, int N, int ld, int rows_per_block, long batch_stride_dy,
+                                                     int batch_stride_db, int* counters, float* __restrict__ part) {
+  colsum_body(dy, db, out_bf, M, N, ld, rows_per_block, batch_stride_dy, batch_stride_db, counters, part, (int)blockIdx.x, (int)blockIdx.y,
+              (int)blockIdx.z, (int)gridDim.x, (int)gridDim.y);
+}
+
+#define COLSUM_GROUP_MAX 32
+struct ColsumGroupItem {
+  const bf16_t* dy;
+  bf16_t* out;
+  long M;
+  int N, ld, rows_per_block, gx, gy;
+  int counter0;
+  long part0;
+};
+struct ColsumGroupParams {
+  int n;
+  int wg_end[COLSUM_GROUP_MAX];
+  ColsumGroupItem item[COLSUM_GROUP_MAX];
+};
+static_assert(sizeof(ColsumGroupParams) <= 4096, "the grouped column-sum launch passes its problem table as kernel arguments");
+__global__ void __launch_bounds__(256) colsum_group_kernel(const ColsumGroupParams gp, int* counters, float* __restrict__ part) {
+  const int blk = blockIdx.x;
+  int i = 0;
+  while (i + 1 < gp.n && blk >= gp.wg_end[i]) ++i;
+  const int local = blk - (i ? gp.wg_end[i - 1] : 0);
+  const ColsumGroupItem it = gp.item[i];
+  const int bx = local % it.gx, rest = local / it.gx;
+  const int by = rest % it.gy, bz = rest / it.gy;
+  colsum_body(it.dy, nullptr, it.out, it.M, it.N, it.ld, it.rows_per_block, it.M * it.ld, it.N, counters + it.counter0, part + it.part0, bx, by,
+              bz, it.gx, it.gy);
 }
 
 
@@ -1827,14 +1860,21 @@
   return colsum_ws_need(ncb * batch, (int)((rows_per_batch + 63) / 64));
 }
 
-static int colsum_launch(const uint16_t* dy, float* db, uint16_t* out_bf, int batch, int64_t rows, int N, int ld, int want_blocks,
-                         void* workspace, int64_t workspace_bytes, const char* name, hipStream_t stream) {
+static void colsum_plan(int batch, int64_t rows, int N, int want_blocks, int* ncb_out, int* nby_out, int* rpb_out) {
   const int ncb = sdt_ceil_div(sdt_ceil_div(N, 8), 32);
   int nby = (int)((rows + 63) / 64);
   const int want = (want_blocks + ncb * batch - 1) / (ncb * batch);
   if (nby > want) nby = want;
   const int rpb = (int)((rows + nby - 1) / nby);
-  nby = sdt_ceil_div(rows, rpb);
+  *ncb_out = ncb;
+  *nby_out = sdt_ceil_div(rows, rpb);
+  *rpb_out = rpb;
+}
+
+static int colsum_launch(const uint16_t* dy, float* db, uint16_t* out_bf, int batch, int64_t rows, int N, int ld, int want_blocks,
+                         void* workspace, int64_t workspace_bytes, const char* name, hipStream_t stream) {
+  int ncb, nby, rpb;
+  colsum_plan(batch, rows, N, want_blocks, &ncb, &nby, &rpb);
   SDT_CHECK_ARG((int64_t)ncb * batch * (int64_t)sizeof(int) <= SDT_WS_COUNTER_BYTES, "%s: too many column groups", name);
   SDT_CHECK_ARG(workspace && ((uintptr_t)workspace & 15) == 0 && workspace_bytes >= colsum_ws_need(ncb * batch, nby),
                 "%s: workspace of sdt_colsum_workspace_bytes() needed", name);
@@ -1865,6 +1905,48 @@
   return SDT_OK;
 }
 
+int sdt_colsum_batched_group_max(void) { return COLSUM_GROUP_MAX; }
+
+static bool colsum_problem_ok(const SdtColsumProblem& q) {
+  return q.dy && q.out && q.batch > 0 && q.batch < 65536 && q.rows_per_batch > 0 && q.N > 0 && q.ld >= q.N && q.ld % 8 == 0 &&
+         ((uintptr_t)q.dy & 15) == 0;
+}
+static int64_t colsum_group_plan(const SdtColsumProblem* q, int n, ColsumGroupParams* gp) {
+  if (!q || n <= 0 || n > COLSUM_GROUP_MAX) return 0;
+  long counters = 0, parts = 0, wgs = 0;
+  for (int i = 0; i < n; ++i) {
+    if (!colsum_problem_ok(q[i])) return 0;
+    int ncb, nby, rpb;
+    colsum_plan(q[i].batch, q[i].rows_per_batch, q[i].N, 512, &ncb, &nby, &rpb);
+    wgs += (long)ncb * nby * q[i].batch;
+    if (wgs >= (1L << 30)) return 0;
+    if (gp) {
+      gp->item[i] = ColsumGroupItem{(const bf16_t*)q[i].dy, (bf16_t*)q[i].out, (long)q[i].rows_per_batch, q[i].N, q[i].ld, rpb, ncb, nby,
+                                    (int)counters, parts};
+      gp->wg_end[i] = (int)wgs;
+    }
+    counters += (long)ncb * q[i].batch;
+    parts += (long)ncb * q[i].batch * nby * 256;
+  }
+  if (counters * (long)sizeof(int) > SDT_WS_COUNTER_BYTES) return 0;
+  if (gp) gp->n = n;
+  return SDT_WS_COUNTER_BYTES + parts * (int64_t)sizeof(float);
+}
+
+int64_t sdt_colsum_batched_group_workspace_bytes(const SdtColsumProblem* problems, int n) { return colsum_group_plan(problems, n, nullptr); }
+
+int sdt_colsum_batched_group(const SdtColsumProblem* problems, int n, void* workspace, int64_t workspace_bytes, hipStream_t stream) {
+  ColsumGroupParams gp;
+  const int64_t need = colsum_group_plan(problems, n, &gp);
+  SDT_CHECK_ARG(need > 0, "sdt_colsum_batched_group: bad args (1..%d problems, each as sdt_colsum_batched_bf16 takes them)", COLSUM_GROUP_MAX);
+  SDT_CHECK_ARG(workspace && ((uintptr_t)workspace & 15) == 0 && workspace_bytes >= need,
+                "sdt_colsum_batched_group: workspace of sdt_colsum_batched_group_workspace_bytes() needed");
+  hipLaunchKernelGGL(colsum_group_kernel, dim3(gp.wg_end[n - 1]), dim3(256), 0, stream, gp, reinterpret_cast<int*>(workspace),
+                     reinterpret_cast<float*>((unsigned char*)workspace + SDT_WS_COUNTER_BYTES));
+  SDT_LAUNCH_CHECK("sdt_colsum_batched_group");
+  return SDT_OK;
+}
+
 int sdt_softmax_rows_inplace(uint16_t* x, int64_t rows, int n, float scale, hipStream_t stream) {
   SDT_CHECK_ARG(x && rows > 0 && n > 0 && rows < 2147483647L, "sdt_softmax_rows_inplace: bad args");
   hipLaunchKernelGGL(softmax_rows_kernel, dim3((unsigned)rows), dim3(256), 0, stream, (bf16_t*)x, n, scale);
diff --git a/stable_diffusion_training_amd/ops.py b/stable_diffusion_training_amd/ops.py
--- a/stable_diffusion_training_amd/ops.py
+++ b/stable_diffusion_training_amd/ops.py
@@ -260,22 +260,73 @@
 _NORM_QUEUE = []
 
 
+_DKV_QUEUE = []
+_COLSUM_QUEUE = []
+_OFFCHAIN = False
+
+
 class wgrad_grouping:
+
+    def __init__(self, offchain=True):
+        self.offchain = bool(offchain)
+
     def __enter__(self):
-        global _WGRAD_QUEUE
-        self.prev = _WGRAD_QUEUE
+        global _WGRAD_QUEUE, _OFFCHAIN
+        self.prev = (_WGRAD_QUEUE, _OFFCHAIN)
         _WGRAD_QUEUE = []
+        _OFFCHAIN = self.offchain
         return self
 
     def __exit__(self, *exc):
-        global _WGRAD_QUEUE
+        global _WGRAD_QUEUE, _OFFCHAIN
         try:
             if exc[0] is None:
                 flush_wgrads()
+                flush_offchain()
         finally:
-            _WGRAD_QUEUE = self.prev
+            _WGRAD_QUEUE, _OFFCHAIN = self.prev
             del _NORM_QUEUE[:]
             del _CONV_QUEUE[:]
+            del _DKV_QUEUE[:]
+            del _COLSUM_QUEUE[:]
+
+
+def _slice_tag(t):
+    tag = getattr(t, "_sdt_col_slice", None)
+    if tag is not None:
+        tag[0] += 1
+    return tag
+
+
+def _deferrable(tag):
+    return _OFFCHAIN and _WGRAD_QUEUE is not None and tag is not None and tag[0] == 1
+
+
+def _note_deferred(tag, grad):
+    tag[1] = grad
+
+
+def defer_colsum(dy, out, batch, rows_per_batch, N, ld):
+    _COLSUM_QUEUE.append((_lib.SdtColsumProblem(dy.data_ptr(), out.data_ptr(), batch, rows_per_batch, N, ld), (dy, out)))
+
+
+def flush_offchain():
+    if _DKV_QUEUE:
+        step = _lib.load().sdt_attention_bwd_dkv_group_max()
+        for i in range(0, len(_DKV_QUEUE), step):
+            jobs = _DKV_QUEUE[i: i + step]
+            arr = (_lib.SdtAttnDkvProblem * len(jobs))(*[j[0] for j in jobs])
+            call("sdt_attention_bwd_dkv_group", arr, len(jobs), _stream())
+        del _DKV_QUEUE[:]
+    if _COLSUM_QUEUE:
+        lib = _lib.load()
+        step = lib.sdt_colsum_batched_group_max()
+        for i in range(0, len(_COLSUM_QUEUE), step):
+            jobs = _COLSUM_QUEUE[i: i + step]
+            arr = (_lib.SdtColsumProblem * len(jobs))(*[j[0] for j in jobs])
+            ws = reduce_workspace(lib.sdt_colsum_batched_group_workspace_bytes(arr, len(jobs)), jobs[0][1][0].device)
+            call("sdt_colsum_batched_group", arr, len(jobs), ws.data_ptr(), ws.numel(), _stream())
+        del _COLSUM_QUEUE[:]
 
 
 def flush_norm_grads():
@@ -552,6 +603,7 @@
                 gn_stats=stats, gn_groups=gn_groups if stats is not None else 0, b_kmajor=True)
         ctx.save_for_backward(x)
         ctx.meta = (store, wpath, bpath, geom, plain, rowbias is not None, residual is not None)
+        ctx.rb_tag = None if rowbias is None else _slice_tag(rowbias)
         if gn_groups:
             ctx.set_materialize_grads(False)
             if stats is not None:
@@ -588,9 +640,13 @@
         drb = None
         if has_rb:
             drb = torch.empty(B, lf.Cp, dtype=BF16, device=x.device)
-            ws = reduce_workspace(_lib.load().sdt_colsum_workspace_bytes(B, geom.out_h * geom.out_w, lf.Cp), x.device)
-            call("sdt_colsum_batched_bf16", dy.data_ptr(), drb.data_ptr(), B, geom.out_h * geom.out_w, lf.Cp, lf.Cp, ws.data_ptr(),
-                 ws.numel(), _stream())
+            if _deferrable(ctx.rb_tag):
+                defer_colsum(dy, drb, B, geom.out_h * geom.out_w, lf.Cp, lf.Cp)
+                _note_deferred(ctx.rb_tag, drb)
+            else:
+                ws = reduce_workspace(_lib.load().sdt_colsum_workspace_bytes(B, geom.out_h * geom.out_w, lf.Cp), x.device)
+                call("sdt_colsum_batched_bf16", dy.data_ptr(), drb.data_ptr(), B, geom.out_h * geom.out_w, lf.Cp, lf.Cp, ws.data_ptr(),
+                     ws.numel(), _stream())
         return dx, drb, (dy if has_res else None), None, None, None, None, None, None
 
 
@@ -765,12 +821,19 @@
     def forward(ctx, y, n):
         ctx.set_materialize_grads(False)
         ctx.n = n
+        ctx.tags = [[0, None] for _ in range(n)]
         C = y.shape[-1] // n
         return tuple(y[..., i * C: (i + 1) * C] for i in range(n))
 
     @staticmethod
     def backward(ctx, *grads):
         n = ctx.n
+        flush_offchain()
+        for i, (g, tag) in enumerate(zip(grads, ctx.tags)):
+            want, tag[1] = tag[1], None
+            if want is not None and (g is None or g.data_ptr() != want.data_ptr()):
+                raise _lib.SdtError(f"col_slices: the gradient of slice {i} was deferred (wgrad_grouping) but the slice has a second consumer; "
+                                    "its sum was formed from an unwritten buffer")
         g0 = next((g for g in grads if g is not None), None)
         if g0 is None:
             return None, None
@@ -782,7 +845,12 @@
 
 
 def col_slices(y, n):
-    return _ColSlices.apply(y, n)
+    out = _ColSlices.apply(y, n)
+    node = out[0].grad_fn
+    tags = node.tags if node is not None else [[0, None] for _ in range(n)]
+    for t, tag in zip(out, tags):
+        t._sdt_col_slice = tag
+    return out
 
 
 def fanout(x, n):
@@ -1107,6 +1175,7 @@
         call("sdt_attention_fwd", q, k, v, out.data_ptr(), lse.data_ptr(), _lib.ctypes.addressof(desc), _stream())
         ctx.save_for_backward(a, b, out, lse)
         ctx.desc, ctx.C = desc, C
+        ctx.kv_tag = None if b is None else _slice_tag(b)
         return out
 
     @staticmethod
@@ -1122,11 +1191,26 @@
         else:
             q, k, v = a.data_ptr(), b.data_ptr(), b.data_ptr() + 2 * C
             dq, dk, dv = da.data_ptr(), db.data_ptr(), db.data_ptr() + 2 * C
+        if _deferrable(ctx.kv_tag):
+            _attention_bwd_deferred(ctx.desc, q, k, v, out, dout, lse, dq, dk, dv, (a, b, db, ctx.key_weight))
+            _note_deferred(ctx.kv_tag, db)
+            return da, db, None, None, None, None
         need = _lib.load().sdt_attention_bwd_workspace_bytes(_lib.ctypes.addressof(ctx.desc))
         ws = torch.empty(need, dtype=torch.uint8, device=a.device)
         call("sdt_attention_bwd", q, k, v, out.data_ptr(), dout.data_ptr(), lse.data_ptr(), dq, dk, dv, ws.data_ptr(), need,
              _lib.ctypes.addressof(ctx.desc), _stream())
         return da, db, None, None, None, None
+
+
+def _attention_bwd_deferred(desc, q, k, v, out, dout, lse, dq, dk, dv, keep):
+    lib = _lib.load()
+    dp = _lib.ctypes.addressof(desc)
+    delta = torch.empty(lib.sdt_attention_bwd_delta_bytes(dp) // 4, dtype=torch.float32, device=out.device)
+    nslab = lib.sdt_attention_bwd_slab_bytes(dp)
+    slabs = torch.empty(nslab // 4, dtype=torch.float32, device=out.device) if nslab else None
+    call("sdt_attention_bwd_dq", q, k, v, out.data_ptr(), dout.data_ptr(), lse.data_ptr(), dq, delta.data_ptr(), dp, _stream())
+    prob = _lib.SdtAttnDkvProblem(q, k, v, dout.data_ptr(), lse.data_ptr(), delta.data_ptr(), dk, dv, _ptr(slabs), desc)
+    _DKV_QUEUE.append((prob, (dout, lse, delta, slabs) + tuple(keep)))
 
 
 def attention_packed(a, b, heads, scale, causal=False, key_weight=None):
@@ -1166,6 +1250,7 @@
              C, ld_ip, scale, _stream())
         ctx.save_for_backward(q, kv_txt, kv_ip, o_txt, lse, scale_ip)
         ctx.desc, ctx.dims = desc, (B, heads, Nq, T, D, C, ld_ip, scale)
+        ctx.kv_tag = _slice_tag(kv_txt)
         return out
 
     @staticmethod
@@ -1175,11 +1260,16 @@
         dout = dout.contiguous()
         dq_txt = torch.empty_like(q)
         dkv_txt = torch.empty(kv_txt.shape, dtype=BF16, device=q.device)
-        need = _lib.load().sdt_attention_bwd_workspace_bytes(_lib.ctypes.addressof(ctx.desc))
-        ws = torch.empty(need, dtype=torch.uint8, device=q.device)
-        call("sdt_attention_bwd", q.data_ptr(), kv_txt.data_ptr(), kv_txt.data_ptr() + 2 * C, o_txt.data_ptr(), dout.data_ptr(),
-             lse.data_ptr(), dq_txt.data_ptr(), dkv_txt.data_ptr(), dkv_txt.data_ptr() + 2 * C, ws.data_ptr(), need,
-             _lib.ctypes.addressof(ctx.desc), _stream())
+        if _deferrable(ctx.kv_tag):
+            _attention_bwd_deferred(ctx.desc, q.data_ptr(), kv_txt.data_ptr(), kv_txt.data_ptr() + 2 * C, o_txt, dout, lse, dq_txt.data_ptr(),
+                                    dkv_txt.data_ptr(), dkv_txt.data_ptr() + 2 * C, (q, kv_txt, dkv_txt, ctx.key_weight))
+            _note_deferred(ctx.kv_tag, dkv_txt)
+        else:
+            need = _lib.load().sdt_attention_bwd_workspace_bytes(_lib.ctypes.addressof(ctx.desc))
+            ws = torch.empty(need, dtype=torch.uint8, device=q.device)
+            call("sdt_attention_bwd", q.data_ptr(), kv_txt.data_ptr(), kv_txt.data_ptr() + 2 * C, o_txt.data_ptr(), dout.data_ptr(),
+                 lse.data_ptr(), dq_txt.data_ptr(), dkv_txt.data_ptr(), dkv_txt.data_ptr() + 2 * C, ws.data_ptr(), need,
+                 _lib.ctypes.addressof(ctx.desc), _stream())
         dq = torch.empty_like(q)
         dkv_ip = torch.empty(B, T, 2 * C, dtype=BF16, device=q.device)
         need = _lib.load().sdt_ip_attention_bwd_workspace_bytes(B, heads, Nq, T, D)
```
